# GaryGky/IDEAL-NeRF

Hardware: AMD Instinct MI355X
Metric: ray-samples/sec (64+128 pts, 512x512), whole job (higher is better)
Workload: dtype f32

## Files before the change

ideal-nerf_amd/_lib.py:

```python
import ctypes as C
import os

HERE = os.path.dirname(os.path.abspath(__file__))
LIB_PATH = os.environ.get("IDN_LIB") or os.path.join(HERE, "libidealnerf.so")

IDN_PREC_F32, IDN_PREC_BF16X3, IDN_PREC_BF16, IDN_PREC_FP16X3, IDN_PREC_BF16X6 = 0, 1, 2, 3, 4
RAY_FLOATS = 11
SAMPLE_MAX_REGION = 4096
SCORE_TILE = 32
PROF_KINDS = ("mlp_fwd", "mlp_fwd_save", "delta_chain", "dw_gemm", "dw_gemm_x6", "mlp_fwd_save_x6", "delta_chain_x6")

fp = C.c_void_p


class FaceNerfParams(C.Structure):
    _fields_ = [("pts_w", fp * 8), ("pts_b", fp * 8), ("views_w", fp * 3), ("views_b", fp * 3),
                ("alpha_w", fp), ("alpha_b", fp), ("rgb_w", fp), ("rgb_b", fp),
                ("dim_aud", C.c_int), ("dim_expr", C.c_int), ("dim_latent", C.c_int)]


class FaceNerfGrads(C.Structure):
    _fields_ = [("pts_w", fp * 8), ("pts_b", fp * 8), ("views_w", fp * 3), ("views_b", fp * 3),
                ("alpha_w", fp), ("alpha_b", fp), ("rgb_w", fp), ("rgb_b", fp)]


class CompositeOut(C.Structure):
    _fields_ = [(n, fp) for n in ("rgb_map", "disp_map", "acc_map", "depth_map", "weights", "rgb_fg", "last_weight")]


class RenderArgs(C.Structure):
    _fields_ = [("rays", fp), ("bc_rgb", fp), ("n_rays", C.c_int64), ("n_samples", C.c_int),
                ("n_importance", C.c_int), ("precision", C.c_int),
                ("packed_coarse", fp), ("folded_coarse", fp), ("packed_fine", fp), ("folded_fine", fp),
                ("t_vals", fp), ("t_rand", fp), ("u", fp), ("u_per_ray", C.c_int)] + \
               [(n, fp) for n in ("rgb_map", "disp_map", "acc_map", "depth_map", "last_weight", "rgb_fg",
                                  "rgb0", "disp0", "acc0", "z_std", "last_weight0", "rgb_fg0",
                                  "tap_z_coarse", "tap_raw_coarse", "tap_weights_coarse", "tap_cdf", "tap_inds",
                                  "tap_z_samples", "tap_z_fine", "tap_raw_fine", "tap_weights_fine")] + \
               [("workspace", fp), ("workspace_bytes", C.c_size_t), ("precision_fine_plus1", C.c_int),
                ("lindisp", C.c_int), ("white_bkgd", C.c_int), ("noise_coarse", fp), ("noise_fine", fp), ("fused_march", C.c_int),
                ("rng_mode", C.c_int), ("rng_seed", C.c_uint64), ("rng_ray0", C.c_int64)]


class AudioNetParams(C.Structure):
    _fields_ = [("conv_w", fp * 4), ("conv_b", fp * 4), ("fc_w", fp * 2), ("fc_b", fp * 2), ("dim_aud", C.c_int)]


class AudioNetGrads(C.Structure):
    _fields_ = [("conv_w", fp * 4), ("conv_b", fp * 4), ("fc_w", fp * 2), ("fc_b", fp * 2)]


class Frame(C.Structure):
    _fields_ = [("c2w", C.c_float * 12), ("H", C.c_int), ("W", C.c_int), ("focal", C.c_float), ("cx", C.c_float), ("cy", C.c_float),
                ("near_", C.c_float), ("far_", C.c_float), ("row0", C.c_int), ("nrows", C.c_int), ("rays_out", fp)]


class RenderOpts(C.Structure):
    _fields_ = [("colour_gate", C.c_int), ("gate_counters", fp)]


ABI_VERSION = 4

PROTOTYPES = {
    "idealnerf_version": (C.c_int, []),
    "idealnerf_last_error": (C.c_char_p, []),
    "idealnerf_packed_weight_floats": (C.c_size_t, [C.c_int]),
    "idealnerf_folded_bias_floats": (C.c_size_t, []),
    "idealnerf_pack_weights": (C.c_int, [C.POINTER(FaceNerfParams), C.c_int, fp, fp]),
    "idealnerf_fold_conditioning": (C.c_int, [C.POINTER(FaceNerfParams), fp, fp, fp, fp, fp]),
    "idealnerf_facenerf_fwd": (C.c_int, [fp, fp, C.c_int, fp, C.c_int64, fp, fp]),
    "idealnerf_query_rays_fwd": (C.c_int, [fp, fp, C.c_int, fp, fp, C.c_int64, C.c_int, fp, fp]),
    "idealnerf_query_points_fwd": (C.c_int, [fp, fp, C.c_int, fp, fp, C.c_int64, C.c_int, fp, fp]),
    "idealnerf_frame_rays": (C.c_int, [C.POINTER(C.c_float), C.c_int, C.c_int, C.c_float, C.c_float, C.c_float,
                                       C.c_float, C.c_float, C.c_int, C.c_int, fp, fp]),
    "idealnerf_to8b": (C.c_int, [fp, C.c_int64, C.c_int, fp, fp, fp]),
    "idealnerf_compose_to8b": (C.c_int, [fp, fp, fp, C.c_int64, C.c_int, fp, fp, fp, fp]),
    "idealnerf_philox_uniform": (C.c_int, [C.c_uint64, C.c_int, C.c_int64, C.c_int64, C.c_int, fp, fp]),
    "idealnerf_sample_pixels_workspace_bytes": (C.c_size_t, []),
    "idealnerf_sample_pixels": (C.c_int, [fp, C.c_int, C.c_int, C.c_int, C.c_int, C.c_int, C.c_int, C.c_uint64, C.c_uint64,
                                          fp, C.c_size_t, fp, fp]),
    "idealnerf_gather_rays": (C.c_int, [fp, C.c_int64, C.POINTER(C.c_float), C.c_int, C.c_int, C.c_float, C.c_float, C.c_float,
                                        fp, fp, fp, fp, fp, fp, fp, fp]),
    "idealnerf_frame_scores_workspace_bytes": (C.c_size_t, [C.c_int, C.c_int]),
    "idealnerf_frame_scores": (C.c_int, [fp, fp, fp, C.c_int, C.c_int, fp, fp, C.c_size_t, fp]),
    "idealnerf_coarse_depths": (C.c_int, [fp, fp, fp, C.c_int, C.c_int64, C.c_int, fp, fp]),
    "idealnerf_composite_fwd": (C.c_int, [fp, fp, fp, fp, fp, C.c_int, C.c_int64, C.c_int, C.POINTER(CompositeOut), fp]),
    "idealnerf_sample_pdf_fwd": (C.c_int, [fp, fp, fp, C.c_int, C.c_int64, C.c_int, C.c_int, fp, fp, fp, fp, fp, fp]),
    "idealnerf_march_fwd": (C.c_int, [fp, fp, fp, fp, fp, C.c_int, fp, C.c_int, C.c_int64, C.c_int, C.c_int,
                                      C.POINTER(CompositeOut), fp, fp, fp, fp, fp, fp]),
    "idealnerf_sample_pdf_bins_fwd": (C.c_int, [fp, fp, fp, C.c_int, C.c_int64, C.c_int, C.c_int, fp, fp, fp, fp]),
    "idealnerf_invert_cdf": (C.c_int, [fp, fp, fp, C.c_int, C.c_int64, C.c_int, C.c_int, fp, fp, fp]),
    "idealnerf_render_workspace_bytes": (C.c_size_t, [C.c_int64, C.c_int, C.c_int]),
    "idealnerf_render_rays_fwd": (C.c_int, [C.POINTER(RenderArgs), fp]),
    "idealnerf_render_frame_workspace_bytes": (C.c_size_t, [C.c_int64, C.c_int, C.c_int]),
    "idealnerf_render_frame_fwd": (C.c_int, [C.POINTER(RenderArgs), C.POINTER(Frame), fp]),
    "idealnerf_render_rays_fwd_opts": (C.c_int, [C.POINTER(RenderArgs), C.POINTER(RenderOpts), fp]),
    "idealnerf_render_frame_fwd_opts": (C.c_int, [C.POINTER(RenderArgs), C.POINTER(Frame), C.POINTER(RenderOpts), fp]),
    "idealnerf_colour_gate_max_dist": (C.c_float, []),
    "idealnerf_audio_net_saved_floats": (C.c_size_t, [C.c_int]),
    "idealnerf_audio_net_fwd": (C.c_int, [C.POINTER(AudioNetParams), fp, C.c_int, fp, fp, fp]),
    "idealnerf_audio_net_bwd": (C.c_int, [C.POINTER(AudioNetParams), C.POINTER(AudioNetGrads), fp, fp, fp, C.c_int, fp]),
    "idealnerf_train_acts_floats": (C.c_size_t, [C.c_int64]),
    "idealnerf_query_rays_train_fwd": (C.c_int, [fp, fp, C.c_int, fp, fp, C.c_int64, C.c_int, fp, fp, fp]),
    "idealnerf_pass_bwd_workspace_bytes": (C.c_size_t, [C.c_int64, C.c_int]),
    "idealnerf_pass_bwd": (C.c_int, [C.POINTER(FaceNerfParams), C.POINTER(FaceNerfGrads), fp, fp, fp, fp, fp, fp, fp,
                                     fp, C.c_int64, C.c_int, fp, fp, fp, fp, fp, fp, fp, C.c_size_t, fp]),
    "idealnerf_facenerf_train_fwd": (C.c_int, [fp, fp, C.c_int, fp, C.c_int64, fp, fp, fp]),
    "idealnerf_facenerf_bwd_workspace_bytes": (C.c_size_t, [C.c_int64]),
    "idealnerf_facenerf_bwd": (C.c_int, [C.POINTER(FaceNerfParams), C.POINTER(FaceNerfGrads), fp, fp, fp, fp, C.c_int64, fp,
                                         fp, fp, fp, fp, fp, C.c_size_t, fp]),
    "idealnerf_dw_gemm_workspace_bytes": (C.c_size_t, []),
    "idealnerf_dw_gemm": (C.c_int, [fp, C.c_int, fp, C.c_int, C.c_int64, fp, fp, C.c_int, fp, C.c_size_t, fp]),
    "idealnerf_profile_begin": (None, []),
    "idealnerf_profile_end": (C.c_int, [C.POINTER(C.c_double), C.POINTER(C.c_int64), C.POINTER(C.c_int64)]),
    "idealnerf_profile_end_kinds": (C.c_int, [C.POINTER(C.c_double), C.POINTER(C.c_int64), C.POINTER(C.c_int64)]),
}

_lib = None


class IdealNerfError(RuntimeError):
    pass


def load():
    global _lib
    if _lib is not None:
        return _lib
    if not os.path.exists(LIB_PATH):
        raise IdealNerfError(
            f"{LIB_PATH} is missing: build the HIP extension first "
            "(python ideal-nerf_amd/build.py, or __graft_entry__.build()). There is no fallback path.")
    lib = C.CDLL(LIB_PATH)
    for name, (res, args) in PROTOTYPES.items():
        fn = getattr(lib, name)
        fn.restype = res
        fn.argtypes = args
    if lib.idealnerf_version() != ABI_VERSION:
        raise IdealNerfError(f"{LIB_PATH} has ABI version {lib.idealnerf_version()}, this package binds version {ABI_VERSION}: rebuild it")
    _lib = lib
    return lib


def check(rc):
    if rc != 0:
        msg = load().idealnerf_last_error()
        raise IdealNerfError(f"libidealnerf error {rc}: {msg.decode() if msg else '?'}")
```

ideal-nerf_amd/csrc/capi.hip:

```cpp
#include "idn_internal.h"
#include <cstdarg>
#include <cstdio>

namespace idn {

static thread_local char g_err[512] = "";

int fail(int code, const char* fmt, ...) {
    va_list ap;
    va_start(ap, fmt);
    vsnprintf(g_err, sizeof(g_err), fmt, ap);
    va_end(ap);
    return code;
}

static int check_precision(int precision) {
    if (precision == IDN_PREC_F32 || precision == IDN_PREC_BF16X3 || precision == IDN_PREC_BF16 || precision == IDN_PREC_FP16X3 ||
        precision == IDN_PREC_BF16X6)
        return IDN_OK;
    return fail(IDN_EUNSUPPORTED, "precision %d is unknown (IDN_PREC_F32, IDN_PREC_BF16X3, IDN_PREC_BF16, IDN_PREC_FP16X3, IDN_PREC_BF16X6)", precision);
}
static int check_precision_train(int precision) {
    if (precision == IDN_PREC_F32 || precision == IDN_PREC_BF16X6) return IDN_OK;
    return fail(IDN_EUNSUPPORTED, "the training path runs fp32-grade arithmetic only: IDN_PREC_F32 or IDN_PREC_BF16X6 (got %d)", precision);
}

int launch_mlp(int precision, const float* packed, const float* folded, const float* x, const float* rays,
               const float* z, const float* pts, const float* dirs, int64_t n_points, int n_samples, float* raw,
               hipStream_t s, int gate, int64_t* gate_counters) {
    if (n_points > 0x7fffffffLL) return fail(IDN_EUNSUPPORTED, "n_points %lld exceeds 2^31-1 per launch", (long long)n_points);
    if ((rays || pts) && n_samples < 1) return fail(IDN_EINVAL, "n_samples < 1");
    if (precision == IDN_PREC_BF16X3)
        return launch_mlp_bf16x3(packed, folded, x, rays, z, pts, dirs, n_points, n_samples, raw, s);
    if (precision == IDN_PREC_BF16)
        return launch_mlp_bf16(packed, folded, x, rays, z, pts, dirs, n_points, n_samples, raw, s);
    if (precision == IDN_PREC_FP16X3)
        return launch_mlp_fp16x3(packed, folded, x, rays, z, pts, dirs, n_points, n_samples, raw, s);
    if (precision == IDN_PREC_BF16X6)
        return launch_mlp_bf16x6(packed, folded, x, rays, z, pts, dirs, n_points, n_samples, raw, s);
    return launch_mlp_f32(packed, folded, x, rays, z, pts, dirs, n_points, n_samples, raw, s, nullptr, 0, gate, gate_counters);
}

static int check_params(const idn_facenerf_params* p) {
    if (!p) return fail(IDN_EINVAL, "params is NULL");
    for (int i = 0; i < 8; ++i)
        if (!p->pts_w[i] || !p->pts_b[i]) return fail(IDN_EINVAL, "pts_linears.%d is NULL", i);
    for (int i = 0; i < 3; ++i)
        if (!p->views_w[i] || !p->views_b[i]) return fail(IDN_EINVAL, "views_linears.%d is NULL", i);
    if (!p->alpha_w || !p->alpha_b || !p->rgb_w || !p->rgb_b) return fail(IDN_EINVAL, "alpha/rgb head is NULL");
    if (p->dim_aud < 0 || p->dim_expr < 0 || p->dim_latent < 0) return fail(IDN_EINVAL, "negative conditioning width");
    return IDN_OK;
}

static const int kProfSlots = 8192;
static bool g_prof_on = false;
static int g_prof_n = 0;
static hipEvent_t g_prof_ev[kProfSlots][2];
static int g_prof_created = 0;
static int64_t g_prof_points[kProfSlots];
static int g_prof_kind[kProfSlots];

ProfScope::ProfScope(hipStream_t s_, int64_t points, int kind) : slot(-1), s(s_) {
    if (!g_prof_on || g_prof_n >= kProfSlots) return;
    slot = g_prof_n++;
    if (slot >= g_prof_created) {
        (void)hipEventCreate(&g_prof_ev[slot][0]);
        (void)hipEventCreate(&g_prof_ev[slot][1]);
        g_prof_created = slot + 1;
    }
    g_prof_points[slot] = points;
    g_prof_kind[slot] = (kind >= 0 && kind < IDN_PROF_KINDS) ? kind : 0;
    (void)hipEventRecord(g_prof_ev[slot][0], s);
}
ProfScope::~ProfScope() {
    if (slot >= 0) (void)hipEventRecord(g_prof_ev[slot][1], s);
}

}

using namespace idn;

extern "C" {

int idealnerf_version(void) { return 4; }
const char* idealnerf_last_error(void) { return g_err; }

size_t idealnerf_packed_weight_floats(int precision) {
    if (precision == IDN_PREC_F32 || precision == IDN_PREC_BF16X3 || precision == IDN_PREC_FP16X3) return (size_t)kStreamFrags * kFragFloats;
    if (precision == IDN_PREC_BF16) return (size_t)kPlainStreamFrags * kFragFloats;
    if (precision == IDN_PREC_BF16X6) return (size_t)kX6StreamFrags * kFragFloats;
    return 0;
}
size_t idealnerf_folded_bias_floats(void) { return kBiasFloats; }

int idealnerf_pack_weights(const idn_facenerf_params* p, int precision, float* packed, void* stream) {
    if (int e = check_params(p)) return e;
    if (int e = check_precision(precision)) return e;
    if (!packed) return fail(IDN_EINVAL, "packed is NULL");
    if (precision == IDN_PREC_BF16X3) return launch_pack_bf16x3(*p, packed, (hipStream_t)stream);
    if (precision == IDN_PREC_FP16X3) return launch_pack_bf16x3(*p, packed, (hipStream_t)stream, 1);
    if (precision == IDN_PREC_BF16) return launch_pack_bf16(*p, packed, (hipStream_t)stream);
    if (precision == IDN_PREC_BF16X6) return launch_pack_bf16x6(*p, packed, (hipStream_t)stream);
    return launch_pack_f32(*p, packed, (hipStream_t)stream);
}

int idealnerf_fold_conditioning(const idn_facenerf_params* p, const float* aud, const float* expr,
                                const float* latent, float* folded, void* stream) {
    if (int e = check_params(p)) return e;
    if (!folded) return fail(IDN_EINVAL, "folded is NULL");
    if ((p->dim_aud > 0) != (aud != nullptr)) return fail(IDN_EINVAL, "aud pointer does not match dim_aud=%d", p->dim_aud);
    if ((p->dim_expr > 0) != (expr != nullptr)) return fail(IDN_EINVAL, "expr pointer does not match dim_expr=%d", p->dim_expr);
    if ((p->dim_latent > 0) != (latent != nullptr))
        return fail(IDN_EINVAL, "latent pointer does not match dim_latent=%d", p->dim_latent);
    return launch_fold(*p, aud, expr, latent, folded, (hipStream_t)stream);
}

int idealnerf_facenerf_fwd(const float* packed, const float* folded, int precision, const float* x, int64_t n,
                           float* out, void* stream) {
    if (int e = check_precision(precision)) return e;
    if (n < 0) return fail(IDN_EINVAL, "n < 0");
    if (n == 0) return IDN_OK;
    if (!packed || !folded || !x || !out) return fail(IDN_EINVAL, "NULL pointer");
    return launch_mlp(precision, packed, folded, x, nullptr, nullptr, nullptr, nullptr, n, 1, out, (hipStream_t)stream);
}

int idealnerf_query_rays_fwd(const float* packed, const float* folded, int precision, const float* rays,
                             const float* z, int64_t n_rays, int n_samples, float* raw, void* stream) {
    if (int e = check_precision(precision)) return e;
    if (n_rays < 0 || n_samples < 1) return fail(IDN_EINVAL, "bad sizes n_rays=%lld n_samples=%d", (long long)n_rays, n_samples);
    if (n_rays == 0) return IDN_OK;
    if (!packed || !folded || !rays || !z || !raw) return fail(IDN_EINVAL, "NULL pointer");
    return launch_mlp(precision, packed, folded, nullptr, rays, z, nullptr, nullptr, n_rays * n_samples, n_samples, raw,
                      (hipStream_t)stream);
}

int idealnerf_query_points_fwd(const float* packed, const float* folded, int precision, const float* pts,
                               const float* viewdirs, int64_t n_rays, int n_samples, float* raw, void* stream) {
    if (int e = check_precision(precision)) return e;
    if (n_rays < 0 || n_samples < 1) return fail(IDN_EINVAL, "bad sizes n_rays=%lld n_samples=%d", (long long)n_rays, n_samples);
    if (n_rays == 0) return IDN_OK;
    if (!packed || !folded || !pts || !viewdirs || !raw) return fail(IDN_EINVAL, "NULL pointer");
    return launch_mlp(precision, packed, folded, nullptr, nullptr, nullptr, pts, viewdirs, n_rays * n_samples, n_samples,
                      raw, (hipStream_t)stream);
}

int idealnerf_frame_rays(const float* c2w, int H, int W, float focal, float cx, float cy, float near_, float far_,
                         int row0, int nrows, float* rays_out, void* stream) {
    if (!c2w || !rays_out) return fail(IDN_EINVAL, "NULL pointer");
    if (H <= 0 || W <= 0 || row0 < 0 || nrows < 0 || row0 + nrows > H) return fail(IDN_EINVAL, "bad frame/rows");
    if (nrows == 0) return IDN_OK;
    return launch_frame_rays(c2w, H, W, focal, cx, cy, near_, far_, row0, nrows, rays_out, (hipStream_t)stream);
}

int idealnerf_philox_uniform(uint64_t seed, int which, int64_t row0, int64_t n_rows, int n_cols, float* out, void* stream) {
    if (which != 0 && which != 1) return fail(IDN_EINVAL, "which %d (0 = stratified offsets, 1 = importance draws)", which);
    if (row0 < 0 || n_rows < 0 || n_cols < 0) return fail(IDN_EINVAL, "bad sizes");
    if (n_rows == 0 || n_cols == 0) return IDN_OK;
    if (!out) return fail(IDN_EINVAL, "NULL pointer");
    return launch_philox_uniform((unsigned long long)seed, which, row0, n_rows, n_cols, out, (hipStream_t)stream);
}

size_t idealnerf_sample_pixels_workspace_bytes(void) { return 4 * sizeof(int); }

int idealnerf_sample_pixels(const uint8_t* region_map, int H, int W, int n_rect, int n_outside, int n_mouth, int n_torso,
                            uint64_t seed, uint64_t draw, void* workspace, size_t workspace_bytes, int64_t* sel, void* stream) {
    const int counts[4] = {n_rect, n_outside, n_mouth, n_torso};
    static const char* const names[4] = {"rect", "outside", "mouth", "torso"};
    if (H <= 0 || W <= 0 || (int64_t)H * W > (1LL << 30)) return fail(IDN_EINVAL, "bad frame %d x %d", H, W);
    int64_t total = 0;
    for (int g = 0; g < 4; ++g) {
        if (counts[g] < 0) return fail(IDN_EINVAL, "negative %s count %d", names[g], counts[g]);
        if (counts[g] > IDN_SAMPLE_MAX_REGION)
            return fail(IDN_EUNSUPPORTED, "%s count %d exceeds IDN_SAMPLE_MAX_REGION = %d picks per region", names[g], counts[g],
                        IDN_SAMPLE_MAX_REGION);
        total += counts[g];
    }
    if (!region_map || !workspace || (total > 0 && !sel)) return fail(IDN_EINVAL, "NULL pointer");
    if (workspace_bytes < idealnerf_sample_pixels_workspace_bytes() || ((uintptr_t)workspace & 3u))
        return fail(IDN_EWORKSPACE, "workspace of %zu bytes (need %zu, int32-aligned)", workspace_bytes, idealnerf_sample_pixels_workspace_bytes());
    return launch_sample_pixels(region_map, H, W, counts, (unsigned long long)seed, (unsigned long long)draw, (int*)workspace,
                                (long long*)sel, (hipStream_t)stream);
}

int idealnerf_gather_rays(const int64_t* sel, int64_t n, const float* c2w, int H, int W, float focal, float cx, float cy,
                          const uint8_t* image, const uint8_t* background, const float* target_table, const float* background_table,
                          float* batch_rays, float* target_s, float* bc_rgb, void* stream) {
    if (H <= 0 || W <= 0 || (int64_t)H * W > (1LL << 30)) return fail(IDN_EINVAL, "bad frame %d x %d", H, W);
    if (n < 0 || n > 0x7fffffffLL / 8) return fail(IDN_EINVAL, "bad n %lld", (long long)n);
    if (n == 0) return IDN_OK;
    if (!sel || !c2w || !image || !background || !target_table || !background_table || !batch_rays || !target_s || !bc_rgb)
        return fail(IDN_EINVAL, "NULL pointer");
    return launch_gather_rays((const long long*)sel, n, c2w, H, W, focal, cx, cy, image, background, target_table, background_table,
                              batch_rays, target_s, bc_rgb, (hipStream_t)stream);
}

size_t idealnerf_frame_scores_workspace_bytes(int H, int W) { return frame_scores_workspace_bytes(H, W); }

int idealnerf_frame_scores(const float* pred, const uint8_t* truth, const uint8_t* regions, int H, int W, double* out,
                           void* workspace, size_t workspace_bytes, void* stream) {
    if (H <= 0 || W <= 0 || (int64_t)H * W > (1LL << 30)) return fail(IDN_EINVAL, "bad frame %d x %d", H, W);
    if (!pred || !truth || !out) return fail(IDN_EINVAL, "NULL pointer (pred, truth or out)");
    const size_t need = frame_scores_workspace_bytes(H, W);
    if (!workspace || workspace_bytes < need || ((uintptr_t)workspace & 7u))
        return fail(IDN_EINVAL, "workspace of %zu bytes (need %zu, 8-byte aligned)", workspace_bytes, need);
    return launch_frame_scores(pred, truth, regions, H, W, out, (double*)workspace, (hipStream_t)stream);
}

int idealnerf_coarse_depths(const float* rays, const float* t_vals, const float* t_rand, int lindisp, int64_t n_rays,
                            int n_samples, float* z, void* stream) {
    if (n_rays < 0 || n_samples < 1) return fail(IDN_EINVAL, "bad sizes");
    if (n_rays == 0) return IDN_OK;
    if (!rays || !t_vals || !z) return fail(IDN_EINVAL, "NULL pointer");
    return launch_coarse_depths(rays, t_vals, t_rand, n_rays, n_samples, lindisp, z, (hipStream_t)stream);
}

size_t idealnerf_audio_net_saved_floats(int n_windows) { return audio_net_saved_floats(n_windows); }
int idealnerf_audio_net_fwd(const idn_audio_net_params* p, const float* windows, int n_windows, float* out, float* saved,
                            void* stream) {
    return launch_audio_net_fwd(p, windows, n_windows, out, saved, (hipStream_t)stream);
}
int idealnerf_audio_net_bwd(const idn_audio_net_params* p, const idn_audio_net_grads* grads, const float* windows,
                            const float* saved, const float* d_out, int n_windows, void* stream) {
    return launch_audio_net_bwd(p, grads, windows, saved, d_out, n_windows, (hipStream_t)stream);
}

int idealnerf_to8b(const float* rgb, int64_t n_pixels, int swap_rb, uint8_t* out, int* nonfinite_flag, void* stream) {
    if (n_pixels < 0) return fail(IDN_EINVAL, "n_pixels < 0");
    if (n_pixels == 0) return IDN_OK;
    if (!rgb || !out) return fail(IDN_EINVAL, "NULL pointer");
    return launch_to8b(rgb, n_pixels, swap_rb, out, nonfinite_flag, (hipStream_t)stream);
}

int idealnerf_compose_to8b(const float* rgb_head, const float* last_weight, const float* rgb_fg, int64_t n_pixels,
                           int swap_rb, uint8_t* out, uint8_t* fg_out, int* nonfinite_flag, void* stream) {
    if (n_pixels < 0) return fail(IDN_EINVAL, "n_pixels < 0");
    if (n_pixels == 0) return IDN_OK;
    if (!rgb_head || !last_weight || !rgb_fg || !out) return fail(IDN_EINVAL, "NULL pointer");
    return launch_compose_to8b(rgb_head, last_weight, rgb_fg, n_pixels, swap_rb, out, fg_out, nonfinite_flag,
                               (hipStream_t)stream);
}

int idealnerf_composite_fwd(const float* raw, const float* z, const float* rays, const float* bc_rgb,
                            const float* sigma_noise, int white_bkgd, int64_t n_rays, int n_samples,
                            const idn_composite_out* out, void* stream) {
    if (n_rays < 0) return fail(IDN_EINVAL, "n_rays < 0");
    if (n_rays == 0) return IDN_OK;
    if (!raw || !z || !rays || !bc_rgb || !out) return fail(IDN_EINVAL, "NULL pointer");
    return launch_composite(raw, z, rays, bc_rgb, n_rays, n_samples, sigma_noise, white_bkgd, *out, (hipStream_t)stream);
}

int idealnerf_sample_pdf_fwd(const float* z, const float* weights, const float* u, int u_per_ray, int64_t n_rays,
                             int n_samples, int n_importance, float* z_samples, int64_t* inds, float* cdf,
                             float* z_fine, float* z_std, void* stream) {
    if (n_rays < 0) return fail(IDN_EINVAL, "n_rays < 0");
    if (n_rays == 0) return IDN_OK;
    if (!z || !weights || !u) return fail(IDN_EINVAL, "NULL pointer");
    if (n_samples < 3) return fail(IDN_EUNSUPPORTED, "sample_pdf needs n_samples >= 3");
    return launch_sample_pdf(z, weights, nullptr, nullptr, u, u_per_ray, n_rays, n_samples, n_importance, z_samples,
                             inds, cdf, z_fine, z_std, (hipStream_t)stream);
}

int idealnerf_march_fwd(const float* raw, const float* z, const float* rays, const float* bc_rgb, const float* sigma_noise,
                        int white_bkgd, const float* u, int u_per_ray, int64_t n_rays, int n_samples, int n_importance,
                        const idn_composite_out* out, float* z_samples, int64_t* inds, float* cdf, float* z_fine,
                        float* z_std, void* stream) {
    if (n_rays < 0) return fail(IDN_EINVAL, "n_rays < 0");
    if (n_rays == 0) return IDN_OK;
    if (!raw || !z || !rays || !bc_rgb || !u || !out) return fail(IDN_EINVAL, "NULL pointer");
    return launch_march(raw, z, rays, bc_rgb, sigma_noise, white_bkgd, *out, u, u_per_ray, n_rays, n_samples, n_importance,
                        z_samples, inds, cdf, z_fine, z_std, (hipStream_t)stream);
}

int idealnerf_sample_pdf_bins_fwd(const float* bins, const float* weights, const float* u, int u_per_ray,
                                  int64_t n_rays, int n_bins, int n_importance, float* z_samples, int64_t* inds,
                                  float* cdf, void* stream) {
    if (n_rays < 0) return fail(IDN_EINVAL, "n_rays < 0");
    if (n_rays == 0) return IDN_OK;
    if (!bins || !weights || !u) return fail(IDN_EINVAL, "NULL pointer");
    return launch_sample_pdf(nullptr, weights, nullptr, bins, u, u_per_ray, n_rays, n_bins + 1, n_importance, z_samples,
                             inds, cdf, nullptr, nullptr, (hipStream_t)stream);
}

int idealnerf_invert_cdf(const float* cdf, const float* bins, const float* u, int u_per_ray, int64_t n_rays,
                         int n_bins, int n_importance, float* z_samples, int64_t* inds, void* stream) {
    if (n_rays < 0) return fail(IDN_EINVAL, "n_rays < 0");
    if (n_rays == 0) return IDN_OK;
    if (!cdf || !bins || !u) return fail(IDN_EINVAL, "NULL pointer");
    return launch_sample_pdf(nullptr, nullptr, cdf, bins, u, u_per_ray, n_rays, n_bins + 1, n_importance, z_samples,
                             inds, nullptr, nullptr, nullptr, (hipStream_t)stream);
}

size_t idealnerf_train_acts_floats(int64_t n_points) {
    if (n_points <= 0) return 0;
    return (size_t)((n_points + 127) / 128 * 128) * kActColsAll;
}

int idealnerf_query_rays_train_fwd(const float* packed, const float* folded, int precision, const float* rays,
                                   const float* z, int64_t n_rays, int n_samples, float* raw, float* acts,
                                   void* stream) {
    if (int e = check_precision_train(precision)) return e;
    if (n_rays < 0 || n_samples < 1) return fail(IDN_EINVAL, "bad sizes");
    if (n_rays == 0) return IDN_OK;
    if (!packed || !folded || !rays || !z || !raw || !acts) return fail(IDN_EINVAL, "NULL pointer");
    const int64_t n = n_rays * n_samples;
    const int64_t p_pad = (n + 127) / 128 * 128;
    if (precision == IDN_PREC_BF16X6)
        return launch_mlp_bf16x6(packed, folded, nullptr, rays, z, nullptr, nullptr, n, n_samples, raw, (hipStream_t)stream, acts, p_pad);
    return launch_mlp_f32(packed, folded, nullptr, rays, z, nullptr, nullptr, n, n_samples, raw, (hipStream_t)stream,
                          acts, p_pad);
}

size_t idealnerf_pass_bwd_workspace_bytes(int64_t n_rays, int n_samples) {
    if (n_rays <= 0 || n_samples <= 0) return 0;
    return bwd_workspace_bytes(n_rays * n_samples);
}

static int check_grads(const idn_facenerf_grads* grads) {
    if (!grads) return fail(IDN_EINVAL, "grads is NULL");
    for (int i = 0; i < 8; ++i)
        if (!grads->pts_w[i] || !grads->pts_b[i]) return fail(IDN_EINVAL, "grad pts_linears.%d is NULL", i);
    for (int i = 0; i < 3; ++i)
        if (!grads->views_w[i] || !grads->views_b[i]) return fail(IDN_EINVAL, "grad views_linears.%d is NULL", i);
    if (!grads->alpha_w || !grads->alpha_b || !grads->rgb_w || !grads->rgb_b) return fail(IDN_EINVAL, "grad head is NULL");
    return IDN_OK;
}

int idealnerf_pass_bwd(const idn_facenerf_params* p, const idn_facenerf_grads* grads, const float* aud,
                       const float* expr, const float* latent, const float* acts, const float* raw, const float* z,
                       const float* rays, const float* bc_rgb, int64_t n_rays, int n_samples, const float* g_rgb_map,
                       const float* g_rgb_fg, const float* g_last_weight, const float* g_acc, float* d_aud,
                       float* d_latent, void* workspace, size_t workspace_bytes, void* stream) {
    if (int e = check_params(p)) return e;
    if (int e = check_grads(grads)) return e;
    if ((p->dim_aud > 0) != (aud != nullptr) || (p->dim_expr > 0) != (expr != nullptr) ||
        (p->dim_latent > 0) != (latent != nullptr))
        return fail(IDN_EINVAL, "conditioning pointers do not match the widths");
    if (n_rays < 0) return fail(IDN_EINVAL, "n_rays < 0");
    if (n_rays == 0) return IDN_OK;
    if (!acts || !raw || !z || !rays || !bc_rgb) return fail(IDN_EINVAL, "NULL pointer");
    return launch_pass_bwd(*p, *grads, aud, expr, latent, acts, raw, z, rays, bc_rgb, n_rays, n_samples, g_rgb_map,
                           g_rgb_fg, g_last_weight, g_acc, d_aud, d_latent, workspace, workspace_bytes,
                           (hipStream_t)stream);
}

int idealnerf_facenerf_train_fwd(const float* packed, const float* folded, int precision, const float* x, int64_t n,
                                 float* out, float* acts, void* stream) {
    if (int e = check_precision_train(precision)) return e;
    if (n < 0) return fail(IDN_EINVAL, "n < 0");
    if (n == 0) return IDN_OK;
    if (!packed || !folded || !x || !out || !acts) return fail(IDN_EINVAL, "NULL pointer");
    if (n > 0x7fffffffLL) return fail(IDN_EUNSUPPORTED, "n %lld exceeds 2^31-1 per launch", (long long)n);
    const int64_t p_pad = (n + 127) / 128 * 128;
    if (precision == IDN_PREC_BF16X6)
        return launch_mlp_bf16x6(packed, folded, x, nullptr, nullptr, nullptr, nullptr, n, 1, out, (hipStream_t)stream, acts, p_pad);
    return launch_mlp_f32(packed, folded, x, nullptr, nullptr, nullptr, nullptr, n, 1, out, (hipStream_t)stream, acts, p_pad);
}

size_t idealnerf_facenerf_bwd_workspace_bytes(int64_t n) {
    if (n <= 0) return 0;
    return bwd_workspace_bytes(n);
}

int idealnerf_facenerf_bwd(const idn_facenerf_params* p, const idn_facenerf_grads* grads, const float* aud, const float* expr,
                           const float* latent, const float* acts, int64_t n, const float* g_out, float* d_x, float* d_aud,
                           float* d_expr, float* d_latent, void* workspace, size_t workspace_bytes, void* stream) {
    if (int e = check_params(p)) return e;
    if (int e = check_grads(grads)) return e;
    if ((p->dim_aud > 0) != (aud != nullptr) || (p->dim_expr > 0) != (expr != nullptr) ||
        (p->dim_latent > 0) != (latent != nullptr))
        return fail(IDN_EINVAL, "conditioning pointers do not match the widths");
    if (n < 0) return fail(IDN_EINVAL, "n < 0");
    if (n == 0) return IDN_OK;
    if (!acts || !g_out) return fail(IDN_EINVAL, "NULL pointer");
    return launch_facenerf_bwd(*p, *grads, aud, expr, latent, acts, n, g_out, d_x, d_aud, d_expr, d_latent, workspace,
                               workspace_bytes, (hipStream_t)stream);
}

size_t idealnerf_dw_gemm_workspace_bytes(void) { return dw_gemm_workspace_bytes(); }

int idealnerf_dw_gemm(const float* delta, int ld_delta, const float* acts, int ld_acts, int64_t rows, float* dW, float* db,
                      int pipe, void* workspace, size_t workspace_bytes, void* stream) {
    if (!delta || !acts || !dW) return fail(IDN_EINVAL, "NULL pointer");
    return launch_dw_gemm(delta, ld_delta, acts, ld_acts, rows, dW, db, pipe, workspace, workspace_bytes, (hipStream_t)stream);
}

void idealnerf_profile_begin(void) {
    g_prof_n = 0;
    g_prof_on = true;
}

int idealnerf_profile_end_kinds(double* total_ms, int64_t* launches, int64_t* points) {
    g_prof_on = false;
    double ms[IDN_PROF_KINDS] = {0};
    int64_t n[IDN_PROF_KINDS] = {0}, pts[IDN_PROF_KINDS] = {0};
    for (int i = 0; i < g_prof_n; ++i) {
        IDN_HIP_CHECK(hipEventSynchronize(g_prof_ev[i][1]));
        float t = 0;
        IDN_HIP_CHECK(hipEventElapsedTime(&t, g_prof_ev[i][0], g_prof_ev[i][1]));
        const int k = g_prof_kind[i];
        ms[k] += t;
        n[k] += 1;
        pts[k] += g_prof_points[i];
    }
    for (int k = 0; k < IDN_PROF_KINDS; ++k) {
        if (total_ms) total_ms[k] = ms[k];
        if (launches) launches[k] = n[k];
        if (points) points[k] = pts[k];
    }
    return IDN_OK;
}

int idealnerf_profile_end(double* total_ms, int64_t* launches, int64_t* points) {
    double ms[IDN_PROF_KINDS];
    int64_t n[IDN_PROF_KINDS], pts[IDN_PROF_KINDS];
    if (int e = idealnerf_profile_end_kinds(ms, n, pts)) return e;
    if (total_ms) *total_ms = ms[IDN_PROF_MLP_FWD] + ms[IDN_PROF_MLP_FWD_SAVE] + ms[IDN_PROF_MLP_FWD_SAVE_X6];
    if (launches) *launches = n[IDN_PROF_MLP_FWD] + n[IDN_PROF_MLP_FWD_SAVE] + n[IDN_PROF_MLP_FWD_SAVE_X6];
    if (points) *points = pts[IDN_PROF_MLP_FWD] + pts[IDN_PROF_MLP_FWD_SAVE] + pts[IDN_PROF_MLP_FWD_SAVE_X6];
    return IDN_OK;
}

static const int64_t kRenderChunk = 32768;

static size_t align256(size_t x) { return (x + 255) & ~(size_t)255; }

struct RenderWs {
    float *z_c, *raw_c, *z_f, *raw_f;
    size_t bytes;
};
static RenderWs carve(char* base, int64_t n, int S, int Ni) {
    RenderWs w;
    const int64_t c = n < kRenderChunk ? n : kRenderChunk;
    const int Sf = S + Ni;
    size_t off = 0;
    auto take = [&](size_t floats) {
        float* p = reinterpret_cast<float*>(base + off);
        off += align256(floats * sizeof(float));
        return p;
    };
    w.z_c = take((size_t)c * S);
    w.raw_c = take((size_t)c * S * 4);
    w.z_f = take((size_t)c * Sf);
    w.raw_f = take((size_t)c * Sf * 4);
    w.bytes = off;
    return w;
}

size_t idealnerf_render_workspace_bytes(int64_t n_rays, int n_samples, int n_importance) {
    if (n_rays <= 0 || n_samples <= 0 || n_importance < 0) return 0;
    return carve(nullptr, n_rays, n_samples, n_importance).bytes;
}

static int render_impl(const idn_render_args* a, const idn_frame* frame, const idn_render_opts* opts, void* stream_);
int idealnerf_render_rays_fwd(const idn_render_args* a, void* stream_) { return render_impl(a, nullptr, nullptr, stream_); }
int idealnerf_render_rays_fwd_opts(const idn_render_args* a, const idn_render_opts* opts, void* stream_) { return render_impl(a, nullptr, opts, stream_); }
float idealnerf_colour_gate_max_dist(void) { return kGateMaxDist; }

static size_t frame_scratch_bytes(int64_t n_rays) {
    const int64_t c = n_rays < kRenderChunk ? n_rays : kRenderChunk;
    return align256((size_t)c * IDN_RAY_FLOATS * sizeof(float));
}
size_t idealnerf_render_frame_workspace_bytes(int64_t n_rays, int n_samples, int n_importance) {
    const size_t base = idealnerf_render_workspace_bytes(n_rays, n_samples, n_importance);
    return base ? base + frame_scratch_bytes(n_rays) : 0;
}
int idealnerf_render_frame_fwd(const idn_render_args* a, const idn_frame* f, void* stream_) { return idealnerf_render_frame_fwd_opts(a, f, nullptr, stream_); }
int idealnerf_render_frame_fwd_opts(const idn_render_args* a, const idn_frame* f, const idn_render_opts* opts, void* stream_) {
    if (!a || !f) return fail(IDN_EINVAL, "args / frame is NULL");
    if (a->rays) return fail(IDN_EINVAL, "frame mode derives the rays from the camera: args->rays must be NULL");
    if (f->H <= 0 || f->W <= 0 || f->row0 < 0 || f->nrows < 0 || f->row0 + f->nrows > f->H) return fail(IDN_EINVAL, "bad frame / rows");
    if (a->n_rays != (int64_t)f->nrows * f->W) return fail(IDN_EINVAL, "n_rays %lld != nrows * W = %lld", (long long)a->n_rays, (long long)f->nrows * f->W);
    return render_impl(a, f, opts, stream_);
}

static int render_impl(const idn_render_args* a, const idn_frame* frame, const idn_render_opts* opts, void* stream_) {
    if (!a) return fail(IDN_EINVAL, "args is NULL");
    if (opts && opts->colour_gate != 0 && opts->colour_gate != 1) return fail(IDN_EINVAL, "colour_gate %d (1 = on, the default; 0 = off)", opts->colour_gate);
    if (int e = check_precision(a->precision)) return e;
    const int prec_fine = a->precision_fine_plus1 ? a->precision_fine_plus1 - 1 : a->precision;
    if (int e = check_precision(prec_fine)) return e;
    const int64_t n = a->n_rays;
    const int S = a->n_samples, Ni = a->n_importance, Sf = S + Ni;
    if (n < 0 || S < 2 || Ni < 0) return fail(IDN_EINVAL, "bad sizes n=%lld S=%d Ni=%d", (long long)n, S, Ni);
    if (n == 0) return IDN_OK;
    if ((!a->rays && !frame) || !a->bc_rgb || !a->t_vals || !a->packed_coarse || !a->folded_coarse)
        return fail(IDN_EINVAL, "NULL input pointer");
    if (a->rng_mode != 0 && a->rng_mode != 1) return fail(IDN_EINVAL, "rng_mode %d (0 = t_rand / u as tensors, 1 = drawn in the kernels)", a->rng_mode);
    if (a->rng_mode && (a->t_rand || a->u)) return fail(IDN_EINVAL, "rng_mode 1 draws t_rand and u in the kernels: both pointers must be NULL");
    if (a->rng_mode && a->rng_ray0 < 0) return fail(IDN_EINVAL, "rng_ray0 < 0");
    if (Ni > 0 && (!a->packed_fine || !a->folded_fine || (!a->u && !a->rng_mode))) return fail(IDN_EINVAL, "fine pass inputs are NULL");
    if (Ni > 0 && S < 3) return fail(IDN_EUNSUPPORTED, "importance sampling needs n_samples >= 3");
    const size_t need_base = idealnerf_render_workspace_bytes(n, S, Ni);
    const size_t need = need_base + (frame ? frame_scratch_bytes(n) : 0);
    if (!a->workspace || a->workspace_bytes < need)
        return fail(IDN_EWORKSPACE, "workspace %zu bytes < required %zu", a->workspace_bytes, need);
    float* const ray_scratch = frame ? reinterpret_cast<float*>(reinterpret_cast<char*>(a->workspace) + need_base) : nullptr;
    if (a->fused_march != 0 && a->fused_march != 1 && a->fused_march != 2) return fail(IDN_EINVAL, "fused_march %d (0 = kernel sequence, 1 = one kernel, 2 = two kernels)", a->fused_march);
    if (a->fused_march) {
        if (a->precision != IDN_PREC_F32 || prec_fine != IDN_PREC_F32) return fail(IDN_EUNSUPPORTED, "fused march: built for the fp32 arithmetic");
        if (S != 64 || Ni != 128) return fail(IDN_EUNSUPPORTED, "fused march: built for n_samples = 64, n_importance = 128 (got %d, %d)", S, Ni);
        if (a->noise_coarse || a->noise_fine) return fail(IDN_EUNSUPPORTED, "fused march: no density noise");
    }
    const bool gate_on = !opts || opts->colour_gate;
    const int gate_c = gate_on && a->precision == IDN_PREC_F32 && !a->noise_coarse && !a->tap_raw_coarse;
    const int gate_f = gate_on && prec_fine == IDN_PREC_F32 && !a->noise_fine && !a->tap_raw_fine;
    int64_t* const gate_counters = opts ? opts->gate_counters : nullptr;
    hipStream_t st = (hipStream_t)stream_;
    const RenderWs w = carve(reinterpret_cast<char*>(a->workspace), n, S, Ni);

    auto off = [](auto* p, int64_t elems) { return p ? p + elems : p; };
    auto tap = [&](void* dst, const void* src, size_t bytes) -> int {
        if (!dst) return IDN_OK;
        IDN_HIP_CHECK(hipMemcpyAsync(dst, src, bytes, hipMemcpyDeviceToDevice, st));
        return IDN_OK;
    };

    for (int64_t r0 = 0; r0 < n; r0 += kRenderChunk) {
        const int64_t c = (n - r0 < kRenderChunk) ? n - r0 : kRenderChunk;
        const float* rays = frame ? ray_scratch : a->rays + r0 * IDN_RAY_FLOATS;
        if (frame) {
            if (int e = launch_frame_rays_pixels(frame->c2w, frame->H, frame->W, frame->focal, frame->cx, frame->cy, frame->near_, frame->far_,
                                                 (int64_t)frame->row0 * frame->W + r0, (int)c, ray_scratch, st))
                return e;
            if (frame->rays_out)
                IDN_HIP_CHECK(hipMemcpyAsync(frame->rays_out + r0 * IDN_RAY_FLOATS, ray_scratch, (size_t)c * IDN_RAY_FLOATS * sizeof(float),
                                             hipMemcpyDeviceToDevice, st));
        }
        const float* bc = a->bc_rgb + r0 * 3;
        const Draws draws{(unsigned long long)a->rng_seed, (long)(a->rng_ray0 + r0), a->rng_mode};
        if (int e = launch_coarse_depths(rays, a->t_vals, off(a->t_rand, r0 * S), c, S, a->lindisp, w.z_c, st, draws)) return e;
        if (!a->fused_march)
            if (int e = launch_mlp(a->precision, a->packed_coarse, a->folded_coarse, nullptr, rays, w.z_c, nullptr, nullptr, c * S, S, w.raw_c, st, gate_c, gate_counters)) return e;
        idn_composite_out co = {};
        const bool fine = Ni > 0;
        co.rgb_map = off(fine ? a->rgb0 : a->rgb_map, r0 * 3);
        co.disp_map = off(fine ? a->disp0 : a->disp_map, r0);
        co.acc_map = off(fine ? a->acc0 : a->acc_map, r0);
        co.depth_map = fine ? nullptr : off(a->depth_map, r0);
        co.weights = off(a->tap_weights_coarse, r0 * S);
        co.rgb_fg = off(fine ? a->rgb_fg0 : a->rgb_fg, r0 * 3);
        co.last_weight = off(fine ? a->last_weight0 : a->last_weight, r0);
        if (int e = tap(off(a->tap_z_coarse, r0 * S), w.z_c, (size_t)c * S * 4)) return e;
        if (a->fused_march) {
            idn_composite_out fo = {};
            fo.rgb_map = off(a->rgb_map, r0 * 3);
            fo.disp_map = off(a->disp_map, r0);
            fo.acc_map = off(a->acc_map, r0);
            fo.depth_map = off(a->depth_map, r0);
            fo.weights = off(a->tap_weights_fine, r0 * Sf);
            fo.rgb_fg = off(a->rgb_fg, r0 * 3);
            fo.last_weight = off(a->last_weight, r0);
            const float* u = a->u_per_ray ? off(a->u, r0 * Ni) : a->u;
            const bool split = a->fused_march == 2;
            if (int e = launch_render_fused(a->fused_march, a->packed_coarse, a->folded_coarse, a->packed_fine, a->folded_fine, rays, bc, w.z_c,
                                            split ? w.z_f : nullptr, u, a->u_per_ray, c, a->white_bkgd, co, fo, off(a->z_std, r0),
                                            off(a->tap_raw_coarse, r0 * S * 4), off(a->tap_raw_fine, r0 * Sf * 4),
                                            split ? nullptr : off(a->tap_z_fine, r0 * Sf), off(a->tap_inds, r0 * Ni), off(a->tap_z_samples, r0 * Ni),
                                            off(a->tap_cdf, r0 * (S - 1)), st, draws))
                return e;
            if (split)
                if (int e = tap(off(a->tap_z_fine, r0 * Sf), w.z_f, (size_t)c * Sf * 4)) return e;
            continue;
        }
        if (int e = tap(off(a->tap_raw_coarse, r0 * S * 4), w.raw_c, (size_t)c * S * 16)) return e;
        if (!fine) {
            if (int e = launch_composite(w.raw_c, w.z_c, rays, bc, c, S, off(a->noise_coarse, r0 * S), a->white_bkgd, co, st)) return e;
            continue;
        }
        const float* u = a->u_per_ray ? off(a->u, r0 * Ni) : a->u;
        if (int e = launch_march(w.raw_c, w.z_c, rays, bc, off(a->noise_coarse, r0 * S), a->white_bkgd, co, u, a->u_per_ray, c, S, Ni,
                                 off(a->tap_z_samples, r0 * Ni), off(a->tap_inds, r0 * Ni), off(a->tap_cdf, r0 * (S - 1)),
                                 w.z_f, off(a->z_std, r0), st, draws))
            return e;
        if (int e = launch_mlp(prec_fine, a->packed_fine, a->folded_fine, nullptr, rays, w.z_f, nullptr, nullptr, c * Sf, Sf, w.raw_f, st, gate_f,
                                 gate_counters ? gate_counters + 2 : nullptr)) return e;
        idn_composite_out fo = {};
        fo.rgb_map = off(a->rgb_map, r0 * 3);
        fo.disp_map = off(a->disp_map, r0);
        fo.acc_map = off(a->acc_map, r0);
        fo.depth_map = off(a->depth_map, r0);
        fo.weights = off(a->tap_weights_fine, r0 * Sf);
        fo.rgb_fg = off(a->rgb_fg, r0 * 3);
        fo.last_weight = off(a->last_weight, r0);
        if (int e = launch_composite(w.raw_f, w.z_f, rays, bc, c, Sf, off(a->noise_fine, r0 * Sf), a->white_bkgd, fo, st)) return e;
        if (int e = tap(off(a->tap_z_fine, r0 * Sf), w.z_f, (size_t)c * Sf * 4)) return e;
        if (int e = tap(off(a->tap_raw_fine, r0 * Sf * 4), w.raw_f, (size_t)c * Sf * 16)) return e;
    }
    return IDN_OK;
}

}
```

ideal-nerf_amd/csrc/idn_internal.h:

```cpp
#pragma once
#include <hip/hip_runtime.h>
#include <mutex>
#include <stdint.h>
#include <stddef.h>
#include "../../include/idealnerf.h"

namespace idn {

constexpr int kFragBytes = 1024;
constexpr int kFragFloats = 256;
constexpr int kSliceFrags = 64;
constexpr int kRingSlots = 2;
constexpr int kRingFrags = kRingSlots * kSliceFrags;
constexpr int kSliceBytes = kSliceFrags * kFragBytes;

constexpr int kNumLayers = 12;
constexpr int kLayerNT[kNumLayers] = {8, 8, 8, 8, 8, 8, 8, 8, 5, 4, 4, 1};
constexpr int kLayerKG[kNumLayers] = {8, 32, 32, 32, 32, 40, 32, 32, 36, 16, 16, 16};

constexpr int layer_f0(int l) {
    int f = 0;
    for (int i = 0; i < l; ++i) f += kLayerNT[i] * kLayerKG[i];
    return f;
}
constexpr int kUsedFrags = layer_f0(kNumLayers);
constexpr int kNumSlices =
    ((kUsedFrags + kSliceFrags - 1) / kSliceFrags + kRingSlots - 1) / kRingSlots * kRingSlots;
constexpr int kStreamFrags = kNumSlices * kSliceFrags;
static_assert(kUsedFrags == 2244, "layer table changed");
static_assert(kNumSlices % kRingSlots == 0, "slot of a slice must be static across passes");
static_assert(kRingFrags == 128, "FragReader addresses the ring as two 64-fragment halves");

constexpr int plain_f0(int l) {
    int f = 0;
    for (int i = 0; i < l; ++i) f += kLayerNT[i] * (kLayerKG[i] / 2);
    return f;
}
constexpr int kPlainUsedFrags = plain_f0(kNumLayers);
constexpr int kPlainNumSlices =
    ((kPlainUsedFrags + kSliceFrags - 1) / kSliceFrags + kRingSlots - 1) / kRingSlots * kRingSlots;
constexpr int kPlainStreamFrags = kPlainNumSlices * kSliceFrags;
static_assert(kPlainUsedFrags == 1122 && kPlainUsedFrags % 2 == 0, "plain stream table changed");

constexpr int kX6KFrags = 3;
constexpr int kX6SliceFrags = 16 * kX6KFrags;
constexpr int kX6RingFrags = kRingSlots * kX6SliceFrags;
constexpr int kX6UsedFrags = kX6KFrags * kPlainUsedFrags;
constexpr int kX6NumSlices = 2 * kNumSlices;
constexpr int kX6StreamFrags = kX6NumSlices * kX6SliceFrags;
static_assert(kX6UsedFrags <= kX6StreamFrags && kX6StreamFrags - kX6UsedFrags < kX6RingFrags + kX6SliceFrags, "x6 stream table");

constexpr int bias_off(int l) {
    int o = 0;
    for (int i = 0; i < l; ++i) o += kLayerNT[i] * 32;
    return o;
}
constexpr int kAlphaOff = bias_off(kNumLayers);
constexpr int kRgbOff = kAlphaOff + 256;
constexpr int kBiasFloats = kRgbOff + 3 * 128;
static_assert(kBiasFloats == 3136, "bias table changed");

constexpr int kSigmaChannel = 128;

constexpr float kGateMaxDist = 0.0125f;

enum { kActX0 = 0, kActDir = 1, kActA1 = 2, kActV1 = 10, kActCount = 13 };
constexpr int act_width(int i) { return i < 2 ? 64 : (i < kActV1 ? 256 : 128); }
constexpr int act_off(int i) {
    int o = 0;
    for (int k = 0; k < i; ++k) o += act_width(k);
    return o;
}
constexpr int kActCols = act_off(kActCount);
static_assert(kActCols == 2560, "activation slab layout changed");
constexpr int kMaskLayers = 11;
constexpr int kMaskFloatsPerPoint = kMaskLayers * 8;
constexpr int kActColsAll = kActCols + kMaskFloatsPerPoint;
__host__ __device__ inline size_t mask_index(int id, int64_t p_pad, int64_t wave_tile, int lane) {
    return ((size_t)id * (size_t)(p_pad / 32) + (size_t)wave_tile) * 64 + (size_t)lane;
}

int fail(int code, const char* fmt, ...);
#define IDN_HIP_CHECK(expr)                                                                   \
    do {                                                                                      \
        hipError_t _e = (expr);                                                               \
        if (_e != hipSuccess) return ::idn::fail(IDN_EHIP, "%s: %s", #expr, hipGetErrorString(_e)); \
    } while (0)

struct LaunchSetup {
    static constexpr int kMaxDevices = 64;
    std::mutex mu;
    int cus[kMaxDevices] = {};
    template <class OptIn>
    int get(OptIn&& opt_in, int* num_cu) {
        int dev = 0;
        IDN_HIP_CHECK(hipGetDevice(&dev));
        if (dev < 0 || dev >= kMaxDevices) return ::idn::fail(IDN_EUNSUPPORTED, "device index %d out of range", dev);
        std::lock_guard<std::mutex> lock(mu);
        if (!cus[dev]) {
            hipDeviceProp_t prop;
            IDN_HIP_CHECK(hipGetDeviceProperties(&prop, dev));
            if (int e = opt_in()) return e;
            cus[dev] = prop.multiProcessorCount;
        }
        *num_cu = cus[dev];
        return IDN_OK;
    }
};

struct ProfScope {
    int slot;
    hipStream_t s;
    ProfScope(hipStream_t s, int64_t points, int kind = IDN_PROF_MLP_FWD);
    ~ProfScope();
};

int launch_pack_f32(const idn_facenerf_params& p, float* packed, hipStream_t s);
int launch_pack_bf16x3(const idn_facenerf_params& p, float* packed, hipStream_t s, int fmt = 0);
int launch_pack_bf16x6(const idn_facenerf_params& p, float* packed, hipStream_t s);
int launch_mlp_bf16x6(const float* packed, const float* folded, const float* x, const float* rays, const float* z,
                      const float* pts, const float* dirs, int64_t n_points, int n_samples, float* raw, hipStream_t s,
                      float* acts = nullptr, int64_t p_pad = 0);
int launch_pack_bf16(const idn_facenerf_params& p, float* packed, hipStream_t s);
int launch_mlp_bf16(const float* packed, const float* folded, const float* x, const float* rays, const float* z,
                    const float* pts, const float* dirs, int64_t n_points, int n_samples, float* raw, hipStream_t s);
int launch_mlp_bf16x3(const float* packed, const float* folded, const float* x, const float* rays, const float* z,
                      const float* pts, const float* dirs, int64_t n_points, int n_samples, float* raw, hipStream_t s);
int launch_mlp_fp16x3(const float* packed, const float* folded, const float* x, const float* rays, const float* z,
                      const float* pts, const float* dirs, int64_t n_points, int n_samples, float* raw, hipStream_t s);
int launch_mlp(int precision, const float* packed, const float* folded, const float* x, const float* rays,
               const float* z, const float* pts, const float* dirs, int64_t n_points, int n_samples, float* raw,
               hipStream_t s, int gate = 0, int64_t* gate_counters = nullptr);
int launch_fold(const idn_facenerf_params& p, const float* aud, const float* expr, const float* latent,
                float* folded, hipStream_t s);
int launch_mlp_f32(const float* packed, const float* folded, const float* x, const float* rays, const float* z,
                   const float* pts, const float* dirs, int64_t n_points, int n_samples, float* raw, hipStream_t s,
                   float* acts = nullptr, int64_t p_pad = 0, int gate = 0, int64_t* gate_counters = nullptr);

int launch_frame_rays(const float* c2w, int H, int W, float focal, float cx, float cy, float near_, float far_,
                      int row0, int nrows, float* rays_out, hipStream_t s);
int launch_frame_rays_pixels(const float* c2w_host, int H, int W, float focal, float cx, float cy, float near_, float far_,
                             int64_t pix0, int npix, float* rays_out, hipStream_t s);
size_t audio_net_saved_floats(int n);
int launch_audio_net_fwd(const idn_audio_net_params* p, const float* windows, int n, float* out, float* saved, hipStream_t s);
int launch_audio_net_bwd(const idn_audio_net_params* p, const idn_audio_net_grads* g, const float* windows, const float* saved,
                         const float* d_out, int n, hipStream_t s);
int launch_to8b(const float* rgb, int64_t n_pixels, int swap_rb, unsigned char* out, int* flag, hipStream_t s);
int launch_compose_to8b(const float* head, const float* lw, const float* fg, int64_t n_pixels, int swap_rb,
                        unsigned char* out, unsigned char* fg_out, int* flag, hipStream_t s);
struct Draws {
    unsigned long long seed;
    long ray0;
    int on;
};
int launch_philox_uniform(unsigned long long seed, int which, int64_t row0, int64_t n_rows, int n_cols, float* out, hipStream_t s);
int launch_sample_pixels(const unsigned char* map, int H, int W, const int counts[4], unsigned long long seed, unsigned long long draw,
                         int* population, long long* sel, hipStream_t s);
int launch_gather_rays(const long long* sel, int64_t n, const float* c2w_host, int H, int W, float focal, float cx, float cy,
                       const unsigned char* image, const unsigned char* background, const float* target_table,
                       const float* background_table, float* batch_rays, float* target_s, float* bc_rgb, hipStream_t s);
size_t frame_scores_workspace_bytes(int H, int W);
int launch_frame_scores(const float* pred, const unsigned char* truth, const unsigned char* regions, int H, int W, double* out,
                        double* partial, hipStream_t s);
int launch_coarse_depths(const float* rays, const float* t_vals, const float* t_rand, int64_t n_rays, int S,
                         int lindisp, float* z, hipStream_t s, Draws draws = Draws{0, 0, 0});
int launch_composite(const float* raw, const float* z, const float* rays, const float* bc, int64_t n_rays, int S,
                     const float* noise, int white_bkgd, const idn_composite_out& out, hipStream_t s);
int launch_march(const float* raw, const float* z, const float* rays, const float* bc, const float* noise, int white_bkgd,
                 const idn_composite_out& out, const float* u, int u_per_ray, int64_t n_rays, int S, int Ni,
                 float* z_samples, int64_t* inds, float* cdf_out, float* z_fine, float* z_std, hipStream_t s,
                 Draws draws = Draws{0, 0, 0});
int launch_render_fused(int arrangement, const float* packed_c, const float* folded_c, const float* packed_f, const float* folded_f,
                        const float* rays, const float* bc, const float* z_c, float* z_f, const float* u, int u_per_ray, int64_t n_rays,
                        int white_bkgd, const idn_composite_out& co, const idn_composite_out& fo, float* z_std, float* tap_raw_c,
                        float* tap_raw_f, float* tap_z_fine, int64_t* tap_inds, float* tap_z_samples, float* tap_cdf, hipStream_t s,
                        Draws draws = Draws{0, 0, 0});
int launch_sample_pdf(const float* z, const float* weights, const float* cdf_in, const float* bins_in,
                      const float* u, int u_per_ray, int64_t n_rays, int S, int Ni, float* z_samples,
                      int64_t* inds, float* cdf_out, float* z_fine, float* z_std, hipStream_t s);

constexpr int kBwdStages = 11;
constexpr int kBwdNT[kBwdStages] = {4, 4, 4, 8, 8, 8, 8, 8, 8, 8, 8};
constexpr int kBwdKG[kBwdStages] = {2, 16, 16, 18, 32, 32, 32, 32, 32, 32, 32};
constexpr int kBwdHeadFrags = 280, kBwdTrunk0 = 384;
constexpr int bwd_f0(int s) {
    if (s >= 4) return kBwdTrunk0 + 256 * (s - 4);
    int f = 0;
    for (int i = 0; i < s; ++i) f += kBwdNT[i] * kBwdKG[i];
    return f;
}
static_assert(bwd_f0(3) + kBwdNT[3] * kBwdKG[3] == kBwdHeadFrags, "head stages");
constexpr int kBwdStreamFrags = kBwdTrunk0 + 7 * 256;
static_assert(kBwdStreamFrags % kSliceFrags == 0 && kBwdTrunk0 % kRingFrags == 0, "ring phase of the trunk stages");
constexpr int kBwdNumSlices = kBwdStreamFrags / kSliceFrags;

int launch_pack_f32_bwd(const idn_facenerf_params& p, float* packed_bwd, hipStream_t s);
int launch_delta_chain(const float* packed_bwd, const float* acts, int64_t p_pad, const float* d_rgb, float* dv0,
                       float* dv2, float* dv1, float* const da[8], hipStream_t s);
size_t bwd_stream_floats_x6();
int launch_pack_bf16x6_bwd(const idn_facenerf_params& p, float* packed_bwd, hipStream_t s);
int launch_delta_chain_x6(const float* packed_bwd, const float* acts, int64_t p_pad, const float* d_rgb, float* dv0,
                          float* dv2, float* dv1, float* const da[8], hipStream_t s);

size_t dw_gemm_workspace_bytes();
int launch_dw_gemm(const float* delta, int ld_delta, const float* acts, int ld_acts, int64_t rows, float* dW, float* db, int pipe,
                   void* ws, size_t ws_bytes, hipStream_t s);

size_t bwd_workspace_bytes(int64_t n_points);
int launch_pass_bwd(const idn_facenerf_params& p, const idn_facenerf_grads& gr, const float* aud, const float* expr,
                    const float* latent, const float* acts, const float* raw, const float* z, const float* rays,
                    const float* bc, int64_t n_rays, int S, const float* g_rgb, const float* g_fg, const float* g_lw,
                    const float* g_acc, float* d_aud, float* d_latent, void* ws, size_t ws_bytes, hipStream_t s);
int launch_facenerf_bwd(const idn_facenerf_params& p, const idn_facenerf_grads& gr, const float* aud, const float* expr,
                        const float* latent, const float* acts, int64_t n, const float* g_out, float* d_x, float* d_aud,
                        float* d_expr, float* d_latent, void* ws, size_t ws_bytes, hipStream_t s);

}
```

ideal-nerf_amd/csrc/mlp_common.h:

```cpp
#pragma once
#include "idn_internal.h"
#include <utility>

namespace idn {

typedef float f32x16 __attribute__((ext_vector_type(16)));
typedef float f32x4 __attribute__((ext_vector_type(4)));

template <int N>
using ic = std::integral_constant<int, N>;

template <class F, int... I>
__device__ __forceinline__ void static_for_impl(F&& f, std::integer_sequence<int, I...>) {
    (f(ic<I>{}), ...);
}
template <int N, class F>
__device__ __forceinline__ void static_for(F&& f) {
    static_for_impl(f, std::make_integer_sequence<int, N>{});
}

#define GLOBAL_PTR(p) ((const __attribute__((address_space(1))) void*)(p))
#define LDS_PTR(p) ((__attribute__((address_space(3))) void*)(p))

constexpr int kAhead = kRingSlots - 1;

template <int NW, int SLICE_FRAGS = kSliceFrags, int SLOTS = kRingSlots, bool DUAL = false>
struct WStreamT {
    static constexpr int kSliceFragsT = SLICE_FRAGS;
    static constexpr int kSliceBytesT = SLICE_FRAGS * kFragBytes;
    static constexpr int kSlotsT = SLOTS;
    static constexpr int kAheadT = SLOTS - 1;
    static constexpr int kPieceBytes = NW * kFragBytes;
    static constexpr int kPieces = kSliceBytesT / kPieceBytes;
    static constexpr int kVmcntOpen = (kAheadT - 1) * kPieces;
    static_assert(kSliceBytesT % kPieceBytes == 0 && kPieces % 4 == 0, "a wave's pieces come in groups of four (one M0 / scalar offset per group)");

    __amdgpu_buffer_rsrc_t rsrc;
    uint32_t voff;
    uint32_t soff;
    int next_slice;
    int num_slices;
    char* ring_wave;
    const float* dual_stream[2];
    int dual_first, dual_period, dual_pass;

    __device__ __forceinline__ void init(const float* stream, int slices, char* ring, int tid, int wave) {
        rsrc = __builtin_amdgcn_make_buffer_rsrc(const_cast<float*>(stream), 0, slices * kSliceBytesT, 0x00020000);
        voff = (tid & 63) * 16 + wave * (kPieces * kFragBytes);
        soff = 0;
        next_slice = 0;
        num_slices = slices;
        ring_wave = ring + wave * (kPieces * kFragBytes);
        static_for<kAheadT>([&](auto S_) { issue_rest<decltype(S_)::value, 0>(); });
    }
    __device__ __forceinline__ void advance() {
        soff += kSliceBytesT;
        if (++next_slice == num_slices) {
            next_slice = 0;
            soff = 0;
            if constexpr (DUAL) {
                if (++dual_pass == dual_period) dual_pass = 0;
                rsrc = __builtin_amdgcn_make_buffer_rsrc(const_cast<float*>(dual_stream[dual_pass < dual_first ? 0 : 1]), 0, num_slices * kSliceBytesT, 0x00020000);
            }
        }
    }
    __device__ __forceinline__ void init_dual(const float* stream0, const float* stream1, int first, int period, int slices, char* ring, int tid, int wave) {
        static_assert(DUAL, "two streams");
        dual_stream[0] = stream0;
        dual_stream[1] = stream1;
        dual_first = first;
        dual_period = period;
        dual_pass = 0;
        init(stream0, slices, ring, tid, wave);
    }
    template <int SLOT, int J>
    __device__ __forceinline__ void issue_piece() {
        __builtin_amdgcn_raw_ptr_buffer_load_lds(rsrc, LDS_PTR(ring_wave + SLOT * kSliceBytesT + (J / 4) * (4 * kFragBytes)), 16, voff,
                                                 soff + (J / 4) * (4 * kFragBytes), (J % 4) * kFragBytes, 0);
        if constexpr (J == kPieces - 1) advance();
    }
    template <int SLOT, int J0>
    __device__ __forceinline__ void issue_rest() {
        static_for<kPieces - J0>([&](auto I) { issue_piece<SLOT, J0 + decltype(I)::value>(); });
    }
    template <int YOUNGER = 0>
    __device__ __forceinline__ void open_slice() {
        static_assert(kVmcntOpen + YOUNGER <= 63, "vmcnt is a 6-bit field");
        asm volatile("s_waitcnt vmcnt(%0)" ::"n"(kVmcntOpen + YOUNGER) : "memory");
        __builtin_amdgcn_s_barrier();
        asm volatile("" ::: "memory");
    }
    template <int F>
    __device__ __forceinline__ void step_piece() {
        constexpr int jpos = (F % SLICE_FRAGS) / 2;
        constexpr int slot = (F / SLICE_FRAGS + kAheadT) % SLOTS;
        if constexpr (jpos < kPieces) issue_piece<slot, jpos>();
    }
    template <int F, int JPOS>
    __device__ __forceinline__ void step_piece_at() {
        constexpr int slot = (F / SLICE_FRAGS + kAheadT) % SLOTS;
        if constexpr (JPOS < kPieces) issue_piece<slot, JPOS>();
    }
};
using WStream = WStreamT<4>;

struct FragReader {
    uint32_t addr0, addr1;
    uint32_t addr2;
    f32x4 pref0, pref1;

    template <int F, int RING_FRAGS = kRingFrags>
    __device__ __forceinline__ f32x4 issue() const {
        constexpr int fr = F % RING_FRAGS;
        f32x4 v;
        if constexpr (fr < 64)
            asm volatile("ds_read_b128 %0, %1 offset:%2" : "=v"(v) : "v"(addr0), "n"(fr * kFragBytes) : "memory");
        else if constexpr (fr < 128)
            asm volatile("ds_read_b128 %0, %1 offset:%2" : "=v"(v) : "v"(addr1), "n"((fr - 64) * kFragBytes) : "memory");
        else
            asm volatile("ds_read_b128 %0, %1 offset:%2" : "=v"(v) : "v"(addr2), "n"((fr - 128) * kFragBytes) : "memory");
        return v;
    }
    template <int Newer>
    static __device__ __forceinline__ void retire(f32x4& v0, f32x4& v1) {
        if constexpr (Newer == 0) asm volatile("s_waitcnt lgkmcnt(0)" : "+v"(v0), "+v"(v1)::"memory");
        else asm volatile("s_waitcnt lgkmcnt(2)" : "+v"(v0), "+v"(v1)::"memory");
    }
};

template <int F_END, int STREAM_FRAGS = kStreamFrags, class WS>
__device__ __forceinline__ void finish_pass(WS& ws) {
    static_assert(F_END % 2 == 0, "pairs");
    static_for<(STREAM_FRAGS - F_END) / 2>([&](auto I) {
        constexpr int f = F_END + 2 * decltype(I)::value;
        if constexpr (f % kSliceFrags == 0) ws.open_slice();
        ws.template step_piece<f>();
    });
}

template <int Q>
__device__ __forceinline__ void bias_quad(f32x16& tile, const float* bias_tile_half ) {
    const f32x4 b = *reinterpret_cast<const f32x4*>(bias_tile_half + 8 * Q);
    tile[4 * Q + 0] = b.x;
    tile[4 * Q + 1] = b.y;
    tile[4 * Q + 2] = b.z;
    tile[4 * Q + 3] = b.w;
}
__device__ __forceinline__ void bias_tile(f32x16& tile, const float* bias_tile_half) {
    bias_quad<0>(tile, bias_tile_half);
    bias_quad<1>(tile, bias_tile_half);
    bias_quad<2>(tile, bias_tile_half);
    bias_quad<3>(tile, bias_tile_half);
}
template <int NT>
__device__ __forceinline__ void load_bias(f32x16 (&acc)[NT], const float* bias_half ) {
    static_for<NT>([&](auto T) { bias_tile(acc[decltype(T)::value], bias_half + 32 * decltype(T)::value); });
}

__device__ __forceinline__ float relu1(float x) {
    const int b = __builtin_bit_cast(int, x);
    return __builtin_bit_cast(float, b > 0 ? b : 0);
}
template <int R0, int CNT>
__device__ __forceinline__ void relu_regs(f32x16& tile) {
    static_for<CNT>([&](auto R) {
        constexpr int r = R0 + decltype(R)::value;
        if constexpr (r < 16) tile[r] = relu1(tile[r]);
    });
}
template <int NT>
__device__ __forceinline__ void relu_tiles(f32x16 (&t)[NT]) {
    static_for<NT>([&](auto T) { relu_regs<0, 16>(t[decltype(T)::value]); });
}

struct NoSide {
    template <int T, int S, int H>
    __device__ __forceinline__ void operator()(ic<T>, ic<S>, ic<H>) const {}
};

struct PeLane {
    int h;
    uint32_t off01, off10;
    __device__ __forceinline__ void init(int h_) {
        h = h_;
        off01 = h_ ? 0x80000000u : 0x40000000u;
        off10 = h_ ? 0x40000000u : 0x80000000u;
    }
};
struct PeAxes {
    uint32_t hi[3], lo[3];
    float raw[3];
    __device__ __forceinline__ void init(const float (&v)[3], int h) {
        uint32_t H[3], Lw[3];
        static_for<3>([&](auto A) {
            constexpr int a = decltype(A)::value;
            const double ph = (double)v[a] * 0.15915494309189535;
            const double t = __builtin_amdgcn_fract(ph) * 4294967296.0;
            H[a] = (uint32_t)t;
            Lw[a] = (uint32_t)((t - (double)H[a]) * 4294967296.0);
        });
        static_for<3>([&](auto A) {
            constexpr int a = decltype(A)::value, a1 = (a + 1) % 3;
            hi[a] = h ? H[a1] : H[a];
            lo[a] = h ? Lw[a1] : Lw[a];
            raw[a] = h ? v[a1] : v[a];
        });
    }
};
template <int K, int L>
struct PeFeat {
    static constexpr bool raw = K < 3;
    static constexpr bool trig = K >= 3 && K < 3 + 6 * L;
    static constexpr int t = trig ? K - 3 : 0;
    static constexpr int b = t / 6, sc = (t % 6) / 3;
};
template <int B>
__device__ __forceinline__ uint32_t pe_phase(const PeAxes& ax, int a) {
    if constexpr (B == 0) return ax.hi[a];
    else return __builtin_amdgcn_alignbit(ax.hi[a], ax.lo[a], 32 - B);
}
template <int K0, int L>
__device__ __forceinline__ float pe_slot(const PeAxes& ax, const PeLane& ln) {
    using F0 = PeFeat<K0, L>;
    using F1 = PeFeat<K0 + 4, L>;
    constexpr int a = K0 % 3;
    if constexpr (!F0::trig && !F1::trig) {
        if constexpr (F0::raw) return ln.h ? 0.0f : ax.raw[a];
        else return 0.0f;
    } else {
        constexpr int b0 = F0::trig ? F0::b : F1::b, b1 = F1::trig ? F1::b : F0::b;
        constexpr int sc0 = F0::trig ? F0::sc : F1::sc, sc1 = F1::trig ? F1::sc : F0::sc;
        uint32_t T;
        if constexpr (b0 == b1) T = pe_phase<b0>(ax, a);
        else T = ln.h ? pe_phase<b1>(ax, a) : pe_phase<b0>(ax, a);
        uint32_t u;
        if constexpr (sc0 == sc1) u = T + (((uint32_t)sc0 << 30) + 0x40000000u);
        else u = T + (sc0 == 0 ? ln.off01 : ln.off10);
        const int rr2 = (int)((u << 1) + 0x80000000u);
        const float x = (float)rr2 * 7.3145905512e-10f;
        const float s2 = x * x;
        float pp = -2.391218132e-08f;
        pp = fmaf(pp, s2, 2.752665757e-06f);
        pp = fmaf(pp, s2, -1.984089153e-04f);
        pp = fmaf(pp, s2, 8.333331268e-03f);
        pp = fmaf(pp, s2, -1.666666663e-01f);
        float r = fmaf(x * s2, pp, x);
        r = __uint_as_float(__float_as_uint(r) ^ (u & 0x80000000u));
        if constexpr (!F0::trig) r = ln.h ? r : (F0::raw ? ax.raw[a] : 0.0f);
        if constexpr (!F1::trig) r = ln.h ? 0.0f : r;
        return r;
    }
}

enum { kModeRays = 0, kModeX = 1, kModePts = 2 };
struct MlpArgs {
    const float* wstream;
    const float* bias;
    const float* x;
    const float* rays;
    const float* z;
    const float* pts;
    const float* dirs;
    long n_points;
    int S;
    float* raw;
    float* acts;
    long p_pad;
};
struct MlpGateArgs : MlpArgs {
    unsigned long long* gate_counters;
};

struct PointIn {
    float f[10];
    float zn;
    int last;
};
struct NoHook {
    __device__ __forceinline__ void operator()() const {}
};
template <int MODE, int NW = 4>
__device__ __forceinline__ void load_point(const MlpArgs& a, long tile, int wave, int m, PointIn& in) {
    if constexpr (MODE == kModeX) return;
    long P = tile * (32 * NW) + wave * 32 + m;
    if (P >= a.n_points) P = a.n_points - 1;
    const unsigned ray = (unsigned)P / (unsigned)a.S;
    if constexpr (MODE == kModeRays) {
        const float* rr = a.rays + (long)ray * IDN_RAY_FLOATS;
        in.f[0] = rr[0]; in.f[1] = rr[1]; in.f[2] = rr[2];
        in.f[3] = rr[3]; in.f[4] = rr[4]; in.f[5] = rr[5];
        in.f[6] = rr[8]; in.f[7] = rr[9]; in.f[8] = rr[10];
        in.f[9] = a.z[P];
    } else {
        in.f[0] = a.pts[P * 3 + 0]; in.f[1] = a.pts[P * 3 + 1]; in.f[2] = a.pts[P * 3 + 2];
        in.f[3] = a.dirs[(long)ray * 3 + 0]; in.f[4] = a.dirs[(long)ray * 3 + 1]; in.f[5] = a.dirs[(long)ray * 3 + 2];
    }
}
__device__ __forceinline__ void touch_point(PointIn& in) {
#pragma unroll
    for (int i = 0; i < 10; ++i) asm volatile("" : "+v"(in.f[i]));
}

__device__ __forceinline__ void load_gate_point(const MlpArgs& a, long tile, int wave, int m, PointIn& in) {
    long P = tile * 128 + wave * 32 + m;
    if (P >= a.n_points) P = a.n_points - 1;
    const unsigned ray = (unsigned)P / (unsigned)a.S;
    in.last = ((unsigned)P - ray * (unsigned)a.S == (unsigned)a.S - 1u) ? 1 : 0;
    in.zn = a.z[in.last ? P : P + 1];
}
__device__ __forceinline__ void touch_gate_point(PointIn& in) { asm volatile("" : "+v"(in.zn), "+v"(in.last)); }
__device__ __forceinline__ bool gate_point_dead(const PointIn& in, float sigma) {
    const float dn = sqrtf((in.f[3] * in.f[3] + in.f[4] * in.f[4]) + in.f[5] * in.f[5]);
    float dist = in.zn - in.f[9];
    dist = dist * dn;
    return in.last != 0 || (sigma <= 0.0f && fabsf(dist) <= kGateMaxDist);
}
template <int MODE>
__device__ __forceinline__ void point_of(const PointIn& in, float (&p)[3], float (&v)[3]) {
    if constexpr (MODE == kModeRays) {
        p[0] = in.f[0] + in.f[3] * in.f[9];
        p[1] = in.f[1] + in.f[4] * in.f[9];
        p[2] = in.f[2] + in.f[5] * in.f[9];
        v[0] = in.f[6]; v[1] = in.f[7]; v[2] = in.f[8];
    } else {
        p[0] = in.f[0]; p[1] = in.f[1]; p[2] = in.f[2];
        v[0] = in.f[3]; v[1] = in.f[4]; v[2] = in.f[5];
    }
}

template <int MODE, class Use>
__device__ __forceinline__ void input_features(const MlpArgs& a, long Pc, int h, const PeLane& pln, const PointIn& in,
                                               Use&& use) {
    if constexpr (MODE == kModeX) {
        const float* xr = a.x + Pc * (IDN_PTS_CH + IDN_VIEWS_CH) + 4 * h;
        use([&](auto K) { constexpr int k = decltype(K)::value; return (k + 4 * h < IDN_PTS_CH) ? xr[k] : 0.0f; },
            [&](auto K) { constexpr int k = decltype(K)::value; return (k + 4 * h < IDN_VIEWS_CH) ? xr[IDN_PTS_CH + k] : 0.0f; });
    } else {
        float p[3], v[3];
        point_of<MODE>(in, p, v);
        PeAxes axp, axd;
        axp.init(p, h);
        axd.init(v, h);
        use([&](auto K) { return pe_slot<decltype(K)::value, 10>(axp, pln); },
            [&](auto K) { return pe_slot<decltype(K)::value, 4>(axd, pln); });
    }
}

__device__ __forceinline__ uint32_t off_bit_source(float x) {
    const int b = __builtin_bit_cast(int, x);
    return (uint32_t)((b > 0 ? b : 0) - 1);
}
template <int T>
__device__ __forceinline__ void collect_signs(const f32x16& tile, uint32_t* mk) {
    static_for<16>([&](auto R) {
        mk[T >> 1] = __builtin_amdgcn_alignbit(mk[T >> 1], off_bit_source(tile[decltype(R)::value]), 31);
    });
}

__device__ __forceinline__ __amdgpu_buffer_rsrc_t rows_rsrc(float* first_row, int ld) {
    return __builtin_amdgcn_make_buffer_rsrc(first_row, 0, 32 * ld * 4, 0x00020000);
}

constexpr int kMlpLds = kRingFrags * kFragBytes + kBiasFloats * 4;
constexpr int kMlpLdsGate = kMlpLds + 16;
constexpr int kStagePitch = 33;
constexpr int kStageFloats = 32 * kStagePitch;
constexpr int kMlpLdsTrain = kMlpLds + 4 * kStageFloats * 4;


}
```

ideal-nerf_amd/csrc/mlp_f32.hip:

```cpp
#include "mlp_f32_layers.h"

namespace idn {

template <int NT, int STEPS, int LD>
struct SaveSide {
    static constexpr bool kShadowStore = STEPS >= 8;
    uint32_t* mk;
    f32x16* out;
    __amdgpu_buffer_rsrc_t rsrc;
    uint32_t voff;
    float* stage;
    float* rb;
    uint32_t raddr;
    int m, h;
    template <int T>
    __device__ __forceinline__ void scatter(ic<T>) const {
        static_for<16>([&](auto R) {
            constexpr int r = decltype(R)::value;
            stage[m * kStagePitch + (r & 3) + 8 * (r >> 2) + 4 * h] = out[T][r];
        });
        asm volatile("" ::: "memory");
    }
    template <int Q>
    __device__ __forceinline__ void rows_read(ic<Q>) const {
        static_for<4>([&](auto I) {
            constexpr int i = decltype(I)::value;
            asm volatile("ds_read_b32 %0, %1 offset:%2" : "=v"(rb[i]) : "v"(raddr), "n"(2 * (4 * Q + i) * kStagePitch * 4) : "memory");
        });
    }
    template <int T, int Q>
    __device__ __forceinline__ void rows_store(ic<T>, ic<Q>) const {
        asm volatile("" : "+v"(rb[0]), "+v"(rb[1]), "+v"(rb[2]), "+v"(rb[3]));
        static_for<4>([&](auto I) {
            constexpr int i = decltype(I)::value;
            __builtin_amdgcn_raw_buffer_store_b32(__builtin_bit_cast(unsigned, rb[i]), rsrc, voff, (2 * (4 * Q + i) * LD + 32 * T) * 4, 0);
        });
    }
    template <int T>
    __device__ __forceinline__ void flush_tile(ic<T>) const {
        scatter(ic<T>{});
        static_for<4>([&](auto Q) {
            rows_read(Q);
            asm volatile("s_waitcnt lgkmcnt(0)" : "+v"(rb[0]), "+v"(rb[1]), "+v"(rb[2]), "+v"(rb[3])::"memory");
            rows_store(ic<T>{}, Q);
        });
    }
    __device__ __forceinline__ void finish() const {
        if constexpr (!kShadowStore) static_for<NT - 1>([&](auto T) { collect_signs<decltype(T)::value>(out[decltype(T)::value], mk); });
        collect_signs<NT - 1>(out[NT - 1], mk);
        relu_regs<0, 16>(out[NT - 1]);
        if constexpr (kShadowStore) flush_tile(ic<NT - 1>{});
        else {
            static_for<NT - 1>([&](auto T) { relu_regs<0, 16>(out[decltype(T)::value]); });
            static_for<NT>([&](auto T) { flush_tile(T); });
        }
    }
    template <int T, int S, int H>
    __device__ __forceinline__ void operator()(ic<T>, ic<S>, ic<H>) const {
        if constexpr (kShadowStore && T > 0 && H == 0) {
            if constexpr (S == 0) {
                collect_signs<T - 1>(out[T - 1], mk);
                relu_regs<0, 16>(out[T - 1]);
            }
            if constexpr (S == 1) scatter(ic<T - 1>{});
            if constexpr (S >= 3 && S <= 6) rows_store(ic<T - 1>{}, ic<S - 3>{});
            if constexpr (S >= 2 && S <= 5) rows_read(ic<S - 2>{});
        }
    }
};

template <int MODE, bool SAVE, bool GATE = false>
__global__ __launch_bounds__(256, 1) void mlp_f32_kernel(std::conditional_t<GATE, MlpGateArgs, MlpArgs> a) {
    static_assert(!GATE || (MODE == kModeRays && !SAVE), "the colour gate is built for the rays-mode inference pass");
    extern __shared__ __attribute__((aligned(16))) char smem[];
    char* ring = smem;
    float* bias_s = reinterpret_cast<float*>(smem + kRingFrags * kFragBytes);
    float* stage = reinterpret_cast<float*>(smem + kMlpLds) + (threadIdx.x >> 6) * kStageFloats;
    const uint32_t raddr = (uint32_t)(uintptr_t)(__attribute__((address_space(3))) float*)stage +
                           (((threadIdx.x & 63) >> 5) * kStagePitch + (threadIdx.x & 31)) * 4;

    const int tid = threadIdx.x;
    const int lane = tid & 63;
    const int wave = __builtin_amdgcn_readfirstlane(tid >> 6);
    const int m = lane & 31, h = lane >> 5;

    for (int i = tid; i < kBiasFloats; i += 256) bias_s[i] = a.bias[i];
    GateWord* gate_words = (GateWord*)(__attribute__((address_space(3))) char*)(smem + kMlpLds);
    if constexpr (GATE)
        if (tid < 2) gate_words[tid] = 0u;
    int gate_par = 0;
    __syncthreads();

    WStream ws;
    ws.init(a.wstream, kNumSlices, ring, tid, wave);
    PeLane pln;
    pln.init(h);

    FragReader fr;
    fr.addr0 = (uint32_t)(uintptr_t)(__attribute__((address_space(3))) char*)ring + lane * 16;
    fr.addr1 = fr.addr0 + 64 * kFragBytes;
    const float* bias_h = bias_s + 4 * h;
    const long ntiles = (a.n_points + 127) >> 7;

    PointIn cur, nxt;
    load_point<MODE>(a, blockIdx.x, wave, m, cur);
    if constexpr (GATE) load_gate_point(a, blockIdx.x, wave, m, cur);
    nxt = cur;
    for (long tile = blockIdx.x; tile < ntiles; tile += gridDim.x) {
        const long P = tile * 128 + wave * 32 + m;
        const bool valid = P < a.n_points;
        const long Pc = valid ? P : a.n_points - 1;

        float pe[8][4], pd[4][4];
        if constexpr (MODE == kModeX) {
            const float* xr = a.x + Pc * (IDN_PTS_CH + IDN_VIEWS_CH);
            static_for<8>([&](auto G) {
                static_for<4>([&](auto J) {
                    constexpr int g = decltype(G)::value, j = decltype(J)::value;
                    const int k = 8 * g + 4 * h + j;
                    pe[g][j] = (k < IDN_PTS_CH) ? xr[k] : 0.0f;
                });
            });
            static_for<4>([&](auto G) {
                static_for<4>([&](auto J) {
                    constexpr int g = decltype(G)::value, j = decltype(J)::value;
                    const int k = 8 * g + 4 * h + j;
                    pd[g][j] = (k < IDN_VIEWS_CH) ? xr[IDN_PTS_CH + k] : 0.0f;
                });
            });
        } else {
            float p[3], v[3];
            point_of<MODE>(cur, p, v);
            PeAxes axp, axd;
            axp.init(p, h);
            axd.init(v, h);
            static_for<8>([&](auto G) {
                static_for<4>([&](auto J) {
                    constexpr int g = decltype(G)::value, j = decltype(J)::value;
                    pe[g][j] = pe_slot<8 * g + j, 10>(axp, pln);
                    if constexpr (g < 4) pd[g][j] = pe_slot<8 * g + j, 4>(axd, pln);
                });
            });
        }
        const long p0 = tile * 128 + wave * 32;
        if constexpr (SAVE) {
            {
                float* x0 = a.acts + act_off(kActX0) * a.p_pad + P * 64 + 4 * h;
                float* dr = a.acts + act_off(kActDir) * a.p_pad + P * 64 + 4 * h;
                static_for<8>([&](auto G) {
                    constexpr int g = decltype(G)::value;
                    f32x4 v = {pe[g][0], pe[g][1], pe[g][2], pe[g][3]};
                    *reinterpret_cast<f32x4*>(x0 + 8 * g) = v;
                });
                static_for<8>([&](auto G) {
                    constexpr int g = decltype(G)::value;
                    f32x4 v = {0.f, 0.f, 0.f, 0.f};
                    if constexpr (g < 4) v = f32x4{pd[g][0], pd[g][1], pd[g][2], pd[g][3]};
                    *reinterpret_cast<f32x4*>(dr + 8 * g) = v;
                });
            }
        }

        float rgb[3], sigma;
        if constexpr (GATE) {
            const bool skipped = f32_inference_pass<true>(
                pe, pd, bias_s, bias_h, ws, fr,
                [&]() { load_point<MODE>(a, tile + gridDim.x, wave, m, nxt); load_gate_point(a, tile + gridDim.x, wave, m, nxt); },
                [&]() { touch_point(nxt); touch_gate_point(nxt); }, rgb, sigma,
                [&](float sg) { return !valid || gate_point_dead(cur, sg); }, gate_words + gate_par, gate_words + (gate_par ^ 1));
            gate_par ^= 1;
            if (a.gate_counters && tid == 0) {
                atomicAdd(a.gate_counters + 0, 1ull);
                if (skipped) atomicAdd(a.gate_counters + 1, 1ull);
            }
        } else if constexpr (!SAVE) {
            f32_inference_pass(pe, pd, bias_s, bias_h, ws, fr,
                               [&]() { if constexpr (MODE != kModeX) load_point<MODE>(a, tile + gridDim.x, wave, m, nxt); },
                               [&]() { if constexpr (MODE != kModeX) touch_point(nxt); }, rgb, sigma);
        } else {
            f32x16 A[8], B[8], V[5];
            float rb[4];
            uint32_t mk[4] = {0u, 0u, 0u, 0u};
            auto store_mask = [&](int id) {
                typedef uint32_t u32x4 __attribute__((ext_vector_type(4)));
                u32x4* mp = reinterpret_cast<u32x4*>(a.acts + (size_t)kActCols * a.p_pad) + mask_index(id, a.p_pad, tile * 4 + wave, lane);
                *mp = u32x4{mk[0], mk[1], mk[2], mk[3]};
            };
            auto pe_get = [&](auto G, auto J) { return pe[decltype(G)::value][decltype(J)::value]; };
            auto tiles_get = [](f32x16* arr) {
                return [arr](auto G, auto J) {
                    constexpr int g = decltype(G)::value, j = decltype(J)::value;
                    return arr[g >> 2][(g & 3) * 4 + j];
                };
            };
            auto layer = [&](auto F0c, auto NTc, auto KGc, auto& out, auto&& bget, const float* bias_l, int save_idx) {
                constexpr int F0 = decltype(F0c)::value, NT = decltype(NTc)::value, KG = decltype(KGc)::value;
                constexpr bool LAST = (F0 + NT * KG == kUsedFrags) || F0 == layer_f0(8) || F0 == layer_f0(10);
                static_assert(layer_f0(5) % kSliceFrags == 0 && layer_f0(6) % kSliceFrags == 0, "input prefetch hooks sit on slice boundaries");
                auto hook = [&]() {
                    if constexpr (MODE != kModeX && F0 == layer_f0(5)) load_point<MODE>(a, tile + gridDim.x, wave, m, nxt);
                    if constexpr (MODE != kModeX && F0 == layer_f0(6)) touch_point(nxt);
                };
                load_bias<NT>(out, bias_l);
                if (save_idx >= 0) {
                    const SaveSide<NT, KG / 2, 32 * NT> side{mk, &out[0], rows_rsrc(a.acts + (long)act_off(save_idx) * a.p_pad + p0 * (32 * NT), 32 * NT),
                                                             (uint32_t)((h * (32 * NT) + m) * 4), stage, rb, raddr, m, h};
                    run_layer<F0, NT, KG, LAST>(out, bget, ws, fr, side, hook);
                    side.finish();
                    store_mask(save_idx - kActA1);
                } else {
                    run_layer<F0, NT, KG, LAST>(out, bget, ws, fr, NoSide{}, hook);
                }
            };
            layer(ic<layer_f0(0)>{}, ic<8>{}, ic<8>{}, A, pe_get, bias_h + bias_off(0), kActA1 + 0);
#pragma unroll 1
            for (int l = 1; l <= 3; l += 2) {
                layer(ic<layer_f0(1)>{}, ic<8>{}, ic<32>{}, B, tiles_get(A), bias_h + l * 256, kActA1 + l);
                layer(ic<layer_f0(2)>{}, ic<8>{}, ic<32>{}, A, tiles_get(B), bias_h + (l + 1) * 256, kActA1 + l + 1);
            }
            layer(ic<layer_f0(5)>{}, ic<8>{}, ic<40>{}, B,
                  [&](auto G, auto J) {
                      constexpr int g = decltype(G)::value, j = decltype(J)::value;
                      if constexpr (g < 8) return pe[g][j];
                      else return A[(g - 8) >> 2][((g - 8) & 3) * 4 + j];
                  },
                  bias_h + bias_off(5), kActA1 + 5);
            layer(ic<layer_f0(6)>{}, ic<8>{}, ic<32>{}, A, tiles_get(B), bias_h + bias_off(6), kActA1 + 6);
            layer(ic<layer_f0(7)>{}, ic<8>{}, ic<32>{}, B, tiles_get(A), bias_h + bias_off(7), kActA1 + 7);
            f32x16(&V4a)[4] = reinterpret_cast<f32x16(&)[4]>(V);
            layer(ic<layer_f0(8)>{}, ic<4>{}, ic<36>{}, V4a,
                  [&](auto G, auto J) {
                      constexpr int g = decltype(G)::value, j = decltype(J)::value;
                      if constexpr (g < 32) return B[g >> 2][(g & 3) * 4 + j];
                      else return pd[g - 32][j];
                  },
                  bias_h + bias_off(8), -1);
            {
                constexpr int f_from = layer_f0(8) + 4 * 36, f_to = layer_f0(9);
                static_assert(f_from / kSliceFrags == (f_to - 1) / kSliceFrags && f_to % kSliceFrags != 0, "the walk stays inside one open slice");
                static_for<(f_to - f_from) / 2>([&](auto I) { ws.template step_piece<f_from + 2 * decltype(I)::value>(); });
                fr.pref0 = fr.template issue<f_to>();
                fr.pref1 = fr.template issue<f_to + 1>();
            }
            {
                float s0 = 0.f, s1 = 0.f, s2 = 0.f, s3 = 0.f;
                static_for<8>([&](auto T) {
                    constexpr int t = decltype(T)::value;
                    static_for<4>([&](auto Q) {
                        constexpr int q = decltype(Q)::value;
                        const f32x4 w = *reinterpret_cast<const f32x4*>(bias_h + kAlphaOff + 32 * t + 8 * q);
                        s0 = fmaf(w.x, B[t][4 * q + 0], s0);
                        s1 = fmaf(w.y, B[t][4 * q + 1], s1);
                        s2 = fmaf(w.z, B[t][4 * q + 2], s2);
                        s3 = fmaf(w.w, B[t][4 * q + 3], s3);
                    });
                });
                const float part = (s0 + s1) + (s2 + s3);
                sigma = bias_s[bias_off(8) + kSigmaChannel] + (part + __shfl_xor(part, 32, 64));
            }
            {
                f32x16(&V4)[4] = reinterpret_cast<f32x16(&)[4]>(V);
                static_for<4>([&](auto T) { collect_signs<decltype(T)::value>(V4[decltype(T)::value], mk); });
                store_mask(kActV1 - kActA1);
                relu_tiles<4>(V4);
                const SaveSide<4, 1, 128> side{mk, &V4[0], rows_rsrc(a.acts + (long)act_off(kActV1) * a.p_pad + p0 * 128, 128),
                                               (uint32_t)((h * 128 + m) * 4), stage, rb, raddr, m, h};
                static_for<4>([&](auto T) { side.flush_tile(T); });
            }
            f32x16(&A4)[4] = reinterpret_cast<f32x16(&)[4]>(A);
            f32x16(&V4b)[4] = reinterpret_cast<f32x16(&)[4]>(V);
            layer(ic<layer_f0(9)>{}, ic<4>{}, ic<16>{}, A4, tiles_get(V), bias_h + bias_off(9), kActV1 + 1);
            layer(ic<layer_f0(10)>{}, ic<4>{}, ic<16>{}, V4b, tiles_get(A), bias_h + bias_off(10), kActV1 + 2);
            finish_pass<layer_f0(11)>(ws);
            rgb[0] = bias_s[bias_off(11) + 0];
            rgb[1] = bias_s[bias_off(11) + 1];
            rgb[2] = bias_s[bias_off(11) + 2];
            {
                float part[3] = {0.f, 0.f, 0.f};
                static_for<4>([&](auto T) {
                    constexpr int t = decltype(T)::value;
                    f32x16 vt = V[t];
                    asm volatile("" : "+v"(vt));
                    static_for<3>([&](auto Cc) {
                        constexpr int c = decltype(Cc)::value;
                        static_for<4>([&](auto Q) {
                            constexpr int q = decltype(Q)::value;
                            const f32x4 w = *reinterpret_cast<const f32x4*>(bias_h + kRgbOff + 128 * c + 32 * t + 8 * q);
                            part[c] = fmaf(w.x, vt[4 * q + 0], part[c]);
                            part[c] = fmaf(w.y, vt[4 * q + 1], part[c]);
                            part[c] = fmaf(w.z, vt[4 * q + 2], part[c]);
                            part[c] = fmaf(w.w, vt[4 * q + 3], part[c]);
                        });
                    });
                    asm volatile("" : "+v"(part[0]), "+v"(part[1]), "+v"(part[2])::"memory");
                });
                static_for<3>([&](auto Cc) {
                    constexpr int c = decltype(Cc)::value;
                    rgb[c] += part[c] + __shfl_xor(part[c], 32, 64);
                });
            }
        }

        if (valid && h == 0) {
            f32x4 o;
            o.x = rgb[0];
            o.y = rgb[1];
            o.z = rgb[2];
            o.w = sigma;
            *reinterpret_cast<f32x4*>(a.raw + P * 4) = o;
        }
        cur = nxt;
    }
    __builtin_amdgcn_s_waitcnt(0);
    __syncthreads();
}

int launch_mlp_f32(const float* packed, const float* folded, const float* x, const float* rays, const float* z,
                   const float* pts, const float* dirs, int64_t n_points, int n_samples, float* raw, hipStream_t s,
                   float* acts, int64_t p_pad, int gate, int64_t* gate_counters) {
    if (n_points <= 0) return IDN_OK;
    static LaunchSetup setup;
    int num_cu = 0;
    if (int e = setup.get([]() -> int {
            IDN_HIP_CHECK(hipFuncSetAttribute(reinterpret_cast<const void*>(&mlp_f32_kernel<kModeRays, false>),
                                              hipFuncAttributeMaxDynamicSharedMemorySize, kMlpLds));
            IDN_HIP_CHECK(hipFuncSetAttribute(reinterpret_cast<const void*>(&mlp_f32_kernel<kModeRays, false, true>),
                                              hipFuncAttributeMaxDynamicSharedMemorySize, kMlpLdsGate));
            IDN_HIP_CHECK(hipFuncSetAttribute(reinterpret_cast<const void*>(&mlp_f32_kernel<kModeX, false>),
                                              hipFuncAttributeMaxDynamicSharedMemorySize, kMlpLds));
            IDN_HIP_CHECK(hipFuncSetAttribute(reinterpret_cast<const void*>(&mlp_f32_kernel<kModePts, false>),
                                              hipFuncAttributeMaxDynamicSharedMemorySize, kMlpLds));
            IDN_HIP_CHECK(hipFuncSetAttribute(reinterpret_cast<const void*>(&mlp_f32_kernel<kModeRays, true>),
                                              hipFuncAttributeMaxDynamicSharedMemorySize, kMlpLdsTrain));
            IDN_HIP_CHECK(hipFuncSetAttribute(reinterpret_cast<const void*>(&mlp_f32_kernel<kModeX, true>),
                                              hipFuncAttributeMaxDynamicSharedMemorySize, kMlpLdsTrain));
            return IDN_OK;
        }, &num_cu))
        return e;
    const int64_t ntiles = (n_points + 127) / 128;
    const int grid = (int)(ntiles < num_cu ? ntiles : num_cu);
    if (gate && (acts || x || pts)) return fail(IDN_EUNSUPPORTED, "the colour gate is built for the rays-mode inference launch");
    MlpArgs a{packed, folded, x, rays, z, pts, dirs, (long)n_points, n_samples, raw, acts, (long)p_pad};
    ProfScope prof(s, n_points, acts ? IDN_PROF_MLP_FWD_SAVE : IDN_PROF_MLP_FWD);
    if (acts) {
        if (pts) return fail(IDN_EUNSUPPORTED, "activation saving is built for the rays+z and the pre-embedded-row input modes");
        if (x)
            hipLaunchKernelGGL((mlp_f32_kernel<kModeX, true>), dim3(grid), dim3(256), kMlpLdsTrain, s, a);
        else
            hipLaunchKernelGGL((mlp_f32_kernel<kModeRays, true>), dim3(grid), dim3(256), kMlpLdsTrain, s, a);
    } else if (x)
        hipLaunchKernelGGL((mlp_f32_kernel<kModeX, false>), dim3(grid), dim3(256), kMlpLds, s, a);
    else if (pts)
        hipLaunchKernelGGL((mlp_f32_kernel<kModePts, false>), dim3(grid), dim3(256), kMlpLds, s, a);
    else if (gate) {
        MlpGateArgs ga;
        static_cast<MlpArgs&>(ga) = a;
        ga.gate_counters = reinterpret_cast<unsigned long long*>(gate_counters);
        hipLaunchKernelGGL((mlp_f32_kernel<kModeRays, false, true>), dim3(grid), dim3(256), kMlpLdsGate, s, ga);
    }
    else
        hipLaunchKernelGGL((mlp_f32_kernel<kModeRays, false>), dim3(grid), dim3(256), kMlpLds, s, a);
    IDN_HIP_CHECK(hipGetLastError());
    return IDN_OK;
}

}
```

ideal-nerf_amd/csrc/mlp_f32_layers.h:

```cpp
#pragma once
#include "mlp_common.h"

namespace idn {

__device__ __forceinline__ f32x16 mfma(float a, float b, f32x16 c) {
    return __builtin_amdgcn_mfma_f32_32x32x2f32(a, b, c, 0, 0, 0);
}

template <int F0, int NT, int KG, bool LAST = false, bool OPENED = false, class BGet, class Side, class Hook = NoHook, class WS = WStream>
__device__ __forceinline__ void run_layer(f32x16 (&out)[NT], BGet&& bget, WS& ws, FragReader& fr, Side&& side,
                                          Hook&& after_open = NoHook{}) {
    constexpr int STEPS = KG / 2, NP = NT * STEPS;
    static_assert(KG % 2 == 0 && F0 % 2 == 0, "fragments are consumed in pairs");
    static_assert(!OPENED || F0 % kSliceFrags == 0, "only a layer that starts a slice can find it opened");
    if constexpr (F0 % kSliceFrags == 0) {
        if constexpr (!OPENED) ws.open_slice();
        after_open();
        fr.pref0 = fr.template issue<F0>();
        fr.pref1 = fr.template issue<F0 + 1>();
    }
    f32x4 a0 = fr.pref0, a1 = fr.pref1;
    static_for<NP>([&](auto PI) {
        constexpr int pi = decltype(PI)::value;
        constexpr int t = pi / STEPS, s = pi % STEPS, g0 = 2 * s, g1 = g0 + 1;
        constexpr int f = F0 + 2 * pi;
        constexpr bool next_crosses = ((f + 2) % kSliceFrags == 0);
        f32x4 n0 = a0, n1 = a1;
        if constexpr (!next_crosses && !(LAST && pi + 1 == NP)) {
            n0 = fr.template issue<f + 2>();
            n1 = fr.template issue<f + 3>();
            FragReader::retire<2>(a0, a1);
        } else {
            FragReader::retire<0>(a0, a1);
        }
        ws.template step_piece<f>();
        out[t] = mfma(a0.x, bget(ic<g0>{}, ic<0>{}), out[t]);
        out[t] = mfma(a0.y, bget(ic<g0>{}, ic<1>{}), out[t]);
        out[t] = mfma(a0.z, bget(ic<g0>{}, ic<2>{}), out[t]);
        out[t] = mfma(a0.w, bget(ic<g0>{}, ic<3>{}), out[t]);
        side(ic<t>{}, ic<s>{}, ic<0>{});
        out[t] = mfma(a1.x, bget(ic<g1>{}, ic<0>{}), out[t]);
        out[t] = mfma(a1.y, bget(ic<g1>{}, ic<1>{}), out[t]);
        out[t] = mfma(a1.z, bget(ic<g1>{}, ic<2>{}), out[t]);
        out[t] = mfma(a1.w, bget(ic<g1>{}, ic<3>{}), out[t]);
        side(ic<t>{}, ic<s>{}, ic<1>{});
        __builtin_amdgcn_sched_barrier(0);
        if constexpr (next_crosses && pi + 1 < NP) {
            ws.open_slice();
            n0 = fr.template issue<f + 2>();
            n1 = fr.template issue<f + 3>();
        }
        a0 = n0;
        a1 = n1;
    });
    fr.pref0 = a0;
    fr.pref1 = a1;
}

template <int NT, int STEPS, bool DEFER>
struct LayerSide {
    f32x16* out;
    f32x16* deferred;
    const float* bias_half;
    template <int T, int S, int H>
    __device__ __forceinline__ void operator()(ic<T>, ic<S>, ic<H>) const {
        constexpr int C = (16 + STEPS - 1) / STEPS;
        constexpr int CD = (32 + STEPS - 1) / STEPS;
        if constexpr (H == 0) {
            if constexpr (T > 0) relu_regs<S * C, C>(out[T - 1]);
            if constexpr (T == 0 && DEFER) relu_regs<S * CD, CD>(*deferred);
        } else {
            if constexpr (T + 1 < NT && S < 4) bias_quad<S>(out[T + 1], bias_half + 32 * (T + 1));
        }
    }
};

typedef volatile __attribute__((address_space(3))) uint32_t GateWord;
struct NoGate {
    __device__ __forceinline__ bool operator()(float) const { return false; }
};
template <bool GATE = false, class WS, class Hook5, class Hook6, class Dead = NoGate>
__device__ __forceinline__ bool f32_inference_pass(const float (&pe)[8][4], const float (&pd)[4][4], const float* bias_s, const float* bias_h,
                                                   WS& ws, FragReader& fr, Hook5&& after_open5, Hook6&& after_open6, float (&rgb)[3],
                                                   float& sigma, Dead&& dead = NoGate{}, GateWord* gate_mine = nullptr,
                                                   GateWord* gate_next = nullptr) {
    f32x16 A[8], B[8], V[5];
    auto pe_get = [&](auto G, auto J) { return pe[decltype(G)::value][decltype(J)::value]; };
    auto tiles_get = [](f32x16* arr) {
        return [arr](auto G, auto J) {
            constexpr int g = decltype(G)::value, j = decltype(J)::value;
            return arr[g >> 2][(g & 3) * 4 + j];
        };
    };
    auto layer = [&](auto F0c, auto NTc, auto KGc, auto DEFERc, auto& out, f32x16* deferred, auto&& bget, const float* bias_l) {
        constexpr int F0 = decltype(F0c)::value, NT = decltype(NTc)::value, KG = decltype(KGc)::value;
        constexpr bool LAST = (F0 + NT * KG == kUsedFrags) || F0 == layer_f0(8) || F0 == layer_f0(10);
        constexpr bool DEFER = decltype(DEFERc)::value != 0;
        static_assert(layer_f0(5) % kSliceFrags == 0 && layer_f0(6) % kSliceFrags == 0, "input prefetch hooks sit on slice boundaries");
        auto hook = [&]() {
            if constexpr (F0 == layer_f0(5)) after_open5();
            if constexpr (F0 == layer_f0(6)) after_open6();
        };
        bias_tile(out[0], bias_l);
        run_layer<F0, NT, KG, LAST, GATE && F0 == layer_f0(8)>(out, bget, ws, fr, LayerSide<NT, KG / 2, DEFER>{&out[0], deferred, bias_l}, hook);
    };
    layer(ic<layer_f0(0)>{}, ic<8>{}, ic<8>{}, ic<0>{}, A, nullptr, pe_get, bias_h + bias_off(0));
#pragma unroll 1
    for (int l = 1; l <= 3; l += 2) {
        layer(ic<layer_f0(1)>{}, ic<8>{}, ic<32>{}, ic<1>{}, B, &A[7], tiles_get(A), bias_h + l * 256);
        layer(ic<layer_f0(2)>{}, ic<8>{}, ic<32>{}, ic<1>{}, A, &B[7], tiles_get(B), bias_h + (l + 1) * 256);
    }
    layer(ic<layer_f0(5)>{}, ic<8>{}, ic<40>{}, ic<1>{}, B, &A[7],
          [&](auto G, auto J) {
              constexpr int g = decltype(G)::value, j = decltype(J)::value;
              if constexpr (g < 8) return pe[g][j];
              else return A[(g - 8) >> 2][((g - 8) & 3) * 4 + j];
          },
          bias_h + bias_off(5));
    layer(ic<layer_f0(6)>{}, ic<8>{}, ic<32>{}, ic<1>{}, A, &B[7], tiles_get(B), bias_h + bias_off(6));
    layer(ic<layer_f0(7)>{}, ic<8>{}, ic<32>{}, ic<1>{}, B, &A[7], tiles_get(A), bias_h + bias_off(7));
    f32x16(&V4a)[4] = reinterpret_cast<f32x16(&)[4]>(V);
    if constexpr (GATE) {
        static_assert(layer_f0(8) % kSliceFrags == 0 && (layer_f0(8) / kSliceFrags) % kRingSlots == 0 && kNumSlices % kRingSlots == 0,
                      "the gate decides where slot 0 opens: a skipped pass refills that slot with slice 0");
        relu_regs<0, 16>(B[7]);
        {
            float s0 = 0.f, s1 = 0.f, s2 = 0.f, s3 = 0.f;
            static_for<8>([&](auto T) {
                constexpr int t = decltype(T)::value;
                static_for<4>([&](auto Q) {
                    constexpr int q = decltype(Q)::value;
                    const f32x4 w = *reinterpret_cast<const f32x4*>(bias_h + kAlphaOff + 32 * t + 8 * q);
                    s0 = fmaf(w.x, B[t][4 * q + 0], s0);
                    s1 = fmaf(w.y, B[t][4 * q + 1], s1);
                    s2 = fmaf(w.z, B[t][4 * q + 2], s2);
                    s3 = fmaf(w.w, B[t][4 * q + 3], s3);
                });
            });
            const float part = (s0 + s1) + (s2 + s3);
            sigma = bias_s[bias_off(8) + kSigmaChannel] + (part + __shfl_xor(part, 32, 64));
        }
        const bool any_live = __builtin_amdgcn_ballot_w64(!dead(sigma)) != 0;
        if (any_live && (threadIdx.x & 63) == 0) *gate_mine = 1u;
        if (threadIdx.x == 0) *gate_next = 0u;
        asm volatile("s_waitcnt lgkmcnt(0)" ::: "memory");
        ws.open_slice();
        if (__builtin_amdgcn_readfirstlane(*gate_mine) == 0u) {
            rgb[0] = rgb[1] = rgb[2] = 0.0f;
            ws.next_slice = 0;
            ws.soff = 0;
            ws.template issue_rest<0, 0>();
            return true;
        }
    }
    layer(ic<layer_f0(8)>{}, ic<4>{}, ic<36>{}, ic<GATE ? 0 : 1>{}, V4a, GATE ? nullptr : &B[7],
          [&](auto G, auto J) {
              constexpr int g = decltype(G)::value, j = decltype(J)::value;
              if constexpr (g < 32) return B[g >> 2][(g & 3) * 4 + j];
              else return pd[g - 32][j];
          },
          bias_h + bias_off(8));
    relu_regs<0, 16>(V[3]);
    {
        constexpr int f_from = layer_f0(8) + 4 * 36, f_to = layer_f0(9);
        static_assert(f_from / kSliceFrags == (f_to - 1) / kSliceFrags && f_to % kSliceFrags != 0, "the walk stays inside one open slice");
        static_for<(f_to - f_from) / 2>([&](auto I) { ws.template step_piece<f_from + 2 * decltype(I)::value>(); });
        fr.pref0 = fr.template issue<f_to>();
        fr.pref1 = fr.template issue<f_to + 1>();
    }
    if constexpr (!GATE)
    {
        float s0 = 0.f, s1 = 0.f, s2 = 0.f, s3 = 0.f;
        static_for<8>([&](auto T) {
            constexpr int t = decltype(T)::value;
            static_for<4>([&](auto Q) {
                constexpr int q = decltype(Q)::value;
                const f32x4 w = *reinterpret_cast<const f32x4*>(bias_h + kAlphaOff + 32 * t + 8 * q);
                s0 = fmaf(w.x, B[t][4 * q + 0], s0);
                s1 = fmaf(w.y, B[t][4 * q + 1], s1);
                s2 = fmaf(w.z, B[t][4 * q + 2], s2);
                s3 = fmaf(w.w, B[t][4 * q + 3], s3);
            });
        });
        const float part = (s0 + s1) + (s2 + s3);
        sigma = bias_s[bias_off(8) + kSigmaChannel] + (part + __shfl_xor(part, 32, 64));
    }
    f32x16(&A4)[4] = reinterpret_cast<f32x16(&)[4]>(A);
    f32x16(&V4b)[4] = reinterpret_cast<f32x16(&)[4]>(V);
    layer(ic<layer_f0(9)>{}, ic<4>{}, ic<16>{}, ic<0>{}, A4, nullptr, tiles_get(V), bias_h + bias_off(9));
    layer(ic<layer_f0(10)>{}, ic<4>{}, ic<16>{}, ic<1>{}, V4b, &A[3], tiles_get(A), bias_h + bias_off(10));
    relu_regs<0, 16>(V[3]);
    finish_pass<layer_f0(11)>(ws);
    rgb[0] = bias_s[bias_off(11) + 0];
    rgb[1] = bias_s[bias_off(11) + 1];
    rgb[2] = bias_s[bias_off(11) + 2];
    {
        float part[3] = {0.f, 0.f, 0.f};
        static_for<4>([&](auto T) {
            constexpr int t = decltype(T)::value;
            f32x16 vt = V[t];
            asm volatile("" : "+v"(vt));
            static_for<3>([&](auto Cc) {
                constexpr int c = decltype(Cc)::value;
                static_for<4>([&](auto Q) {
                    constexpr int q = decltype(Q)::value;
                    const f32x4 w = *reinterpret_cast<const f32x4*>(bias_h + kRgbOff + 128 * c + 32 * t + 8 * q);
                    part[c] = fmaf(w.x, vt[4 * q + 0], part[c]);
                    part[c] = fmaf(w.y, vt[4 * q + 1], part[c]);
                    part[c] = fmaf(w.z, vt[4 * q + 2], part[c]);
                    part[c] = fmaf(w.w, vt[4 * q + 3], part[c]);
                });
            });
            asm volatile("" : "+v"(part[0]), "+v"(part[1]), "+v"(part[2])::"memory");
        });
        static_for<3>([&](auto Cc) {
            constexpr int c = decltype(Cc)::value;
            rgb[c] += part[c] + __shfl_xor(part[c], 32, 64);
        });
    }
    return false;
}

}
```

ideal-nerf_amd/ops.py:

```python
import contextlib
import ctypes as C
import os
from typing import Dict, Optional

import torch

from . import _lib
from ._lib import IDN_PREC_F32, RAY_FLOATS, IdealNerfError, check

PTS_CH, VIEWS_CH, W_HID = 63, 27, 256


def _ptr(t: Optional[torch.Tensor], name="tensor", dtype=torch.float32):
    if t is None:
        return None
    if not t.is_cuda:
        raise IdealNerfError(f"{name} must live on the GPU (got {t.device}); the HIP path has no CPU fallback")
    if t.dtype != dtype:
        raise IdealNerfError(f"{name} must be {dtype} (got {t.dtype})")
    if not t.is_contiguous():
        raise IdealNerfError(f"{name} must be contiguous")
    return t.data_ptr()


def _shape(t: Optional[torch.Tensor], name: str, *shape):
    if t is None:
        return
    got = tuple(t.shape)
    if len(got) != len(shape) or any(s is not None and int(s) != g for s, g in zip(shape, got)):
        want = "[" + ", ".join("*" if s is None else str(int(s)) for s in shape) + "]"
        raise IdealNerfError(f"{name} must be {want}, got {list(got)}")


class _Launch:

    def __init__(self, *tensors, device=None):
        devs = {t.device for t in tensors if t is not None and t.is_cuda}
        if device is not None:
            d = torch.device(device)
            if d.type != "cuda":
                raise IdealNerfError(f"the HIP path renders on the GPU (got device {device}); there is no CPU fallback")
            devs.add(torch.device("cuda", torch.cuda.current_device() if d.index is None else d.index))
        if len(devs) > 1:
            raise IdealNerfError("all tensors of one call must live on the same GPU, got " +
                                 ", ".join(sorted(str(d) for d in devs)))
        self.device = devs.pop() if devs else None
        self._ctx = contextlib.nullcontext()

    def __enter__(self):
        if self.device is not None:
            self._ctx = torch.cuda.device(self.device)
            self._ctx.__enter__()
            self.stream = torch.cuda.current_stream(self.device).cuda_stream
        else:
            self.stream = None
        return self

    def __exit__(self, *exc):
        return self._ctx.__exit__(*exc)


def _precision(precision):
    if precision not in (_lib.IDN_PREC_F32, _lib.IDN_PREC_BF16X3, _lib.IDN_PREC_BF16, _lib.IDN_PREC_FP16X3, _lib.IDN_PREC_BF16X6):
        raise IdealNerfError(f"unknown precision code {precision}")
    return int(precision)


def _net_buffers(lib, packed, folded, precision, which=""):
    if packed is not None:
        _shape(packed, f"packed{which}", lib.idealnerf_packed_weight_floats(_precision(precision)))
    if folded is not None:
        _shape(folded, f"folded{which}", lib.idealnerf_folded_bias_floats())


def params_struct(sd: Dict[str, torch.Tensor], dim_aud: int, dim_expr: int, dim_latent: int, prefix: str = ""):
    p = _lib.FaceNerfParams()
    C_all = PTS_CH + dim_aud + dim_expr + dim_latent

    def get(key, shape):
        t = sd[prefix + key]
        if tuple(t.shape) != shape:
            raise IdealNerfError(f"{key}: shape {tuple(t.shape)} != {shape} "
                                 "(only D=8, W=256, skips=[4], multires=10/4 is compiled)")
        return _ptr(t, key)

    for i in range(8):
        fan_in = C_all if i == 0 else (W_HID + C_all if i == 5 else W_HID)
        p.pts_w[i] = get(f"pts_linears.{i}.weight", (W_HID, fan_in))
        p.pts_b[i] = get(f"pts_linears.{i}.bias", (W_HID,))
    p.views_w[0] = get("views_linears.0.weight", (W_HID // 2, W_HID + VIEWS_CH + dim_expr))
    p.views_b[0] = get("views_linears.0.bias", (W_HID // 2,))
    for i in (1, 2):
        p.views_w[i] = get(f"views_linears.{i}.weight", (W_HID // 2, W_HID // 2))
        p.views_b[i] = get(f"views_linears.{i}.bias", (W_HID // 2,))
    p.alpha_w = get("alpha_linear.weight", (1, W_HID))
    p.alpha_b = get("alpha_linear.bias", (1,))
    p.rgb_w = get("rgb_linear.weight", (3, W_HID // 2))
    p.rgb_b = get("rgb_linear.bias", (3,))
    p.dim_aud, p.dim_expr, p.dim_latent = dim_aud, dim_expr, dim_latent
    return p


def pack_weights(p, device, precision=IDN_PREC_F32) -> torch.Tensor:
    lib = _lib.load()
    with _Launch(device=device) as L:
        out = torch.empty(lib.idealnerf_packed_weight_floats(_precision(precision)), dtype=torch.float32, device=L.device)
        check(lib.idealnerf_pack_weights(C.byref(p), precision, out.data_ptr(), L.stream))
    return out


def fold_conditioning(p, aud, expr, latent, device) -> torch.Tensor:
    lib = _lib.load()
    _shape(aud, "aud", p.dim_aud)
    _shape(expr, "expr", p.dim_expr)
    _shape(latent, "latent", p.dim_latent)
    if aud is None and p.dim_aud:
        raise IdealNerfError(f"aud is None but the network was built with dim_aud={p.dim_aud}")
    with _Launch(aud, expr, latent, device=device) as L:
        out = torch.empty(lib.idealnerf_folded_bias_floats(), dtype=torch.float32, device=L.device)
        check(lib.idealnerf_fold_conditioning(C.byref(p), _ptr(aud, "aud"), _ptr(expr, "expr"), _ptr(latent, "latent"),
                                              out.data_ptr(), L.stream))
    return out


def facenerf_fwd(packed, folded, x, precision=IDN_PREC_F32) -> torch.Tensor:
    lib = _lib.load()
    _shape(x, "x", None, PTS_CH + VIEWS_CH)
    _net_buffers(lib, packed, folded, precision)
    with _Launch(packed, folded, x) as L:
        out = torch.empty((x.shape[0], 4), dtype=torch.float32, device=x.device)
        check(lib.idealnerf_facenerf_fwd(_ptr(packed, "packed"), _ptr(folded, "folded"), precision, _ptr(x, "x"),
                                         x.shape[0], out.data_ptr(), L.stream))
    return out


def facenerf_train_fwd(packed, folded, x, precision=_lib.IDN_PREC_BF16X6):
    lib = _lib.load()
    _shape(x, "x", None, PTS_CH + VIEWS_CH)
    if precision not in (_lib.IDN_PREC_F32, _lib.IDN_PREC_BF16X6):
        raise IdealNerfError(f"the training forward runs IDN_PREC_F32 or IDN_PREC_BF16X6 only (got {precision})")
    _net_buffers(lib, packed, folded, precision)
    n = x.shape[0]
    with _Launch(packed, folded, x) as L:
        out = torch.empty((n, 4), dtype=torch.float32, device=x.device)
        acts = torch.empty(lib.idealnerf_train_acts_floats(n), dtype=torch.float32, device=x.device)
        check(lib.idealnerf_facenerf_train_fwd(_ptr(packed, "packed"), _ptr(folded, "folded"), precision, _ptr(x, "x"), n,
                                               out.data_ptr(), acts.data_ptr(), L.stream))
    return out, acts


def grads_struct(grads: Dict[str, torch.Tensor]):
    g = _lib.FaceNerfGrads()
    for i in range(8):
        g.pts_w[i] = grads[f"pts_linears.{i}.weight"].data_ptr()
        g.pts_b[i] = grads[f"pts_linears.{i}.bias"].data_ptr()
    for i in range(3):
        g.views_w[i] = grads[f"views_linears.{i}.weight"].data_ptr()
        g.views_b[i] = grads[f"views_linears.{i}.bias"].data_ptr()
    g.alpha_w, g.alpha_b = grads["alpha_linear.weight"].data_ptr(), grads["alpha_linear.bias"].data_ptr()
    g.rgb_w, g.rgb_b = grads["rgb_linear.weight"].data_ptr(), grads["rgb_linear.bias"].data_ptr()
    return g


def facenerf_bwd(p, grads, aud, expr, latent, acts, g_out, d_x=None, d_aud=None, d_expr=None, d_latent=None):
    lib = _lib.load()
    _shape(g_out, "g_out", None, 4)
    n = g_out.shape[0]
    _shape(acts, "acts", lib.idealnerf_train_acts_floats(n))
    _shape(d_x, "d_x", n, PTS_CH + VIEWS_CH)
    for t, name, dim in ((aud, "aud", p.dim_aud), (expr, "expr", p.dim_expr), (latent, "latent", p.dim_latent),
                         (d_aud, "d_aud", p.dim_aud), (d_expr, "d_expr", p.dim_expr), (d_latent, "d_latent", p.dim_latent)):
        _shape(t, name, dim)
    for k, t in grads.items():
        _ptr(t, f"grad {k}")
    with _Launch(aud, expr, latent, acts, g_out, d_x, d_aud, d_expr, d_latent, *grads.values()) as L:
        ptrs = [_ptr(t, name) for t, name in ((aud, "aud"), (expr, "expr"), (latent, "latent"), (acts, "acts"))]
        ptrs += [n, _ptr(g_out, "g_out")]
        ptrs += [_ptr(t, name) for t, name in ((d_x, "d_x"), (d_aud, "d_aud"), (d_expr, "d_expr"), (d_latent, "d_latent"))]
        ws = _workspace(lib.idealnerf_facenerf_bwd_workspace_bytes(n), g_out.device, L.stream)
        check(lib.idealnerf_facenerf_bwd(C.byref(p), C.byref(grads_struct(grads)), *ptrs, ws.data_ptr(), ws.numel(), L.stream))
    return grads


def query_rays_train_fwd(packed, folded, rays, z, precision=_lib.IDN_PREC_BF16X6):
    lib = _lib.load()
    _shape(z, "z", None, None)
    n, S = z.shape
    _shape(rays, "rays", n, RAY_FLOATS)
    with _Launch(packed, folded, rays, z) as L:
        raw = torch.empty((n, S, 4), dtype=torch.float32, device=z.device)
        acts = torch.empty(lib.idealnerf_train_acts_floats(n * S), dtype=torch.float32, device=z.device)
        check(lib.idealnerf_query_rays_train_fwd(_ptr(packed, "packed"), _ptr(folded, "folded"), precision, _ptr(rays, "rays"),
                                                 _ptr(z, "z"), n, S, raw.data_ptr(), acts.data_ptr(), L.stream))
    return raw, acts


def pass_bwd(p, grads, aud, expr, latent, acts, raw, z, rays, bc, g_rgb, g_fg, g_lw, g_acc, d_aud, d_latent):
    lib = _lib.load()
    n, S = z.shape
    for t, name, shape in ((raw, "raw", (n, S, 4)), (rays, "rays", (n, RAY_FLOATS)), (bc, "bc_rgb", (n, 3)),
                           (g_rgb, "g_rgb_map", (n, 3)), (g_fg, "g_rgb_fg", (n, 3)), (g_lw, "g_last_weight", (n,)),
                           (g_acc, "g_acc", (n,))):
        _shape(t, name, *shape)
    tensors = (aud, expr, latent, acts, raw, z, rays, bc, g_rgb, g_fg, g_lw, g_acc, d_aud, d_latent)
    with _Launch(*tensors, *grads.values()) as L:
        ws = _workspace(lib.idealnerf_pass_bwd_workspace_bytes(n, S), z.device, L.stream)
        ptrs = [_ptr(t) for t in tensors]
        check(lib.idealnerf_pass_bwd(C.byref(p), C.byref(grads_struct(grads)), *ptrs[:8], n, S, *ptrs[8:], ws.data_ptr(), ws.numel(), L.stream))
    return grads


def query_rays_fwd(packed, folded, rays, z, precision=IDN_PREC_F32) -> torch.Tensor:
    lib = _lib.load()
    _shape(z, "z", None, None)
    n, S = z.shape
    _shape(rays, "rays", n, RAY_FLOATS)
    _net_buffers(lib, packed, folded, precision)
    with _Launch(packed, folded, rays, z) as L:
        raw = torch.empty((n, S, 4), dtype=torch.float32, device=z.device)
        check(lib.idealnerf_query_rays_fwd(_ptr(packed, "packed"), _ptr(folded, "folded"), precision, _ptr(rays, "rays"),
                                           _ptr(z, "z"), n, S, raw.data_ptr(), L.stream))
    return raw


def query_points_fwd(packed, folded, pts, viewdirs, precision=IDN_PREC_F32) -> torch.Tensor:
    lib = _lib.load()
    _shape(pts, "pts", None, None, 3)
    n, S, _ = pts.shape
    _shape(viewdirs, "viewdirs", n, 3)
    _net_buffers(lib, packed, folded, precision)
    with _Launch(packed, folded, pts, viewdirs) as L:
        raw = torch.empty((n, S, 4), dtype=torch.float32, device=pts.device)
        check(lib.idealnerf_query_points_fwd(_ptr(packed, "packed"), _ptr(folded, "folded"), precision, _ptr(pts, "pts"),
                                             _ptr(viewdirs, "viewdirs"), n, S, raw.data_ptr(), L.stream))
    return raw


def frame_rays(c2w, H, W, focal, near, far, row0=0, nrows=None, cx=None, cy=None, device="cuda") -> torch.Tensor:
    lib = _lib.load()
    nrows = H - row0 if nrows is None else nrows
    if not (0 <= row0 and 0 <= nrows and row0 + nrows <= H and W > 0):
        raise IdealNerfError(f"rows [{row0}, {row0 + nrows}) are outside a {H}x{W} frame")
    if tuple(c2w.shape[-2:]) not in ((3, 4), (4, 4)) or c2w.dim() != 2:
        raise IdealNerfError(f"c2w must be [3, 4] or [4, 4], got {list(c2w.shape)}")
    m = (C.c_float * 12)(*[float(v) for v in c2w[:3, :4].reshape(-1).tolist()])
    with _Launch(device=device) as L:
        out = torch.empty((nrows * W, RAY_FLOATS), dtype=torch.float32, device=L.device)
        check(lib.idealnerf_frame_rays(m, H, W, float(focal), -1.0 if cx is None else float(cx),
                                       -1.0 if cy is None else float(cy), float(near), float(far), row0, nrows,
                                       out.data_ptr(), L.stream))
    return out


def to8b(rgb, swap_rb=False, nonfinite_flag=None) -> torch.Tensor:
    lib = _lib.load()
    if rgb.shape[-1] != 3:
        raise IdealNerfError(f"to8b expects [..., 3], got {tuple(rgb.shape)}")
    if nonfinite_flag is not None and (nonfinite_flag.dtype != torch.int32 or not nonfinite_flag.is_cuda
                                       or nonfinite_flag.numel() < 1):
        raise IdealNerfError("nonfinite_flag must be an int32 device tensor")
    with _Launch(rgb, nonfinite_flag) as L:
        out = torch.empty(rgb.shape, dtype=torch.uint8, device=rgb.device)
        check(lib.idealnerf_to8b(_ptr(rgb, "rgb"), rgb.numel() // 3, int(bool(swap_rb)), out.data_ptr(),
                                 nonfinite_flag.data_ptr() if nonfinite_flag is not None else None, L.stream))
    return out


def compose_to8b(rgb_head, last_weight, rgb_fg, swap_rb=False, nonfinite_flag=None, want_fg=False):
    lib = _lib.load()
    if rgb_head.shape[-1] != 3:
        raise IdealNerfError(f"compose_to8b expects rgb_head [..., 3], got {tuple(rgb_head.shape)}")
    _shape(rgb_fg, "rgb_fg", *rgb_head.shape)
    _shape(last_weight, "last_weight", *rgb_head.shape[:-1])
    if nonfinite_flag is not None and (nonfinite_flag.dtype != torch.int32 or not nonfinite_flag.is_cuda
                                       or nonfinite_flag.numel() < 1):
        raise IdealNerfError("nonfinite_flag must be an int32 device tensor")
    with _Launch(rgb_head, last_weight, rgb_fg, nonfinite_flag) as L:
        ptrs = (_ptr(rgb_head, "rgb_head"), _ptr(last_weight, "last_weight"), _ptr(rgb_fg, "rgb_fg"))
        out = torch.empty(rgb_head.shape, dtype=torch.uint8, device=rgb_head.device)
        fg_out = torch.empty_like(out) if want_fg else None
        check(lib.idealnerf_compose_to8b(*ptrs, rgb_head.numel() // 3, int(bool(swap_rb)), out.data_ptr(),
                                         fg_out.data_ptr() if want_fg else None,
                                         nonfinite_flag.data_ptr() if nonfinite_flag is not None else None, L.stream))
    return (out, fg_out) if want_fg else out


def coarse_depths(rays, t_vals, t_rand=None, lindisp=False) -> torch.Tensor:
    lib = _lib.load()
    _shape(rays, "rays", None, RAY_FLOATS)
    _shape(t_vals, "t_vals", None)
    n, S = rays.shape[0], t_vals.shape[0]
    _shape(t_rand, "t_rand", n, S)
    with _Launch(rays, t_vals, t_rand) as L:
        z = torch.empty((n, S), dtype=torch.float32, device=rays.device)
        check(lib.idealnerf_coarse_depths(_ptr(rays, "rays"), _ptr(t_vals, "t_vals"), _ptr(t_rand, "t_rand"),
                                          int(bool(lindisp)), n, S, z.data_ptr(), L.stream))
    return z


def composite_fwd(raw, z, rays, bc_rgb, with_fg=False, with_weights=True, sigma_noise=None,
                  white_bkgd=False) -> Dict[str, torch.Tensor]:
    lib = _lib.load()
    _shape(z, "z", None, None)
    n, S = z.shape
    _shape(raw, "raw", n, S, 4)
    _shape(rays, "rays", n, RAY_FLOATS)
    _shape(bc_rgb, "bc_rgb", n, 3)
    _shape(sigma_noise, "sigma_noise", n, S)
    dev = z.device
    with _Launch(raw, z, rays, bc_rgb, sigma_noise) as L:
        new = lambda *s: torch.empty(s, dtype=torch.float32, device=dev)
        o = dict(rgb_map=new(n, 3), disp_map=new(n), acc_map=new(n), depth_map=new(n), last_weight=new(n))
        if with_weights:
            o["weights"] = new(n, S)
        if with_fg:
            o["rgb_fg"] = new(n, 3)
        co = _lib.CompositeOut(**{k: v.data_ptr() for k, v in o.items()})
        check(lib.idealnerf_composite_fwd(_ptr(raw, "raw"), _ptr(z, "z"), _ptr(rays, "rays"), _ptr(bc_rgb, "bc_rgb"),
                                          _ptr(sigma_noise, "sigma_noise"), int(bool(white_bkgd)), n, S, C.byref(co), L.stream))
    return o


def _u_shape(u, n, n_importance=None):
    if u.dim() == 2:
        _shape(u, "u", n, n_importance)
        return 1
    _shape(u, "u", n_importance)
    return 0


def sample_pdf_fwd(z, weights, u, n_importance) -> Dict[str, torch.Tensor]:
    lib = _lib.load()
    _shape(z, "z", None, None)
    n, S = z.shape
    _shape(weights, "weights", n, S)
    per_ray = _u_shape(u, n, n_importance)
    dev = z.device
    with _Launch(z, weights, u) as L:
        o = dict(z_samples=torch.empty((n, n_importance), dtype=torch.float32, device=dev),
                 inds=torch.empty((n, n_importance), dtype=torch.int64, device=dev),
                 cdf=torch.empty((n, S - 1), dtype=torch.float32, device=dev),
                 z_fine=torch.empty((n, S + n_importance), dtype=torch.float32, device=dev),
                 z_std=torch.empty((n,), dtype=torch.float32, device=dev))
        check(lib.idealnerf_sample_pdf_fwd(_ptr(z, "z"), _ptr(weights, "weights"), _ptr(u, "u"), per_ray, n, S,
                                           n_importance, o["z_samples"].data_ptr(), o["inds"].data_ptr(),
                                           o["cdf"].data_ptr(), o["z_fine"].data_ptr(), o["z_std"].data_ptr(), L.stream))
    return o


def march_fwd(raw, z, rays, bc_rgb, u, n_importance, with_fg=False, with_weights=False, sigma_noise=None,
              white_bkgd=False) -> Dict[str, torch.Tensor]:
    lib = _lib.load()
    _shape(z, "z", None, None)
    n, S = z.shape
    _shape(raw, "raw", n, S, 4)
    _shape(rays, "rays", n, RAY_FLOATS)
    _shape(bc_rgb, "bc_rgb", n, 3)
    _shape(sigma_noise, "sigma_noise", n, S)
    per_ray = _u_shape(u, n, n_importance)
    dev = z.device
    with _Launch(raw, z, rays, bc_rgb, u, sigma_noise) as L:
        new = lambda *s: torch.empty(s, dtype=torch.float32, device=dev)
        o = dict(rgb_map=new(n, 3), disp_map=new(n), acc_map=new(n), depth_map=new(n), last_weight=new(n))
        if with_weights:
            o["weights"] = new(n, S)
        if with_fg:
            o["rgb_fg"] = new(n, 3)
        co = _lib.CompositeOut(**{k: v.data_ptr() for k, v in o.items()})
        o.update(z_samples=new(n, n_importance), inds=torch.empty((n, n_importance), dtype=torch.int64, device=dev),
                 cdf=new(n, S - 1), z_fine=new(n, S + n_importance), z_std=new(n))
        check(lib.idealnerf_march_fwd(_ptr(raw, "raw"), _ptr(z, "z"), _ptr(rays, "rays"), _ptr(bc_rgb, "bc_rgb"),
                                      _ptr(sigma_noise, "sigma_noise"), int(bool(white_bkgd)), _ptr(u, "u"), per_ray, n, S,
                                      n_importance, C.byref(co), o["z_samples"].data_ptr(), o["inds"].data_ptr(),
                                      o["cdf"].data_ptr(), o["z_fine"].data_ptr(), o["z_std"].data_ptr(), L.stream))
    return o


def sample_pdf_bins_fwd(bins, weights, u) -> Dict[str, torch.Tensor]:
    lib = _lib.load()
    _shape(bins, "bins", None, None)
    n, nb = bins.shape
    _shape(weights, "weights", n, nb - 1)
    per_ray = _u_shape(u, n)
    ni = u.shape[-1]
    dev = bins.device
    with _Launch(bins, weights, u) as L:
        o = dict(z_samples=torch.empty((n, ni), dtype=torch.float32, device=dev),
                 inds=torch.empty((n, ni), dtype=torch.int64, device=dev),
                 cdf=torch.empty((n, nb), dtype=torch.float32, device=dev))
        check(lib.idealnerf_sample_pdf_bins_fwd(_ptr(bins, "bins"), _ptr(weights, "weights"), _ptr(u, "u"), per_ray, n,
                                                nb, ni, o["z_samples"].data_ptr(), o["inds"].data_ptr(),
                                                o["cdf"].data_ptr(), L.stream))
    return o


def invert_cdf(cdf, bins, u):
    lib = _lib.load()
    _shape(cdf, "cdf", None, None)
    n, nb = cdf.shape
    _shape(bins, "bins", n, nb)
    per_ray = _u_shape(u, n)
    ni = u.shape[-1]
    with _Launch(cdf, bins, u) as L:
        zs = torch.empty((n, ni), dtype=torch.float32, device=cdf.device)
        inds = torch.empty((n, ni), dtype=torch.int64, device=cdf.device)
        check(lib.idealnerf_invert_cdf(_ptr(cdf, "cdf"), _ptr(bins, "bins"), _ptr(u, "u"), per_ray, n, nb, ni,
                                       zs.data_ptr(), inds.data_ptr(), L.stream))
    return zs, inds


def dw_gemm(delta, acts, pipe=0, with_bias=True):
    lib = _lib.load()
    _shape(delta, "delta", None, None)
    rows = delta.shape[0]
    _shape(acts, "acts", rows, None)
    with _Launch(delta, acts) as L:
        dW = torch.empty((256, 256), dtype=torch.float32, device=delta.device)
        db = torch.empty(256, dtype=torch.float32, device=delta.device) if with_bias else None
        nbytes = lib.idealnerf_dw_gemm_workspace_bytes()
        ws = _workspace(nbytes, delta.device, L.stream)
        check(lib.idealnerf_dw_gemm(_ptr(delta, "delta"), delta.shape[1], _ptr(acts, "acts"), acts.shape[1], rows, dW.data_ptr(),
                                    None if db is None else db.data_ptr(), int(pipe), ws.data_ptr(), ws.numel(), L.stream))
    return dW, db


AUDIO_NET_MAX_BWD_WINDOWS = 8


def _audio_params_struct(params, dim_aud):
    shapes = [(32, 29, 3), (32,), (32, 32, 3), (32,), (64, 32, 3), (64,), (64, 64, 3), (64,), (64, 64), (64,), (dim_aud, 64), (dim_aud,)]
    if len(params) != 12:
        raise IdealNerfError(f"AudioNet has 12 parameter tensors, got {len(params)}")
    for i, (t, shp) in enumerate(zip(params, shapes)):
        _shape(t, f"AudioNet parameter {i}", *shp)
    p = _lib.AudioNetParams()
    for i in range(4):
        p.conv_w[i], p.conv_b[i] = _ptr(params[2 * i], "conv weight"), _ptr(params[2 * i + 1], "conv bias")
    for i in range(2):
        p.fc_w[i], p.fc_b[i] = _ptr(params[8 + 2 * i], "fc weight"), _ptr(params[9 + 2 * i], "fc bias")
    p.dim_aud = int(dim_aud)
    return p


def audio_net_fwd(params, windows, dim_aud, save=False):
    lib = _lib.load()
    _shape(windows, "windows", None, 16, 29)
    n = windows.shape[0]
    with _Launch(windows, *params) as L:
        p = _audio_params_struct(params, dim_aud)
        out = torch.empty((n, dim_aud), dtype=torch.float32, device=windows.device)
        saved = torch.empty(lib.idealnerf_audio_net_saved_floats(n), dtype=torch.float32, device=windows.device) if save else None
        check(lib.idealnerf_audio_net_fwd(C.byref(p), _ptr(windows, "windows"), n, out.data_ptr(),
                                          None if saved is None else saved.data_ptr(), L.stream))
    return out, saved


def audio_net_bwd(params, windows, saved, d_out, dim_aud):
    lib = _lib.load()
    n = windows.shape[0]
    _shape(windows, "windows", None, 16, 29)
    _shape(d_out, "d_out", n, dim_aud)
    _shape(saved, "saved", lib.idealnerf_audio_net_saved_floats(n))
    with _Launch(windows, saved, d_out, *params) as L:
        p = _audio_params_struct(params, dim_aud)
        grads = [torch.empty_like(t) for t in params]
        g = _lib.AudioNetGrads()
        for i in range(4):
            g.conv_w[i], g.conv_b[i] = grads[2 * i].data_ptr(), grads[2 * i + 1].data_ptr()
        for i in range(2):
            g.fc_w[i], g.fc_b[i] = grads[8 + 2 * i].data_ptr(), grads[9 + 2 * i].data_ptr()
        check(lib.idealnerf_audio_net_bwd(C.byref(p), C.byref(g), _ptr(windows, "windows"), _ptr(saved, "saved"), _ptr(d_out, "d_out"),
                                          n, L.stream))
    return grads


SCORE_GROUPS = ("frame", "rect", "outside", "mouth", "torso")
SCORE_COLUMNS = ("n_pixels", "sse", "n_windows", "ssim_sum")
SCORE_TILE = _lib.SCORE_TILE


def frame_scores_workspace_doubles(H, W) -> int:
    return _lib.load().idealnerf_frame_scores_workspace_bytes(int(H), int(W)) // 8


def frame_scores(pred, truth_u8, regions=None, out=None, workspace=None) -> torch.Tensor:
    lib = _lib.load()
    if pred.dim() != 3 or pred.shape[-1] != 3:
        raise IdealNerfError(f"pred must be [H, W, 3], got {list(pred.shape)}")
    H, W = int(pred.shape[0]), int(pred.shape[1])
    _shape(truth_u8, "truth_u8", H, W, 3)
    _shape(regions, "regions", H, W)
    _shape(out, "out", 5, 4)
    with _Launch(pred, truth_u8, regions, out, workspace) as L:
        ptrs = (_ptr(pred, "pred"), _ptr(truth_u8, "truth_u8", torch.uint8), _ptr(regions, "regions", torch.uint8))
        need = lib.idealnerf_frame_scores_workspace_bytes(H, W)
        if out is None:
            out = torch.empty((5, 4), dtype=torch.float64, device=pred.device)
        if workspace is None:
            workspace = torch.empty(need // 8, dtype=torch.float64, device=pred.device)
        if workspace.numel() * 8 < need:
            raise IdealNerfError(f"workspace must hold {need // 8} float64 for a {H} x {W} frame, got {workspace.numel()}")
        check(lib.idealnerf_frame_scores(*ptrs, H, W, _ptr(out, "out", torch.float64), _ptr(workspace, "workspace", torch.float64),
                                         workspace.numel() * 8, L.stream))
    return out


def summarise_scores(table):
    import numpy as np
    t = np.asarray(table.detach().cpu() if isinstance(table, torch.Tensor) else table, dtype=np.float64)
    if t.ndim < 2 or t.shape[-2:] != (5, 4):
        raise ValueError(f"a score table is [..., 5, 4], got {list(t.shape)}")
    n_pix, sse, n_win, ssim_sum = (t[..., c] for c in range(4))
    with np.errstate(divide="ignore", invalid="ignore"):
        mse = np.where(n_pix > 0, sse / (3.0 * n_pix), np.nan)
        psnr = -10.0 * np.log10(mse)
        ssim = np.where(n_win > 0, ssim_sum / (3.0 * n_win), np.nan)
    return dict(mse=mse, psnr=psnr, ssim=ssim)


_workspaces: Dict[tuple, torch.Tensor] = {}


def _workspace(nbytes: int, device, stream) -> torch.Tensor:
    key = (str(device), int(stream))
    ws = _workspaces.get(key)
    if ws is None or ws.numel() < nbytes:
        ws = torch.zeros(nbytes, dtype=torch.uint8, device=device)
        _workspaces[key] = ws
    return ws


_FUSED_NAMES = {"0": 0, "1": 1, "2": 2, "split": 2}


def _fused_code(fused, where) -> int:
    if isinstance(fused, str) and fused.strip().lower() in _FUSED_NAMES:
        return _FUSED_NAMES[fused.strip().lower()]
    if isinstance(fused, (bool, int)) and int(fused) in (0, 1, 2):
        return int(fused)
    raise IdealNerfError(f"{where} must be one of 0 / False (kernel sequence), 1 / True (one fused kernel), 2 / 'split' "
                         f"(two fused kernels); got {fused!r}")


FUSED_MARCH_DEFAULT = _fused_code(os.environ.get("IDN_FUSED_MARCH", "0") or "0", "IDN_FUSED_MARCH")


COLOUR_GATE_DEFAULT = (os.environ.get("IDN_COLOUR_GATE", "1") or "1").strip() != "0"


def make_frame(c2w, H, W, focal, near, far, row0=0, nrows=None, cx=None, cy=None):
    nrows = H - row0 if nrows is None else nrows
    if not (0 <= row0 and 0 <= nrows and row0 + nrows <= H and W > 0):
        raise IdealNerfError(f"rows [{row0}, {row0 + nrows}) are outside a {H}x{W} frame")
    if c2w.dim() != 2 or tuple(c2w.shape[-2:]) not in ((3, 4), (4, 4)):
        raise IdealNerfError(f"c2w must be [3, 4] or [4, 4], got {list(c2w.shape)}")
    f = _lib.Frame()
    f.c2w = (C.c_float * 12)(*[float(v) for v in c2w[:3, :4].reshape(-1).tolist()])
    f.H, f.W, f.focal = int(H), int(W), float(focal)
    f.cx, f.cy = -1.0 if cx is None else float(cx), -1.0 if cy is None else float(cy)
    f.near_, f.far_, f.row0, f.nrows = float(near), float(far), int(row0), int(nrows)
    f.rays_out = None
    return f


def philox_uniform(seed, which, row0, n_rows, n_cols, device) -> torch.Tensor:
    lib = _lib.load()
    with _Launch(device=device) as L:
        out = torch.empty((int(n_rows), int(n_cols)), dtype=torch.float32, device=L.device)
        check(lib.idealnerf_philox_uniform(int(seed) & (2 ** 64 - 1), int(which), int(row0), int(n_rows), int(n_cols), _ptr(out, "out"), L.stream))
    return out


def sample_counts(n_rand, mouth_rays, torso_rays, sample_rate):
    sample_num = int(n_rand) - int(mouth_rays) - int(torso_rays)
    rect_num = int(sample_num * sample_rate)
    return rect_num, sample_num - rect_num, int(mouth_rays), int(torso_rays)


def camera_floats(c2w):
    if isinstance(c2w, C.Array):
        return c2w
    m = torch.as_tensor(c2w, dtype=torch.float32).detach().cpu()
    if m.dim() != 2 or tuple(m.shape) not in ((3, 4), (4, 4)):
        raise IdealNerfError(f"c2w must be [3, 4] or [4, 4], got {list(m.shape)}")
    return (C.c_float * 12)(*[float(v) for v in m[:3, :4].reshape(-1).tolist()])


def sample_pixels(region_map, counts, seed, draw, out=None, workspace=None) -> torch.Tensor:
    lib = _lib.load()
    if region_map.dim() != 2:
        raise IdealNerfError(f"region_map must be [H, W], got {list(region_map.shape)}")
    counts = [int(c) for c in counts]
    if len(counts) != 4 or min(counts) < 0:
        raise IdealNerfError(f"counts must be four non-negative numbers (rect, outside, mouth, torso), got {counts}")
    if max(counts) > _lib.SAMPLE_MAX_REGION:
        raise IdealNerfError(f"a region count of {max(counts)} exceeds the sampler's {_lib.SAMPLE_MAX_REGION} picks per region")
    H, W = region_map.shape
    n = sum(counts)
    _shape(out, "out", n)
    with _Launch(region_map, out, workspace) as L:
        mp = _ptr(region_map, "region_map", torch.uint8)
        if out is None:
            out = torch.empty(n, dtype=torch.int64, device=region_map.device)
        if workspace is None:
            workspace = torch.empty(4, dtype=torch.int32, device=region_map.device)
        if workspace.numel() < 4:
            raise IdealNerfError("workspace must hold four int32")
        check(lib.idealnerf_sample_pixels(mp, H, W, *counts, int(seed) & (2 ** 64 - 1), int(draw) & (2 ** 64 - 1),
                                          _ptr(workspace, "workspace", torch.int32), workspace.numel() * 4,
                                          _ptr(out, "out", torch.int64), L.stream))
    return out


_byte_tables: Dict[str, tuple] = {}


def byte_tables(device):
    import numpy as np
    device = torch.device(device)
    if device.type == "cuda" and device.index is None:
        device = torch.device("cuda", torch.cuda.current_device())
    key = str(device)
    t = _byte_tables.get(key)
    if t is None:
        target = torch.arange(256, dtype=torch.int32).to(torch.uint8).to(device).float() / 255.0
        background = torch.tensor(np.arange(256, dtype=np.uint8) / 255.0).to(device).to(torch.float32)
        t = _byte_tables[key] = (target.contiguous(), background.contiguous())
    return t


def gather_rays(sel, c2w, H, W, focal, image, background, cx=None, cy=None):
    lib = _lib.load()
    _shape(sel, "sel", None)
    _shape(image, "image", H, W, 3)
    _shape(background, "background", H, W, 3)
    n = sel.shape[0]
    m = camera_floats(c2w)
    with _Launch(sel, image, background) as L:
        tt, tb = byte_tables(L.device)
        batch_rays = torch.empty((2, n, 3), dtype=torch.float32, device=sel.device)
        target_s = torch.empty((n, 3), dtype=torch.float32, device=sel.device)
        bc_rgb = torch.empty((n, 3), dtype=torch.float32, device=sel.device)
        check(lib.idealnerf_gather_rays(_ptr(sel, "sel", torch.int64), n, m, int(H), int(W), float(focal),
                                        -1.0 if cx is None else float(cx), -1.0 if cy is None else float(cy),
                                        _ptr(image, "image", torch.uint8), _ptr(background, "background", torch.uint8),
                                        _ptr(tt, "target table"), _ptr(tb, "background table"),
                                        batch_rays.data_ptr(), target_s.data_ptr(), bc_rgb.data_ptr(), L.stream))
    return batch_rays, target_s, bc_rgb


def render_rays_fwd(rays, bc_rgb, packed_c, folded_c, packed_f, folded_f, t_vals, u, n_importance,
                    t_rand=None, with_fg=False, taps=False, precision=IDN_PREC_F32, precision_fine=None, lindisp=False,
                    white_bkgd=False, noise_coarse=None, noise_fine=None, fused=None, frame=None, draws=None,
                    colour_gate=None, gate_counters=None) -> Dict[str, torch.Tensor]:
    lib = _lib.load()
    if gate_counters is not None:
        _shape(gate_counters, "gate_counters", 2, 2)
    if draws is not None and (u is not None or t_rand is not None):
        raise IdealNerfError("draws=(seed, ray0) replaces BOTH t_rand and u: pass them as None")
    _shape(t_vals, "t_vals", None)
    if frame is not None:
        if rays is not None:
            raise IdealNerfError("frame mode derives the rays from the camera: pass rays=None")
        n = frame.nrows * frame.W
    else:
        _shape(rays, "rays", None, RAY_FLOATS)
        n = rays.shape[0]
    S, Ni = t_vals.shape[0], int(n_importance)
    _shape(bc_rgb, "bc_rgb", n, 3)
    _shape(t_rand, "t_rand", n, S)
    _shape(noise_coarse, "noise_coarse", n, S)
    _shape(noise_fine, "noise_fine", n, S + Ni)
    _net_buffers(lib, packed_c, folded_c, precision, "_coarse")
    if Ni > 0:
        if (u is None and draws is None) or packed_f is None or folded_f is None:
            raise IdealNerfError("n_importance > 0 needs u (or draws=) and the fine network's packed / folded buffers")
        if u is not None:
            _u_shape(u, n, Ni)
        _net_buffers(lib, packed_f, folded_f, precision if precision_fine is None else precision_fine, "_fine")
    dev = bc_rgb.device
    with _Launch(rays, bc_rgb, packed_c, folded_c, packed_f, folded_f, t_vals, u, t_rand, noise_coarse, noise_fine, gate_counters) as L:
        new = lambda *s: torch.empty(s, dtype=torch.float32, device=dev)
        opts = _lib.RenderOpts()
        opts.colour_gate = int(COLOUR_GATE_DEFAULT if colour_gate is None else bool(colour_gate))
        opts.gate_counters = _ptr(gate_counters, "gate_counters", torch.int64)
        out = dict(rgb_map=new(n, 3), disp_map=new(n), acc_map=new(n))
        if Ni > 0:
            out.update(rgb0=new(n, 3), disp0=new(n), acc0=new(n), z_std=new(n), last_weight=new(n))
        if with_fg:
            out["rgb_fg"] = new(n, 3)
            if Ni > 0:
                out.update(rgb_fg0=new(n, 3), last_weight0=new(n))
        if taps:
            out.update(tap_z_coarse=new(n, S), tap_raw_coarse=new(n, S, 4), tap_weights_coarse=new(n, S))
            if Ni > 0:
                out.update(tap_cdf=new(n, S - 1), tap_inds=torch.empty((n, Ni), dtype=torch.int64, device=dev),
                           tap_z_samples=new(n, Ni), tap_z_fine=new(n, S + Ni), tap_raw_fine=new(n, S + Ni, 4),
                           tap_weights_fine=new(n, S + Ni))
        a = _lib.RenderArgs()
        a.rays, a.bc_rgb, a.n_rays = _ptr(rays, "rays"), _ptr(bc_rgb, "bc_rgb"), n
        a.n_samples, a.n_importance, a.precision = S, Ni, _precision(precision)
        a.precision_fine_plus1 = 0 if precision_fine is None else _precision(precision_fine) + 1
        a.packed_coarse, a.folded_coarse = _ptr(packed_c, "packed_coarse"), _ptr(folded_c, "folded_coarse")
        a.packed_fine, a.folded_fine = _ptr(packed_f, "packed_fine"), _ptr(folded_f, "folded_fine")
        a.t_vals, a.t_rand = _ptr(t_vals, "t_vals"), _ptr(t_rand, "t_rand")
        a.u = _ptr(u, "u") if u is not None else None
        a.u_per_ray = 1 if (u is not None and u.dim() == 2) else 0
        a.lindisp, a.white_bkgd = int(bool(lindisp)), int(bool(white_bkgd))
        a.noise_coarse, a.noise_fine = _ptr(noise_coarse, "noise_coarse"), _ptr(noise_fine, "noise_fine")
        if draws is not None:
            a.rng_mode, a.rng_seed, a.rng_ray0 = 1, int(draws[0]) & (2 ** 64 - 1), int(draws[1])
        if fused is None:
            applies = (S == 64 and Ni == 128 and noise_coarse is None and noise_fine is None and
                       _precision(precision) == IDN_PREC_F32 and (precision_fine is None or _precision(precision_fine) == IDN_PREC_F32))
            fused = FUSED_MARCH_DEFAULT if applies else 0
        a.fused_march = _fused_code(fused, "render_rays_fwd(fused=)")
        for k, v in out.items():
            setattr(a, k, v.data_ptr())
        if frame is None:
            nbytes = lib.idealnerf_render_workspace_bytes(n, S, Ni)
            ws = _workspace(nbytes, dev, L.stream or 0)
            a.workspace, a.workspace_bytes = ws.data_ptr(), ws.numel()
            check(lib.idealnerf_render_rays_fwd_opts(C.byref(a), C.byref(opts), L.stream))
        else:
            tap_rays = new(n, RAY_FLOATS) if taps else None
            frame.rays_out = None if tap_rays is None else tap_rays.data_ptr()
            nbytes = lib.idealnerf_render_frame_workspace_bytes(n, S, Ni)
            ws = _workspace(nbytes, dev, L.stream or 0)
            a.workspace, a.workspace_bytes = ws.data_ptr(), ws.numel()
            check(lib.idealnerf_render_frame_fwd_opts(C.byref(a), C.byref(frame), C.byref(opts), L.stream))
            frame.rays_out = None
            if tap_rays is not None:
                out["tap_rays"] = tap_rays
    return out
```

include/idealnerf.h:

```cpp
#ifndef IDEALNERF_H
#define IDEALNERF_H

#include <stddef.h>
#include <stdint.h>

#ifdef __cplusplus
extern "C" {
#endif

#define IDN_OK 0
#define IDN_EINVAL (-1)
#define IDN_EUNSUPPORTED (-2)
#define IDN_EHIP (-3)
#define IDN_EWORKSPACE (-4)

#define IDN_W 256
#define IDN_D 8
#define IDN_PTS_CH 63
#define IDN_VIEWS_CH 27
#define IDN_RAY_FLOATS 11

#define IDN_PREC_F32 0
#define IDN_PREC_BF16X3 1
#define IDN_PREC_BF16 2
#define IDN_PREC_FP16X3 3
#define IDN_PREC_BF16X6 4

int idealnerf_version(void);
const char* idealnerf_last_error(void);

size_t idealnerf_packed_weight_floats(int precision);
size_t idealnerf_folded_bias_floats(void);

typedef struct idn_facenerf_params {
    const float* pts_w[8];
    const float* pts_b[8];
    const float* views_w[3];
    const float* views_b[3];
    const float* alpha_w;
    const float* alpha_b;
    const float* rgb_w;
    const float* rgb_b;
    int dim_aud, dim_expr, dim_latent;
} idn_facenerf_params;

int idealnerf_pack_weights(const idn_facenerf_params* p, int precision, float* packed, void* stream);

int idealnerf_fold_conditioning(const idn_facenerf_params* p, const float* aud, const float* expr,
                                const float* latent, float* folded, void* stream);

int idealnerf_facenerf_fwd(const float* packed, const float* folded, int precision, const float* x,
                           int64_t n, float* out, void* stream);

int idealnerf_query_rays_fwd(const float* packed, const float* folded, int precision, const float* rays,
                             const float* z, int64_t n_rays, int n_samples, float* raw, void* stream);

int idealnerf_query_points_fwd(const float* packed, const float* folded, int precision, const float* pts,
                               const float* viewdirs, int64_t n_rays, int n_samples, float* raw, void* stream);

int idealnerf_frame_rays(const float* c2w, int H, int W, float focal, float cx, float cy, float near_, float far_,
                         int row0, int nrows, float* rays_out, void* stream);

int idealnerf_coarse_depths(const float* rays, const float* t_vals, const float* t_rand, int lindisp, int64_t n_rays,
                            int n_samples, float* z, void* stream);

typedef struct idn_composite_out {
    float* rgb_map;
    float* disp_map;
    float* acc_map;
    float* depth_map;
    float* weights;
    float* rgb_fg;
    float* last_weight;
} idn_composite_out;

int idealnerf_composite_fwd(const float* raw, const float* z, const float* rays, const float* bc_rgb,
                            const float* sigma_noise, int white_bkgd, int64_t n_rays, int n_samples,
                            const idn_composite_out* out, void* stream);

int idealnerf_sample_pdf_fwd(const float* z, const float* weights, const float* u, int u_per_ray,
                             int64_t n_rays, int n_samples, int n_importance, float* z_samples, int64_t* inds,
                             float* cdf, float* z_fine, float* z_std, void* stream);

int idealnerf_march_fwd(const float* raw, const float* z, const float* rays, const float* bc_rgb, const float* sigma_noise,
                        int white_bkgd, const float* u, int u_per_ray, int64_t n_rays, int n_samples, int n_importance,
                        const idn_composite_out* out, float* z_samples, int64_t* inds, float* cdf, float* z_fine,
                        float* z_std, void* stream);

int idealnerf_sample_pdf_bins_fwd(const float* bins, const float* weights, const float* u, int u_per_ray,
                                  int64_t n_rays, int n_bins, int n_importance, float* z_samples, int64_t* inds,
                                  float* cdf, void* stream);

int idealnerf_invert_cdf(const float* cdf, const float* bins, const float* u, int u_per_ray, int64_t n_rays,
                         int n_bins, int n_importance, float* z_samples, int64_t* inds, void* stream);

typedef struct idn_render_args {
    const float* rays;
    const float* bc_rgb;
    int64_t n_rays;
    int n_samples;
    int n_importance;
    int precision;
    const float* packed_coarse;
    const float* folded_coarse;
    const float* packed_fine;
    const float* folded_fine;
    const float* t_vals;
    const float* t_rand;
    const float* u;
    int u_per_ray;
    float* rgb_map;  float* disp_map;  float* acc_map;  float* depth_map;  float* last_weight;  float* rgb_fg;
    float* rgb0;     float* disp0;     float* acc0;     float* z_std;      float* last_weight0; float* rgb_fg0;
    float* tap_z_coarse;
    float* tap_raw_coarse;
    float* tap_weights_coarse;
    float* tap_cdf;
    int64_t* tap_inds;
    float* tap_z_samples;
    float* tap_z_fine;
    float* tap_raw_fine;
    float* tap_weights_fine;
    void* workspace;
    size_t workspace_bytes;
    int precision_fine_plus1;
    int lindisp;
    int white_bkgd;
    const float* noise_coarse;
    const float* noise_fine;
    int fused_march;
    int rng_mode;
    uint64_t rng_seed;
    int64_t rng_ray0;
} idn_render_args;

int idealnerf_philox_uniform(uint64_t seed, int which, int64_t row0, int64_t n_rows, int n_cols, float* out, void* stream);

#define IDN_SAMPLE_MAX_REGION 4096
size_t idealnerf_sample_pixels_workspace_bytes(void);
int idealnerf_sample_pixels(const uint8_t* region_map, int H, int W, int n_rect, int n_outside, int n_mouth, int n_torso,
                            uint64_t seed, uint64_t draw, void* workspace, size_t workspace_bytes, int64_t* sel, void* stream);

int idealnerf_gather_rays(const int64_t* sel, int64_t n, const float* c2w, int H, int W, float focal, float cx, float cy,
                          const uint8_t* image, const uint8_t* background, const float* target_table, const float* background_table,
                          float* batch_rays, float* target_s, float* bc_rgb, void* stream);

#define IDN_SCORE_TILE 32
size_t idealnerf_frame_scores_workspace_bytes(int H, int W);
int idealnerf_frame_scores(const float* pred, const uint8_t* truth, const uint8_t* regions, int H, int W, double* out,
                           void* workspace, size_t workspace_bytes, void* stream);

size_t idealnerf_render_workspace_bytes(int64_t n_rays, int n_samples, int n_importance);
int idealnerf_render_rays_fwd(const idn_render_args* a, void* stream);

typedef struct idn_frame {
    float c2w[12];
    int H, W;
    float focal, cx, cy;
    float near_, far_;
    int row0, nrows;
    float* rays_out;
} idn_frame;
size_t idealnerf_render_frame_workspace_bytes(int64_t n_rays, int n_samples, int n_importance);
int idealnerf_render_frame_fwd(const idn_render_args* a, const idn_frame* frame, void* stream);

typedef struct idn_render_opts {
    int colour_gate;
    int64_t* gate_counters;
} idn_render_opts;
int idealnerf_render_rays_fwd_opts(const idn_render_args* a, const idn_render_opts* opts, void* stream);
int idealnerf_render_frame_fwd_opts(const idn_render_args* a, const idn_frame* frame, const idn_render_opts* opts, void* stream);
float idealnerf_colour_gate_max_dist(void);


size_t idealnerf_train_acts_floats(int64_t n_points);

int idealnerf_query_rays_train_fwd(const float* packed, const float* folded, int precision, const float* rays,
                                   const float* z, int64_t n_rays, int n_samples, float* raw, float* acts,
                                   void* stream);

typedef struct idn_facenerf_grads {
    float* pts_w[8];
    float* pts_b[8];
    float* views_w[3];
    float* views_b[3];
    float* alpha_w;
    float* alpha_b;
    float* rgb_w;
    float* rgb_b;
} idn_facenerf_grads;

size_t idealnerf_pass_bwd_workspace_bytes(int64_t n_rays, int n_samples);

int idealnerf_pass_bwd(const idn_facenerf_params* p, const idn_facenerf_grads* grads, const float* aud,
                       const float* expr, const float* latent, const float* acts, const float* raw, const float* z,
                       const float* rays, const float* bc_rgb, int64_t n_rays, int n_samples, const float* g_rgb_map,
                       const float* g_rgb_fg, const float* g_last_weight, const float* g_acc, float* d_aud,
                       float* d_latent, void* workspace, size_t workspace_bytes, void* stream);

int idealnerf_facenerf_train_fwd(const float* packed, const float* folded, int precision, const float* x, int64_t n,
                                 float* out, float* acts, void* stream);

size_t idealnerf_facenerf_bwd_workspace_bytes(int64_t n);

int idealnerf_facenerf_bwd(const idn_facenerf_params* p, const idn_facenerf_grads* grads, const float* aud, const float* expr,
                           const float* latent, const float* acts, int64_t n, const float* g_out, float* d_x, float* d_aud,
                           float* d_expr, float* d_latent, void* workspace, size_t workspace_bytes, void* stream);

#define IDN_DW_PIPE_BF16X6 0
#define IDN_DW_PIPE_F32 1
#define IDN_DW_PIPE_BF16X6_PASS 2
size_t idealnerf_dw_gemm_workspace_bytes(void);
int idealnerf_dw_gemm(const float* delta, int ld_delta, const float* acts, int ld_acts, int64_t rows, float* dW, float* db,
                      int pipe, void* workspace, size_t workspace_bytes, void* stream);

typedef struct idn_audio_net_params {
    const float* conv_w[4];
    const float* conv_b[4];
    const float* fc_w[2];
    const float* fc_b[2];
    int dim_aud;
} idn_audio_net_params;
typedef struct idn_audio_net_grads {
    float* conv_w[4];
    float* conv_b[4];
    float* fc_w[2];
    float* fc_b[2];
} idn_audio_net_grads;
size_t idealnerf_audio_net_saved_floats(int n_windows);
int idealnerf_audio_net_fwd(const idn_audio_net_params* p, const float* windows, int n_windows, float* out, float* saved,
                            void* stream);
int idealnerf_audio_net_bwd(const idn_audio_net_params* p, const idn_audio_net_grads* grads, const float* windows,
                            const float* saved, const float* d_out, int n_windows, void* stream);

int idealnerf_to8b(const float* rgb, int64_t n_pixels, int swap_rb, uint8_t* out, int* nonfinite_flag, void* stream);

int idealnerf_compose_to8b(const float* rgb_head, const float* last_weight, const float* rgb_fg, int64_t n_pixels,
                           int swap_rb, uint8_t* out, uint8_t* fg_out, int* nonfinite_flag, void* stream);

void idealnerf_profile_begin(void);
int idealnerf_profile_end(double* total_ms, int64_t* launches, int64_t* points);

#define IDN_PROF_MLP_FWD 0
#define IDN_PROF_MLP_FWD_SAVE 1
#define IDN_PROF_DELTA_CHAIN 2
#define IDN_PROF_DW_GEMM 3
#define IDN_PROF_DW_GEMM_X6 4
#define IDN_PROF_MLP_FWD_SAVE_X6 5
#define IDN_PROF_DELTA_CHAIN_X6 6
#define IDN_PROF_KINDS 7
int idealnerf_profile_end_kinds(double* total_ms, int64_t* launches, int64_t* points);

#ifdef __cplusplus
}
#endif
#endif
```

Measured before the change: 131.0 million.

## Skip MFMA work for all-zero post-ReLU activation tiles in gated MLP

Adds a zero-skip mode to the colour-gated f32 MLP kernel. During each ReLU it records a wave-wide ballot bit per register row that is nonzero, and the next layer uses these bits to skip MFMA issues for input fragments that are entirely zero across the wave. It is on by default, with optional counters and new opts2 entry points. The exact-zero skip keeps results identical but adds scalar bookkeeping and branches in the inner layer loop, and the saving depends on how sparse the activations are.

```diff
diff --git a/ideal-nerf_amd/_lib.py b/ideal-nerf_amd/_lib.py
--- a/ideal-nerf_amd/_lib.py
+++ b/ideal-nerf_amd/_lib.py
@@ -59,6 +59,10 @@
     _fields_ = [("colour_gate", C.c_int), ("gate_counters", fp)]
 
 
+class RenderOpts2(C.Structure):
+    _fields_ = [("colour_gate", C.c_int), ("zero_skip", C.c_int), ("gate_counters", fp), ("skip_counters", fp)]
+
+
 ABI_VERSION = 4
 
 PROTOTYPES = {
@@ -97,6 +101,9 @@
     "idealnerf_render_rays_fwd_opts": (C.c_int, [C.POINTER(RenderArgs), C.POINTER(RenderOpts), fp]),
     "idealnerf_render_frame_fwd_opts": (C.c_int, [C.POINTER(RenderArgs), C.POINTER(Frame), C.POINTER(RenderOpts), fp]),
     "idealnerf_colour_gate_max_dist": (C.c_float, []),
+    "idealnerf_render_rays_fwd_opts2": (C.c_int, [C.POINTER(RenderArgs), C.POINTER(RenderOpts2), fp]),
+    "idealnerf_render_frame_fwd_opts2": (C.c_int, [C.POINTER(RenderArgs), C.POINTER(Frame), C.POINTER(RenderOpts2), fp]),
+    "idealnerf_zero_skip_default": (C.c_int, []),
     "idealnerf_audio_net_saved_floats": (C.c_size_t, [C.c_int]),
     "idealnerf_audio_net_fwd": (C.c_int, [C.POINTER(AudioNetParams), fp, C.c_int, fp, fp, fp]),
     "idealnerf_audio_net_bwd": (C.c_int, [C.POINTER(AudioNetParams), C.POINTER(AudioNetGrads), fp, fp, fp, C.c_int, fp]),
diff --git a/ideal-nerf_amd/csrc/capi.hip b/ideal-nerf_amd/csrc/capi.hip
--- a/ideal-nerf_amd/csrc/capi.hip
+++ b/ideal-nerf_amd/csrc/capi.hip
@@ -27,7 +27,7 @@
 
 int launch_mlp(int precision, const float* packed, const float* folded, const float* x, const float* rays,
                const float* z, const float* pts, const float* dirs, int64_t n_points, int n_samples, float* raw,
-               hipStream_t s, int gate, int64_t* gate_counters) {
+               hipStream_t s, int gate, int64_t* gate_counters, int skip, int64_t* skip_counters) {
     if (n_points > 0x7fffffffLL) return fail(IDN_EUNSUPPORTED, "n_points %lld exceeds 2^31-1 per launch", (long long)n_points);
     if ((rays || pts) && n_samples < 1) return fail(IDN_EINVAL, "n_samples < 1");
     if (precision == IDN_PREC_BF16X3)
@@ -38,7 +38,7 @@
         return launch_mlp_fp16x3(packed, folded, x, rays, z, pts, dirs, n_points, n_samples, raw, s);
     if (precision == IDN_PREC_BF16X6)
         return launch_mlp_bf16x6(packed, folded, x, rays, z, pts, dirs, n_points, n_samples, raw, s);
-    return launch_mlp_f32(packed, folded, x, rays, z, pts, dirs, n_points, n_samples, raw, s, nullptr, 0, gate, gate_counters);
+    return launch_mlp_f32(packed, folded, x, rays, z, pts, dirs, n_points, n_samples, raw, s, nullptr, 0, gate, gate_counters, skip, skip_counters);
 }
 
 static int check_params(const idn_facenerf_params* p) {
@@ -451,10 +451,23 @@
     return carve(nullptr, n_rays, n_samples, n_importance).bytes;
 }
 
-static int render_impl(const idn_render_args* a, const idn_frame* frame, const idn_render_opts* opts, void* stream_);
-int idealnerf_render_rays_fwd(const idn_render_args* a, void* stream_) { return render_impl(a, nullptr, nullptr, stream_); }
-int idealnerf_render_rays_fwd_opts(const idn_render_args* a, const idn_render_opts* opts, void* stream_) { return render_impl(a, nullptr, opts, stream_); }
+static int render_impl(const idn_render_args* a, const idn_frame* frame, const idn_render_opts2* opts, void* stream_);
+static idn_render_opts2 opts2_of(const idn_render_opts* o) {
+    idn_render_opts2 r = {1, kZeroSkipDefault, nullptr, nullptr};
+    if (o) {
+        r.colour_gate = o->colour_gate;
+        r.gate_counters = o->gate_counters;
+    }
+    return r;
+}
+int idealnerf_render_rays_fwd(const idn_render_args* a, void* stream_) { return idealnerf_render_rays_fwd_opts2(a, nullptr, stream_); }
+int idealnerf_render_rays_fwd_opts(const idn_render_args* a, const idn_render_opts* opts, void* stream_) {
+    const idn_render_opts2 o2 = opts2_of(opts);
+    return idealnerf_render_rays_fwd_opts2(a, &o2, stream_);
+}
+int idealnerf_render_rays_fwd_opts2(const idn_render_args* a, const idn_render_opts2* opts, void* stream_) { return render_impl(a, nullptr, opts, stream_); }
 float idealnerf_colour_gate_max_dist(void) { return kGateMaxDist; }
+int idealnerf_zero_skip_default(void) { return kZeroSkipDefault; }
 
 static size_t frame_scratch_bytes(int64_t n_rays) {
     const int64_t c = n_rays < kRenderChunk ? n_rays : kRenderChunk;
@@ -464,8 +477,12 @@
     const size_t base = idealnerf_render_workspace_bytes(n_rays, n_samples, n_importance);
     return base ? base + frame_scratch_bytes(n_rays) : 0;
 }
-int idealnerf_render_frame_fwd(const idn_render_args* a, const idn_frame* f, void* stream_) { return idealnerf_render_frame_fwd_opts(a, f, nullptr, stream_); }
+int idealnerf_render_frame_fwd(const idn_render_args* a, const idn_frame* f, void* stream_) { return idealnerf_render_frame_fwd_opts2(a, f, nullptr, stream_); }
 int idealnerf_render_frame_fwd_opts(const idn_render_args* a, const idn_frame* f, const idn_render_opts* opts, void* stream_) {
+    const idn_render_opts2 o2 = opts2_of(opts);
+    return idealnerf_render_frame_fwd_opts2(a, f, &o2, stream_);
+}
+int idealnerf_render_frame_fwd_opts2(const idn_render_args* a, const idn_frame* f, const idn_render_opts2* opts, void* stream_) {
     if (!a || !f) return fail(IDN_EINVAL, "args / frame is NULL");
     if (a->rays) return fail(IDN_EINVAL, "frame mode derives the rays from the camera: args->rays must be NULL");
     if (f->H <= 0 || f->W <= 0 || f->row0 < 0 || f->nrows < 0 || f->row0 + f->nrows > f->H) return fail(IDN_EINVAL, "bad frame / rows");
@@ -473,8 +490,9 @@
     return render_impl(a, f, opts, stream_);
 }
 
-static int render_impl(const idn_render_args* a, const idn_frame* frame, const idn_render_opts* opts, void* stream_) {
+static int render_impl(const idn_render_args* a, const idn_frame* frame, const idn_render_opts2* opts, void* stream_) {
     if (!a) return fail(IDN_EINVAL, "args is NULL");
+    if (opts && opts->zero_skip != 0 && opts->zero_skip != 1) return fail(IDN_EINVAL, "zero_skip %d (1 = on, 0 = off)", opts->zero_skip);
     if (opts && opts->colour_gate != 0 && opts->colour_gate != 1) return fail(IDN_EINVAL, "colour_gate %d (1 = on, the default; 0 = off)", opts->colour_gate);
     if (int e = check_precision(a->precision)) return e;
     const int prec_fine = a->precision_fine_plus1 ? a->precision_fine_plus1 - 1 : a->precision;
@@ -505,6 +523,8 @@
     const int gate_c = gate_on && a->precision == IDN_PREC_F32 && !a->noise_coarse && !a->tap_raw_coarse;
     const int gate_f = gate_on && prec_fine == IDN_PREC_F32 && !a->noise_fine && !a->tap_raw_fine;
     int64_t* const gate_counters = opts ? opts->gate_counters : nullptr;
+    const int skip = opts ? opts->zero_skip : kZeroSkipDefault;
+    int64_t* const skip_counters = opts ? opts->skip_counters : nullptr;
     hipStream_t st = (hipStream_t)stream_;
     const RenderWs w = carve(reinterpret_cast<char*>(a->workspace), n, S, Ni);
 
@@ -530,7 +550,7 @@
         const Draws draws{(unsigned long long)a->rng_seed, (long)(a->rng_ray0 + r0), a->rng_mode};
         if (int e = launch_coarse_depths(rays, a->t_vals, off(a->t_rand, r0 * S), c, S, a->lindisp, w.z_c, st, draws)) return e;
         if (!a->fused_march)
-            if (int e = launch_mlp(a->precision, a->packed_coarse, a->folded_coarse, nullptr, rays, w.z_c, nullptr, nullptr, c * S, S, w.raw_c, st, gate_c, gate_counters)) return e;
+            if (int e = launch_mlp(a->precision, a->packed_coarse, a->folded_coarse, nullptr, rays, w.z_c, nullptr, nullptr, c * S, S, w.raw_c, st, gate_c, gate_counters, gate_c && skip, skip_counters)) return e;
         idn_composite_out co = {};
         const bool fine = Ni > 0;
         co.rgb_map = off(fine ? a->rgb0 : a->rgb_map, r0 * 3);
@@ -573,7 +593,7 @@
                                  w.z_f, off(a->z_std, r0), st, draws))
             return e;
         if (int e = launch_mlp(prec_fine, a->packed_fine, a->folded_fine, nullptr, rays, w.z_f, nullptr, nullptr, c * Sf, Sf, w.raw_f, st, gate_f,
-                                 gate_counters ? gate_counters + 2 : nullptr)) return e;
+                                 gate_counters ? gate_counters + 2 : nullptr, gate_f && skip, skip_counters ? skip_counters + 2 : nullptr)) return e;
         idn_composite_out fo = {};
         fo.rgb_map = off(a->rgb_map, r0 * 3);
         fo.disp_map = off(a->disp_map, r0);
diff --git a/ideal-nerf_amd/csrc/idn_internal.h b/ideal-nerf_amd/csrc/idn_internal.h
--- a/ideal-nerf_amd/csrc/idn_internal.h
+++ b/ideal-nerf_amd/csrc/idn_internal.h
@@ -63,6 +63,7 @@
 constexpr int kSigmaChannel = 128;
 
 constexpr float kGateMaxDist = 0.0125f;
+constexpr int kZeroSkipDefault = 1;
 
 enum { kActX0 = 0, kActDir = 1, kActA1 = 2, kActV1 = 10, kActCount = 13 };
 constexpr int act_width(int i) { return i < 2 ? 64 : (i < kActV1 ? 256 : 128); }
@@ -130,12 +131,13 @@
                       const float* pts, const float* dirs, int64_t n_points, int n_samples, float* raw, hipStream_t s);
 int launch_mlp(int precision, const float* packed, const float* folded, const float* x, const float* rays,
                const float* z, const float* pts, const float* dirs, int64_t n_points, int n_samples, float* raw,
-               hipStream_t s, int gate = 0, int64_t* gate_counters = nullptr);
+               hipStream_t s, int gate = 0, int64_t* gate_counters = nullptr, int skip = 0, int64_t* skip_counters = nullptr);
 int launch_fold(const idn_facenerf_params& p, const float* aud, const float* expr, const float* latent,
                 float* folded, hipStream_t s);
 int launch_mlp_f32(const float* packed, const float* folded, const float* x, const float* rays, const float* z,
                    const float* pts, const float* dirs, int64_t n_points, int n_samples, float* raw, hipStream_t s,
-                   float* acts = nullptr, int64_t p_pad = 0, int gate = 0, int64_t* gate_counters = nullptr);
+                   float* acts = nullptr, int64_t p_pad = 0, int gate = 0, int64_t* gate_counters = nullptr, int skip = 0,
+                   int64_t* skip_counters = nullptr);
 
 int launch_frame_rays(const float* c2w, int H, int W, float focal, float cx, float cy, float near_, float far_,
                       int row0, int nrows, float* rays_out, hipStream_t s);
diff --git a/ideal-nerf_amd/csrc/mlp_common.h b/ideal-nerf_amd/csrc/mlp_common.h
--- a/ideal-nerf_amd/csrc/mlp_common.h
+++ b/ideal-nerf_amd/csrc/mlp_common.h
@@ -167,6 +167,30 @@
         constexpr int r = R0 + decltype(R)::value;
         if constexpr (r < 16) tile[r] = relu1(tile[r]);
     });
+}
+template <int B>
+__device__ __forceinline__ void record_bit(uint32_t& word, unsigned long long some) {
+    uint32_t t;
+    asm volatile("s_cmp_lg_u64 %2, 0\n\ts_cselect_b32 %0, %3, 0\n\ts_or_b32 %1, %1, %0" : "=&s"(t), "+s"(word) : "s"(some), "n"((int)(1u << B)) : "scc");
+}
+template <int R0, int CNT, int SH>
+__device__ __forceinline__ void relu_regs_bits(f32x16& tile, uint32_t& word) {
+    if constexpr (R0 == 0) word &= ~(0xffffu << SH);
+    static_for<CNT>([&](auto R) {
+        constexpr int r = R0 + decltype(R)::value;
+        if constexpr (r < 16) {
+            const float x = tile[r];
+            const unsigned long long some = __builtin_amdgcn_ballot_w64(__builtin_bit_cast(int, x) > 0);
+            tile[r] = relu1(x);
+            record_bit<SH + r>(word, some);
+        }
+    });
+}
+template <int B>
+__device__ __forceinline__ bool mask_bit(uint32_t word) {
+    uint32_t t;
+    asm volatile("s_and_b32 %0, %1, %2" : "=s"(t) : "s"(word), "n"((int)(1u << B)) : "scc");
+    return t != 0u;
 }
 template <int NT>
 __device__ __forceinline__ void relu_tiles(f32x16 (&t)[NT]) {
@@ -269,6 +293,7 @@
 };
 struct MlpGateArgs : MlpArgs {
     unsigned long long* gate_counters;
+    unsigned long long* skip_counters;
 };
 
 struct PointIn {
diff --git a/ideal-nerf_amd/csrc/mlp_f32.hip b/ideal-nerf_amd/csrc/mlp_f32.hip
--- a/ideal-nerf_amd/csrc/mlp_f32.hip
+++ b/ideal-nerf_amd/csrc/mlp_f32.hip
@@ -69,9 +69,10 @@
     }
 };
 
-template <int MODE, bool SAVE, bool GATE = false>
+template <int MODE, bool SAVE, bool GATE = false, bool SKIP = false>
 __global__ __launch_bounds__(256, 1) void mlp_f32_kernel(std::conditional_t<GATE, MlpGateArgs, MlpArgs> a) {
     static_assert(!GATE || (MODE == kModeRays && !SAVE), "the colour gate is built for the rays-mode inference pass");
+    static_assert(!SKIP || GATE, "zero skip is built into the colour-gated kernel");
     extern __shared__ __attribute__((aligned(16))) char smem[];
     char* ring = smem;
     float* bias_s = reinterpret_cast<float*>(smem + kRingFrags * kFragBytes);
@@ -163,15 +164,24 @@
 
         float rgb[3], sigma;
         if constexpr (GATE) {
-            const bool skipped = f32_inference_pass<true>(
+            uint32_t skip_count[2] = {0u, 0u};
+            const bool skipped = f32_inference_pass<true, SKIP>(
                 pe, pd, bias_s, bias_h, ws, fr,
                 [&]() { load_point<MODE>(a, tile + gridDim.x, wave, m, nxt); load_gate_point(a, tile + gridDim.x, wave, m, nxt); },
                 [&]() { touch_point(nxt); touch_gate_point(nxt); }, rgb, sigma,
-                [&](float sg) { return !valid || gate_point_dead(cur, sg); }, gate_words + gate_par, gate_words + (gate_par ^ 1));
+                [&](float sg) { return !valid || gate_point_dead(cur, sg); }, gate_words + gate_par, gate_words + (gate_par ^ 1), skip_count);
             gate_par ^= 1;
             if (a.gate_counters && tid == 0) {
                 atomicAdd(a.gate_counters + 0, 1ull);
                 if (skipped) atomicAdd(a.gate_counters + 1, 1ull);
+            }
+            if constexpr (SKIP) {
+                if (a.skip_counters) {
+                    if (lane == 0) {
+                        atomicAdd(a.skip_counters + 0, (unsigned long long)skip_count[0]);
+                        atomicAdd(a.skip_counters + 1, (unsigned long long)skip_count[1]);
+                    }
+                }
             }
         } else if constexpr (!SAVE) {
             f32_inference_pass(pe, pd, bias_s, bias_h, ws, fr,
@@ -317,7 +327,7 @@
 
 int launch_mlp_f32(const float* packed, const float* folded, const float* x, const float* rays, const float* z,
                    const float* pts, const float* dirs, int64_t n_points, int n_samples, float* raw, hipStream_t s,
-                   float* acts, int64_t p_pad, int gate, int64_t* gate_counters) {
+                   float* acts, int64_t p_pad, int gate, int64_t* gate_counters, int skip, int64_t* skip_counters) {
     if (n_points <= 0) return IDN_OK;
     static LaunchSetup setup;
     int num_cu = 0;
@@ -325,6 +335,8 @@
             IDN_HIP_CHECK(hipFuncSetAttribute(reinterpret_cast<const void*>(&mlp_f32_kernel<kModeRays, false>),
                                               hipFuncAttributeMaxDynamicSharedMemorySize, kMlpLds));
             IDN_HIP_CHECK(hipFuncSetAttribute(reinterpret_cast<const void*>(&mlp_f32_kernel<kModeRays, false, true>),
+                                              hipFuncAttributeMaxDynamicSharedMemorySize, kMlpLdsGate));
+            IDN_HIP_CHECK(hipFuncSetAttribute(reinterpret_cast<const void*>(&mlp_f32_kernel<kModeRays, false, true, true>),
                                               hipFuncAttributeMaxDynamicSharedMemorySize, kMlpLdsGate));
             IDN_HIP_CHECK(hipFuncSetAttribute(reinterpret_cast<const void*>(&mlp_f32_kernel<kModeX, false>),
                                               hipFuncAttributeMaxDynamicSharedMemorySize, kMlpLds));
@@ -340,6 +352,7 @@
     const int64_t ntiles = (n_points + 127) / 128;
     const int grid = (int)(ntiles < num_cu ? ntiles : num_cu);
     if (gate && (acts || x || pts)) return fail(IDN_EUNSUPPORTED, "the colour gate is built for the rays-mode inference launch");
+    if (skip && !gate) return fail(IDN_EUNSUPPORTED, "zero skip is built into the colour-gated launch");
     MlpArgs a{packed, folded, x, rays, z, pts, dirs, (long)n_points, n_samples, raw, acts, (long)p_pad};
     ProfScope prof(s, n_points, acts ? IDN_PROF_MLP_FWD_SAVE : IDN_PROF_MLP_FWD);
     if (acts) {
@@ -356,7 +369,11 @@
         MlpGateArgs ga;
         static_cast<MlpArgs&>(ga) = a;
         ga.gate_counters = reinterpret_cast<unsigned long long*>(gate_counters);
-        hipLaunchKernelGGL((mlp_f32_kernel<kModeRays, false, true>), dim3(grid), dim3(256), kMlpLdsGate, s, ga);
+        ga.skip_counters = skip ? reinterpret_cast<unsigned long long*>(skip_counters) : nullptr;
+        if (skip)
+            hipLaunchKernelGGL((mlp_f32_kernel<kModeRays, false, true, true>), dim3(grid), dim3(256), kMlpLdsGate, s, ga);
+        else
+            hipLaunchKernelGGL((mlp_f32_kernel<kModeRays, false, true>), dim3(grid), dim3(256), kMlpLdsGate, s, ga);
     }
     else
         hipLaunchKernelGGL((mlp_f32_kernel<kModeRays, false>), dim3(grid), dim3(256), kMlpLds, s, a);
diff --git a/ideal-nerf_amd/csrc/mlp_f32_layers.h b/ideal-nerf_amd/csrc/mlp_f32_layers.h
--- a/ideal-nerf_amd/csrc/mlp_f32_layers.h
+++ b/ideal-nerf_amd/csrc/mlp_f32_layers.h
@@ -1,5 +1,6 @@
 #pragma once
 #include "mlp_common.h"
+#include <type_traits>
 
 namespace idn {
 
@@ -7,9 +8,30 @@
     return __builtin_amdgcn_mfma_f32_32x32x2f32(a, b, c, 0, 0, 0);
 }
 
-template <int F0, int NT, int KG, bool LAST = false, bool OPENED = false, class BGet, class Side, class Hook = NoHook, class WS = WStream>
+struct NoSkip {
+    template <int G, int J>
+    __device__ __forceinline__ constexpr bool operator()(ic<G>, ic<J>) const { return true; }
+};
+template <int G0, int G1>
+struct SkipBits {
+    static constexpr int kRegs = 4 * (G1 - G0);
+    const uint32_t* mask;
+    template <int G, int J>
+    __device__ __forceinline__ bool operator()(ic<G>, ic<J>) const {
+        if constexpr (G < G0 || G >= G1) return true;
+        else return mask_bit<(4 * (G - G0) + J) & 31>(mask[(4 * (G - G0) + J) >> 5]);
+    }
+    __device__ __forceinline__ uint32_t on_count() const {
+        uint32_t n = 0;
+        static_for<kRegs / 32>([&](auto W) { n += (uint32_t)__builtin_popcount(mask[decltype(W)::value]); });
+        return n;
+    }
+};
+
+template <int F0, int NT, int KG, bool LAST = false, bool OPENED = false, class BGet, class Side, class Hook = NoHook, class WS = WStream,
+          class On = NoSkip>
 __device__ __forceinline__ void run_layer(f32x16 (&out)[NT], BGet&& bget, WS& ws, FragReader& fr, Side&& side,
-                                          Hook&& after_open = NoHook{}) {
+                                          Hook&& after_open = NoHook{}, On on = NoSkip{}) {
     constexpr int STEPS = KG / 2, NP = NT * STEPS;
     static_assert(KG % 2 == 0 && F0 % 2 == 0, "fragments are consumed in pairs");
     static_assert(!OPENED || F0 % kSliceFrags == 0, "only a layer that starts a slice can find it opened");
@@ -34,15 +56,15 @@
             FragReader::retire<0>(a0, a1);
         }
         ws.template step_piece<f>();
-        out[t] = mfma(a0.x, bget(ic<g0>{}, ic<0>{}), out[t]);
-        out[t] = mfma(a0.y, bget(ic<g0>{}, ic<1>{}), out[t]);
-        out[t] = mfma(a0.z, bget(ic<g0>{}, ic<2>{}), out[t]);
-        out[t] = mfma(a0.w, bget(ic<g0>{}, ic<3>{}), out[t]);
+        if (on(ic<g0>{}, ic<0>{})) out[t] = mfma(a0.x, bget(ic<g0>{}, ic<0>{}), out[t]);
+        if (on(ic<g0>{}, ic<1>{})) out[t] = mfma(a0.y, bget(ic<g0>{}, ic<1>{}), out[t]);
+        if (on(ic<g0>{}, ic<2>{})) out[t] = mfma(a0.z, bget(ic<g0>{}, ic<2>{}), out[t]);
+        if (on(ic<g0>{}, ic<3>{})) out[t] = mfma(a0.w, bget(ic<g0>{}, ic<3>{}), out[t]);
         side(ic<t>{}, ic<s>{}, ic<0>{});
-        out[t] = mfma(a1.x, bget(ic<g1>{}, ic<0>{}), out[t]);
-        out[t] = mfma(a1.y, bget(ic<g1>{}, ic<1>{}), out[t]);
-        out[t] = mfma(a1.z, bget(ic<g1>{}, ic<2>{}), out[t]);
-        out[t] = mfma(a1.w, bget(ic<g1>{}, ic<3>{}), out[t]);
+        if (on(ic<g1>{}, ic<0>{})) out[t] = mfma(a1.x, bget(ic<g1>{}, ic<0>{}), out[t]);
+        if (on(ic<g1>{}, ic<1>{})) out[t] = mfma(a1.y, bget(ic<g1>{}, ic<1>{}), out[t]);
+        if (on(ic<g1>{}, ic<2>{})) out[t] = mfma(a1.z, bget(ic<g1>{}, ic<2>{}), out[t]);
+        if (on(ic<g1>{}, ic<3>{})) out[t] = mfma(a1.w, bget(ic<g1>{}, ic<3>{}), out[t]);
         side(ic<t>{}, ic<s>{}, ic<1>{});
         __builtin_amdgcn_sched_barrier(0);
         if constexpr (next_crosses && pi + 1 < NP) {
@@ -57,18 +79,25 @@
     fr.pref1 = a1;
 }
 
-template <int NT, int STEPS, bool DEFER>
+template <int NT, int STEPS, bool DEFER, bool SKIP = false>
 struct LayerSide {
     f32x16* out;
     f32x16* deferred;
     const float* bias_half;
+    uint32_t* mask_out = nullptr;
+    uint32_t* mask_def = nullptr;
     template <int T, int S, int H>
     __device__ __forceinline__ void operator()(ic<T>, ic<S>, ic<H>) const {
         constexpr int C = (16 + STEPS - 1) / STEPS;
         constexpr int CD = (32 + STEPS - 1) / STEPS;
         if constexpr (H == 0) {
-            if constexpr (T > 0) relu_regs<S * C, C>(out[T - 1]);
-            if constexpr (T == 0 && DEFER) relu_regs<S * CD, CD>(*deferred);
+            if constexpr (SKIP) {
+                if constexpr (T > 0) relu_regs_bits<S * C, C, 16 * ((T - 1) & 1)>(out[T - 1], mask_out[(T - 1) >> 1]);
+                if constexpr (T == 0 && DEFER) relu_regs_bits<S * CD, CD, 16>(*deferred, *mask_def);
+            } else {
+                if constexpr (T > 0) relu_regs<S * C, C>(out[T - 1]);
+                if constexpr (T == 0 && DEFER) relu_regs<S * CD, CD>(*deferred);
+            }
         } else {
             if constexpr (T + 1 < NT && S < 4) bias_quad<S>(out[T + 1], bias_half + 32 * (T + 1));
         }
@@ -79,12 +108,18 @@
 struct NoGate {
     __device__ __forceinline__ bool operator()(float) const { return false; }
 };
-template <bool GATE = false, class WS, class Hook5, class Hook6, class Dead = NoGate>
+template <int L>
+constexpr int kBiasOffOf = bias_off(L);
+#define IDN_BIAS_OFF(L) (SKIP ? kBiasOffOf<L> : bias_off(L))
+template <bool GATE = false, bool SKIP = false, class WS, class Hook5, class Hook6, class Dead = NoGate>
 __device__ __forceinline__ bool f32_inference_pass(const float (&pe)[8][4], const float (&pd)[4][4], const float* bias_s, const float* bias_h,
                                                    WS& ws, FragReader& fr, Hook5&& after_open5, Hook6&& after_open6, float (&rgb)[3],
                                                    float& sigma, Dead&& dead = NoGate{}, GateWord* gate_mine = nullptr,
-                                                   GateWord* gate_next = nullptr) {
+                                                   GateWord* gate_next = nullptr, uint32_t* skip_count = nullptr) {
+    static_assert(!SKIP || GATE, "zero skip is built into the colour-gated pass");
     f32x16 A[8], B[8], V[5];
+    uint32_t mA[4] = {0u, 0u, 0u, 0u}, mB[4] = {0u, 0u, 0u, 0u}, mV[2] = {0u, 0u};
+    uint32_t n_eligible = 0, n_skipped = 0;
     auto pe_get = [&](auto G, auto J) { return pe[decltype(G)::value][decltype(J)::value]; };
     auto tiles_get = [](f32x16* arr) {
         return [arr](auto G, auto J) {
@@ -92,7 +127,8 @@
             return arr[g >> 2][(g & 3) * 4 + j];
         };
     };
-    auto layer = [&](auto F0c, auto NTc, auto KGc, auto DEFERc, auto& out, f32x16* deferred, auto&& bget, const float* bias_l) {
+    auto layer = [&](auto F0c, auto NTc, auto KGc, auto DEFERc, auto& out, f32x16* deferred, auto&& bget, const float* bias_l, auto on,
+                     uint32_t* mask_out, uint32_t* mask_def) {
         constexpr int F0 = decltype(F0c)::value, NT = decltype(NTc)::value, KG = decltype(KGc)::value;
         constexpr bool LAST = (F0 + NT * KG == kUsedFrags) || F0 == layer_f0(8) || F0 == layer_f0(10);
         constexpr bool DEFER = decltype(DEFERc)::value != 0;
@@ -102,13 +138,30 @@
             if constexpr (F0 == layer_f0(6)) after_open6();
         };
         bias_tile(out[0], bias_l);
-        run_layer<F0, NT, KG, LAST, GATE && F0 == layer_f0(8)>(out, bget, ws, fr, LayerSide<NT, KG / 2, DEFER>{&out[0], deferred, bias_l}, hook);
+        if constexpr (SKIP) {
+            run_layer<F0, NT, KG, LAST, GATE && F0 == layer_f0(8)>(out, bget, ws, fr,
+                                                                   LayerSide<NT, KG / 2, DEFER, true>{&out[0], deferred, bias_l, mask_out, mask_def}, hook, on);
+            if constexpr (!std::is_same_v<decltype(on), NoSkip>) {
+                n_eligible += NT * on.kRegs;
+                n_skipped += NT * (on.kRegs - on.on_count());
+            }
+        } else {
+            run_layer<F0, NT, KG, LAST, GATE && F0 == layer_f0(8)>(out, bget, ws, fr, LayerSide<NT, KG / 2, DEFER>{&out[0], deferred, bias_l}, hook);
+        }
     };
-    layer(ic<layer_f0(0)>{}, ic<8>{}, ic<8>{}, ic<0>{}, A, nullptr, pe_get, bias_h + bias_off(0));
+    auto flush_counts = [&]() {
+        if constexpr (SKIP) {
+            if (skip_count) {
+                skip_count[0] += n_eligible;
+                skip_count[1] += n_skipped;
+            }
+        }
+    };
+    layer(ic<layer_f0(0)>{}, ic<8>{}, ic<8>{}, ic<0>{}, A, nullptr, pe_get, bias_h + IDN_BIAS_OFF(0), NoSkip{}, mA, nullptr);
 #pragma unroll 1
     for (int l = 1; l <= 3; l += 2) {
-        layer(ic<layer_f0(1)>{}, ic<8>{}, ic<32>{}, ic<1>{}, B, &A[7], tiles_get(A), bias_h + l * 256);
-        layer(ic<layer_f0(2)>{}, ic<8>{}, ic<32>{}, ic<1>{}, A, &B[7], tiles_get(B), bias_h + (l + 1) * 256);
+        layer(ic<layer_f0(1)>{}, ic<8>{}, ic<32>{}, ic<1>{}, B, &A[7], tiles_get(A), bias_h + l * 256, SkipBits<0, 32>{mA}, mB, &mA[3]);
+        layer(ic<layer_f0(2)>{}, ic<8>{}, ic<32>{}, ic<1>{}, A, &B[7], tiles_get(B), bias_h + (l + 1) * 256, SkipBits<0, 32>{mB}, mA, &mB[3]);
     }
     layer(ic<layer_f0(5)>{}, ic<8>{}, ic<40>{}, ic<1>{}, B, &A[7],
           [&](auto G, auto J) {
@@ -116,14 +169,15 @@
               if constexpr (g < 8) return pe[g][j];
               else return A[(g - 8) >> 2][((g - 8) & 3) * 4 + j];
           },
-          bias_h + bias_off(5));
-    layer(ic<layer_f0(6)>{}, ic<8>{}, ic<32>{}, ic<1>{}, A, &B[7], tiles_get(B), bias_h + bias_off(6));
-    layer(ic<layer_f0(7)>{}, ic<8>{}, ic<32>{}, ic<1>{}, B, &A[7], tiles_get(A), bias_h + bias_off(7));
+          bias_h + IDN_BIAS_OFF(5), SkipBits<8, 40>{mA}, mB, &mA[3]);
+    layer(ic<layer_f0(6)>{}, ic<8>{}, ic<32>{}, ic<1>{}, A, &B[7], tiles_get(B), bias_h + IDN_BIAS_OFF(6), SkipBits<0, 32>{mB}, mA, &mB[3]);
+    layer(ic<layer_f0(7)>{}, ic<8>{}, ic<32>{}, ic<1>{}, B, &A[7], tiles_get(A), bias_h + IDN_BIAS_OFF(7), SkipBits<0, 32>{mA}, mB, &mA[3]);
     f32x16(&V4a)[4] = reinterpret_cast<f32x16(&)[4]>(V);
     if constexpr (GATE) {
         static_assert(layer_f0(8) % kSliceFrags == 0 && (layer_f0(8) / kSliceFrags) % kRingSlots == 0 && kNumSlices % kRingSlots == 0,
                       "the gate decides where slot 0 opens: a skipped pass refills that slot with slice 0");
-        relu_regs<0, 16>(B[7]);
+        if constexpr (SKIP) relu_regs_bits<0, 16, 16>(B[7], mB[3]);
+        else relu_regs<0, 16>(B[7]);
         {
             float s0 = 0.f, s1 = 0.f, s2 = 0.f, s3 = 0.f;
             static_for<8>([&](auto T) {
@@ -138,7 +192,7 @@
                 });
             });
             const float part = (s0 + s1) + (s2 + s3);
-            sigma = bias_s[bias_off(8) + kSigmaChannel] + (part + __shfl_xor(part, 32, 64));
+            sigma = bias_s[IDN_BIAS_OFF(8) + kSigmaChannel] + (part + __shfl_xor(part, 32, 64));
         }
         const bool any_live = __builtin_amdgcn_ballot_w64(!dead(sigma)) != 0;
         if (any_live && (threadIdx.x & 63) == 0) *gate_mine = 1u;
@@ -150,6 +204,7 @@
             ws.next_slice = 0;
             ws.soff = 0;
             ws.template issue_rest<0, 0>();
+            flush_counts();
             return true;
         }
     }
@@ -159,8 +214,9 @@
               if constexpr (g < 32) return B[g >> 2][(g & 3) * 4 + j];
               else return pd[g - 32][j];
           },
-          bias_h + bias_off(8));
-    relu_regs<0, 16>(V[3]);
+          bias_h + IDN_BIAS_OFF(8), SkipBits<0, 32>{mB}, mV, nullptr);
+    if constexpr (SKIP) relu_regs_bits<0, 16, 16>(V[3], mV[1]);
+    else relu_regs<0, 16>(V[3]);
     {
         constexpr int f_from = layer_f0(8) + 4 * 36, f_to = layer_f0(9);
         static_assert(f_from / kSliceFrags == (f_to - 1) / kSliceFrags && f_to % kSliceFrags != 0, "the walk stays inside one open slice");
@@ -183,17 +239,18 @@
             });
         });
         const float part = (s0 + s1) + (s2 + s3);
-        sigma = bias_s[bias_off(8) + kSigmaChannel] + (part + __shfl_xor(part, 32, 64));
+        sigma = bias_s[IDN_BIAS_OFF(8) + kSigmaChannel] + (part + __shfl_xor(part, 32, 64));
     }
     f32x16(&A4)[4] = reinterpret_cast<f32x16(&)[4]>(A);
     f32x16(&V4b)[4] = reinterpret_cast<f32x16(&)[4]>(V);
-    layer(ic<layer_f0(9)>{}, ic<4>{}, ic<16>{}, ic<0>{}, A4, nullptr, tiles_get(V), bias_h + bias_off(9));
-    layer(ic<layer_f0(10)>{}, ic<4>{}, ic<16>{}, ic<1>{}, V4b, &A[3], tiles_get(A), bias_h + bias_off(10));
+    layer(ic<layer_f0(9)>{}, ic<4>{}, ic<16>{}, ic<0>{}, A4, nullptr, tiles_get(V), bias_h + IDN_BIAS_OFF(9), SkipBits<0, 16>{mV}, mA, nullptr);
+    layer(ic<layer_f0(10)>{}, ic<4>{}, ic<16>{}, ic<1>{}, V4b, &A[3], tiles_get(A), bias_h + IDN_BIAS_OFF(10), SkipBits<0, 16>{mA}, mV, &mA[1]);
+    flush_counts();
     relu_regs<0, 16>(V[3]);
     finish_pass<layer_f0(11)>(ws);
-    rgb[0] = bias_s[bias_off(11) + 0];
-    rgb[1] = bias_s[bias_off(11) + 1];
-    rgb[2] = bias_s[bias_off(11) + 2];
+    rgb[0] = bias_s[IDN_BIAS_OFF(11) + 0];
+    rgb[1] = bias_s[IDN_BIAS_OFF(11) + 1];
+    rgb[2] = bias_s[IDN_BIAS_OFF(11) + 2];
     {
         float part[3] = {0.f, 0.f, 0.f};
         static_for<4>([&](auto T) {
@@ -220,5 +277,6 @@
     }
     return false;
 }
-
-}
+#undef IDN_BIAS_OFF
+
+}
diff --git a/ideal-nerf_amd/ops.py b/ideal-nerf_amd/ops.py
--- a/ideal-nerf_amd/ops.py
+++ b/ideal-nerf_amd/ops.py
@@ -546,6 +546,8 @@
 
 
 COLOUR_GATE_DEFAULT = (os.environ.get("IDN_COLOUR_GATE", "1") or "1").strip() != "0"
+_zs = (os.environ.get("IDN_ZERO_SKIP", "") or "").strip()
+ZERO_SKIP_DEFAULT = None if _zs == "" else _zs != "0"
 
 
 def make_frame(c2w, H, W, focal, near, far, row0=0, nrows=None, cx=None, cy=None):
@@ -652,10 +654,14 @@
 def render_rays_fwd(rays, bc_rgb, packed_c, folded_c, packed_f, folded_f, t_vals, u, n_importance,
                     t_rand=None, with_fg=False, taps=False, precision=IDN_PREC_F32, precision_fine=None, lindisp=False,
                     white_bkgd=False, noise_coarse=None, noise_fine=None, fused=None, frame=None, draws=None,
-                    colour_gate=None, gate_counters=None) -> Dict[str, torch.Tensor]:
+                    colour_gate=None, gate_counters=None, zero_skip=None, skip_counters=None) -> Dict[str, torch.Tensor]:
     lib = _lib.load()
     if gate_counters is not None:
         _shape(gate_counters, "gate_counters", 2, 2)
+    if skip_counters is not None:
+        _shape(skip_counters, "skip_counters", 2, 2)
+    if zero_skip is None:
+        zero_skip = lib.idealnerf_zero_skip_default() if ZERO_SKIP_DEFAULT is None else ZERO_SKIP_DEFAULT
     if draws is not None and (u is not None or t_rand is not None):
         raise IdealNerfError("draws=(seed, ray0) replaces BOTH t_rand and u: pass them as None")
     _shape(t_vals, "t_vals", None)
@@ -679,11 +685,13 @@
             _u_shape(u, n, Ni)
         _net_buffers(lib, packed_f, folded_f, precision if precision_fine is None else precision_fine, "_fine")
     dev = bc_rgb.device
-    with _Launch(rays, bc_rgb, packed_c, folded_c, packed_f, folded_f, t_vals, u, t_rand, noise_coarse, noise_fine, gate_counters) as L:
+    with _Launch(rays, bc_rgb, packed_c, folded_c, packed_f, folded_f, t_vals, u, t_rand, noise_coarse, noise_fine, gate_counters, skip_counters) as L:
         new = lambda *s: torch.empty(s, dtype=torch.float32, device=dev)
-        opts = _lib.RenderOpts()
+        opts = _lib.RenderOpts2()
         opts.colour_gate = int(COLOUR_GATE_DEFAULT if colour_gate is None else bool(colour_gate))
+        opts.zero_skip = int(bool(zero_skip))
         opts.gate_counters = _ptr(gate_counters, "gate_counters", torch.int64)
+        opts.skip_counters = _ptr(skip_counters, "skip_counters", torch.int64)
         out = dict(rgb_map=new(n, 3), disp_map=new(n), acc_map=new(n))
         if Ni > 0:
             out.update(rgb0=new(n, 3), disp0=new(n), acc0=new(n), z_std=new(n), last_weight=new(n))
@@ -721,14 +729,14 @@
             nbytes = lib.idealnerf_render_workspace_bytes(n, S, Ni)
             ws = _workspace(nbytes, dev, L.stream or 0)
             a.workspace, a.workspace_bytes = ws.data_ptr(), ws.numel()
-            check(lib.idealnerf_render_rays_fwd_opts(C.byref(a), C.byref(opts), L.stream))
+            check(lib.idealnerf_render_rays_fwd_opts2(C.byref(a), C.byref(opts), L.stream))
         else:
             tap_rays = new(n, RAY_FLOATS) if taps else None
             frame.rays_out = None if tap_rays is None else tap_rays.data_ptr()
             nbytes = lib.idealnerf_render_frame_workspace_bytes(n, S, Ni)
             ws = _workspace(nbytes, dev, L.stream or 0)
             a.workspace, a.workspace_bytes = ws.data_ptr(), ws.numel()
-            check(lib.idealnerf_render_frame_fwd_opts(C.byref(a), C.byref(frame), C.byref(opts), L.stream))
+            check(lib.idealnerf_render_frame_fwd_opts2(C.byref(a), C.byref(frame), C.byref(opts), L.stream))
             frame.rays_out = None
             if tap_rays is not None:
                 out["tap_rays"] = tap_rays
diff --git a/include/idealnerf.h b/include/idealnerf.h
--- a/include/idealnerf.h
+++ b/include/idealnerf.h
@@ -171,6 +171,16 @@
 int idealnerf_render_frame_fwd_opts(const idn_render_args* a, const idn_frame* frame, const idn_render_opts* opts, void* stream);
 float idealnerf_colour_gate_max_dist(void);
 
+typedef struct idn_render_opts2 {
+    int colour_gate;
+    int zero_skip;
+    int64_t* gate_counters;
+    int64_t* skip_counters;
+} idn_render_opts2;
+int idealnerf_render_rays_fwd_opts2(const idn_render_args* a, const idn_render_opts2* opts, void* stream);
+int idealnerf_render_frame_fwd_opts2(const idn_render_args* a, const idn_frame* frame, const idn_render_opts2* opts, void* stream);
+int idealnerf_zero_skip_default(void);
+
 
 size_t idealnerf_train_acts_floats(int64_t n_points);
 
```

After: 118.6 million. 0.905x the previous value.
